# geometrian/simple-spectral

Measured on AMD Instinct MI355X. Metric: Msamples/s (w*h*spp/s) cornell-srgb 512x512, higher is better.
Workload: dtype f32

## Files before the change

### include/ssx.h

```cpp
#ifndef SSX_H
#define SSX_H

#include <stddef.h>
#include <stdint.h>

#ifdef __cplusplus
extern "C" {
#endif

#define SSX_ABI_VERSION 2

enum {
	SSX_OK = 0,
	SSX_ERR_DATA = -1,
	SSX_ERR_ARG = -2,
	SSX_ERR_SCENE = -3,
	SSX_ERR_DEVICE = -10,
	SSX_ERR_STATE = -11
};

#define SSX_MAX_DEPTH 10u
#define SSX_TILE_SIZE 8u
#define SSX_SAMPLE_WAVELENGTHS 4u
#define SSX_MAX_TEXTURES 64u
// ... 46 lines not shown
	uint32_t struct_size;
	uint32_t reserved;
	double pv_inv[16];
	float cam_pos[3];
	float lambda_min;
	float lambda_step;
	uint32_t spec_xbar, spec_ybar, spec_zbar;
	uint32_t spec_basis_r, spec_basis_g, spec_basis_b;
	const ssx_spectrum* spectra;  uint32_t n_spectra;
	const float* samples;         uint32_t n_samples;
	const ssx_material* materials; uint32_t n_materials;
	const ssx_quad* quads;        uint32_t n_quads;
	const uint32_t* lights;       uint32_t n_lights;
	const ssx_texture* textures;  uint32_t n_textures;
	float srgb_to_linear[256];
	uint32_t uplift;
	uint32_t jh_res;
	const float* jh_scale;
	const float* jh_data;
	const ssx_meng_grid* meng;
	float cam_dir[3];
	uint32_t reserved2;
} ssx_scene_desc;

typedef struct ssx_render_params {
	uint32_t struct_size;
	uint32_t width, height;
	uint32_t spp;
	uint32_t indirect_only;
	uint32_t tile_first;
	uint32_t tile_stride;
	uint32_t spp_per_launch;
	uint32_t no_explicit_light_sampling;
	uint32_t no_flat_field_correction;
	uint32_t tile_major;
	uint32_t tile_skew;
	uint64_t seed;
	uint32_t libm;
	uint32_t reserved3;
} ssx_render_params;
enum { SSX_LIBM_BUILD = 0, SSX_LIBM_GLIBC_2_35 = 1 };


typedef struct ssx_ctx ssx_ctx;

int ssx_create(int device, ssx_ctx** out);
void ssx_destroy(ssx_ctx* ctx);

int ssx_upload_scene(ssx_ctx* ctx, const ssx_scene_desc* scene);

int ssx_render_start(ssx_ctx* ctx, const ssx_render_params* params);
int ssx_render_stop(ssx_ctx* ctx);
int ssx_is_rendering(ssx_ctx* ctx);
float ssx_progress(ssx_ctx* ctx);
uint32_t ssx_done_spp(ssx_ctx* ctx);
uint32_t ssx_done_tiles(ssx_ctx* ctx);
int ssx_render_wait(ssx_ctx* ctx, float* xyza_out);

int ssx_render_device(ssx_ctx* ctx, const ssx_render_params* params, void* d_xyza_out, void* hip_stream);
int ssx_render_device_wait(ssx_ctx* ctx);

void* ssx_device_framebuffer(ssx_ctx* ctx);
int ssx_device_index(ssx_ctx* ctx);
int ssx_read_framebuffer(ssx_ctx* ctx, float* xyza_out);
int ssx_accumulate_peer(ssx_ctx* ctx, void* d_dst, int src_device, const void* d_src, uint32_t width, uint32_t height, void* hip_stream);

int ssx_reduce_rccl(ssx_ctx** ctxs, int n, uint32_t width, uint32_t height);
int ssx_rccl_probe(char* report, size_t report_size);
uint64_t ssx_rccl_groups_made(void);

const char* ssx_last_error(const ssx_ctx* ctx);

int ssx_set_timing(ssx_ctx* ctx, int enable);
int ssx_get_timing(ssx_ctx* ctx, float stage_ms[4]);

int ssx_abi_version(void);
int ssx_kernel_info(ssx_ctx* ctx, int* vgprs, int* sgprs, int* lds_bytes, int* scratch_bytes, int* max_blocks_per_cu);
int ssx_plan_info(ssx_ctx* ctx, float* frames_per_sample, int* fold_in_path_kernel);
int ssx_calibration_info(ssx_ctx* ctx, float* frames_per_sample, float* rays_left_per_sample, int* camera_rays_pretraced);
int ssx_scratch_info(ssx_ctx* ctx, uint64_t* sample_bytes, uint64_t* log_bytes);
int ssx_sums_info(ssx_ctx* ctx, uint64_t* units_parked, uint64_t* units_chained);
int ssx_units_info(ssx_ctx* ctx, uint64_t* units_enqueued);
int ssx_generate_info(ssx_ctx* ctx, uint64_t* generate_launches, uint64_t* fused_launches);
int ssx_kernel_variant(ssx_ctx* ctx);
enum { SSX_JIT_OFF = 0, SSX_JIT_AT_UPLOAD = 1, SSX_JIT_BACKGROUND = 2 };
int ssx_set_jit(ssx_ctx* ctx, int mode);
enum { SSX_JIT_STATE_NONE = 0,
       SSX_JIT_STATE_GENERIC_MEANWHILE = 1,
       SSX_JIT_STATE_SPECIALISED = 2,
       SSX_JIT_STATE_FAILED = -1 };
int ssx_jit_status(ssx_ctx* ctx, int wait_ms, char* message, size_t message_size);
void ssx_jit_counters(uint64_t* compiled, uint64_t* disk_hits);
const char* ssx_kernel_name(ssx_ctx* ctx);
enum { SSX_TRAIT_INDIRECT_ONLY = 1u, SSX_TRAIT_NO_ELS = 2u, SSX_TRAIT_MIRROR = 4u, SSX_TRAIT_TRI_LIGHT = 8u, SSX_TRAIT_UPLIFT = 16u,
       SSX_TRAIT_RGB_MODE = 32u, SSX_TRAIT_NO_FLAT_FIELD = 64u, SSX_TRAIT_KEEP_SAMPLES = 128u,
       SSX_TRAIT_LIBM = 256u, SSX_TRAIT_SPECTRAL_BINS = 512u, SSX_TRAIT_FORCED_OFF = 1024u };
int ssx_scene_traits(const ssx_scene_desc* scene);
int ssx_render_traits(const ssx_render_params* params);
int ssx_switches_info(ssx_ctx* ctx);


int ssx_render_continue(ssx_ctx* ctx, uint32_t spp_more);

typedef struct ssx_sums_info_t {
	uint32_t struct_size;
	uint32_t width, height;
	uint32_t done_spp;
	uint64_t seed;
	uint32_t indirect_only, no_explicit_light_sampling, no_flat_field_correction, libm;
	uint32_t rgb_mode;
	uint32_t tile_first, tile_stride, tile_skew;
	uint32_t noise_batches;
	uint32_t reserved;
	uint64_t scene_digest;
} ssx_sums_info_t;
uint64_t ssx_scene_digest(ssx_ctx* ctx);
int ssx_sums_export(ssx_ctx* ctx, ssx_sums_info_t* info, double* sums, double* noise_s2);
int ssx_sums_import(ssx_ctx* ctx, const ssx_render_params* params, const ssx_sums_info_t* info, const double* sums, const double* noise_s2);

int ssx_set_noise_estimate(ssx_ctx* ctx, int enable);
int ssx_noise_info(ssx_ctx* ctx, double* v_out, double summary[4]);


int ssx_set_spectral_bins(ssx_ctx* ctx, uint32_t bins);
typedef struct ssx_spectral_info_t {
	uint32_t struct_size;
	uint32_t width, height;
	uint32_t bins;
	uint32_t done_spp;
	uint32_t reserved;
	float lambda_min;
	float bin_width;
} ssx_spectral_info_t;
int ssx_spectral_read(ssx_ctx* ctx, ssx_spectral_info_t* info, float* mean, double* sums, uint32_t* counts);
int ssx_spectral_import(ssx_ctx* ctx, const ssx_spectral_info_t* info, const double* sums , const uint32_t* counts );


int ssx_guides(ssx_ctx* ctx, uint32_t width, uint32_t height, uint32_t* prim, float* depth, float* normal, float* albedo);
typedef struct ssx_denoise_params {
	uint32_t struct_size;
	uint32_t levels;
	float sigma_l, sigma_a;
} ssx_denoise_params;
int ssx_denoise_images(ssx_ctx* ctx, const ssx_denoise_params* params, uint32_t width, uint32_t height, const float* xyza, const float* var,
                       const uint32_t* prim, const float* albedo, float* xyza_out, float* var_out);
int ssx_denoise(ssx_ctx* ctx, const ssx_denoise_params* params, float* xyza_out, float* var_out);


int ssx_denoise_channels(ssx_ctx* ctx, const ssx_denoise_params* params, uint32_t width, uint32_t height, const float* xyza, const float* var,
                         const uint32_t* prim, const float* albedo, uint32_t channels, const float* extra ,
                         float* xyza_out, float* var_out, float* extra_out );
int ssx_denoise_spectral(ssx_ctx* ctx, const ssx_denoise_params* params, float* mean_out , float* xyza_out, float* var_out);


int ssx_develop_images(ssx_ctx* ctx, uint32_t width, uint32_t height, uint32_t bins, const float* q , const float* weights ,
                       uint32_t channels, float* out );
int ssx_spectral_develop(ssx_ctx* ctx, const ssx_denoise_params* denoise, const float* weights , uint32_t channels, float* out );


int ssx_albedo_bins(ssx_ctx* ctx, uint32_t width, uint32_t height, uint32_t bins, uint32_t supersample, float* rho_out );
#define SSX_DEMOD_DEFAULT_FLOOR 0.0625f
#define SSX_DEMOD_DEFAULT_SIGMA_L 1.0f
typedef struct ssx_demod_params {
	uint32_t struct_size;
	uint32_t supersample;
	float albedo_floor;
// ... 190 lines not shown
```

### simple_spectral_amd/_capi.py

```python
import ctypes as C
import os

from . import build as _build


class SsxSpectrum(C.Structure):
    _fields_ = [("offset", C.c_uint32), ("n", C.c_uint32), ("low", C.c_float), ("high", C.c_float),
                ("delta_recip", C.c_float)]


class SsxVertex(C.Structure):
    _fields_ = [("pos", C.c_float * 3), ("st", C.c_float * 2)]


class SsxQuad(C.Structure):
    _fields_ = [("v00", SsxVertex), ("v10", SsxVertex), ("v11", SsxVertex), ("v01", SsxVertex),
                ("normal0", C.c_float * 3), ("normal1", C.c_float * 3),
                ("material", C.c_uint32), ("flags", C.c_uint32)]


class SsxMaterial(C.Structure):
    _fields_ = [("kind", C.c_uint32), ("albedo_mode", C.c_uint32), ("albedo_spectrum", C.c_uint32),
                ("albedo_texture", C.c_uint32), ("emission_spectrum", C.c_uint32)]

# ... 41 lines not shown
                ("indirect_only", C.c_uint32), ("no_explicit_light_sampling", C.c_uint32), ("no_flat_field_correction", C.c_uint32), ("libm", C.c_uint32),
                ("rgb_mode", C.c_uint32), ("tile_first", C.c_uint32), ("tile_stride", C.c_uint32), ("tile_skew", C.c_uint32),
                ("noise_batches", C.c_uint32), ("reserved", C.c_uint32), ("scene_digest", C.c_uint64)]


class SsxSpectralInfo(C.Structure):
    _fields_ = [("struct_size", C.c_uint32), ("width", C.c_uint32), ("height", C.c_uint32), ("bins", C.c_uint32), ("done_spp", C.c_uint32),
                ("reserved", C.c_uint32), ("lambda_min", C.c_float), ("bin_width", C.c_float)]


class SsxDemodParams(C.Structure):
    _fields_ = [("struct_size", C.c_uint32), ("supersample", C.c_uint32), ("albedo_floor", C.c_float)]


SSX_DEMOD_DEFAULT_SUPERSAMPLE, SSX_DEMOD_DEFAULT_FLOOR, SSX_DEMOD_DEFAULT_SIGMA_L = 2, 0.0625, 1.0


class SsxDenoiseParams(C.Structure):
    _fields_ = [("struct_size", C.c_uint32), ("levels", C.c_uint32), ("sigma_l", C.c_float), ("sigma_a", C.c_float)]


class SsxOpticsParams(C.Structure):
    _fields_ = [("struct_size", C.c_uint32), ("cx", C.c_float), ("cy", C.c_float), ("max_radius", C.c_uint32),
                ("scale", C.c_void_p), ("radius", C.c_void_p), ("taps", C.c_void_p)]


SSX_OPTICS_MAX_RADIUS = 12


class SsxDefocusParams(C.Structure):
    _fields_ = [("struct_size", C.c_uint32), ("max_radius", C.c_uint32), ("gain", C.c_float), ("focus", C.c_void_p)]


SSX_DEFOCUS_MAX_RADIUS = 12


class SsxSensorParams(C.Structure):
    _fields_ = [("struct_size", C.c_uint32), ("cfa", C.c_uint32 * 4), ("noise", C.c_uint32), ("seed", C.c_uint32), ("frame", C.c_uint32),
                ("exposure", C.c_float), ("inv_exposure", C.c_float), ("read_var", C.c_float), ("dn_per_e", C.c_float), ("e_per_dn", C.c_float),
                ("black", C.c_float), ("white", C.c_float), ("weights", C.c_void_p), ("taps", C.c_void_p), ("ccm", C.c_void_p)]


SSH_DEMOSAIC_BILINEAR, SSH_DEMOSAIC_MHC = 0, 1


class SshSpectrum(C.Structure):
    _fields_ = [("samples", C.POINTER(C.c_float)), ("n", C.c_uint32), ("low", C.c_float), ("high", C.c_float)]


SSH_SPACE_XYZ, SSH_SPACE_LRGB = 0, 1
SSX_LIBM_BUILD, SSX_LIBM_GLIBC_2_35 = 0, 1
LIBM_MODES = {"build": SSX_LIBM_BUILD, "glibc-2.35": SSX_LIBM_GLIBC_2_35}


SSX_MODE_RGB, SSX_UPLIFT_OURS, SSX_UPLIFT_MENG, SSX_UPLIFT_JH = 0, 1, 2, 3
SSX_PRIM_LIGHT, SSX_PRIM_TRI = 1, 0x100
SSX_OK, SSX_ERR_DATA, SSX_ERR_ARG, SSX_ERR_SCENE, SSX_ERR_DEVICE, SSX_ERR_STATE = 0, -1, -2, -3, -10, -11
SSX_ABI_VERSION = 2
SSX_JIT_OFF, SSX_JIT_AT_UPLOAD, SSX_JIT_BACKGROUND = 0, 1, 2
(SSX_TRAIT_INDIRECT_ONLY, SSX_TRAIT_NO_ELS, SSX_TRAIT_MIRROR, SSX_TRAIT_TRI_LIGHT, SSX_TRAIT_UPLIFT, SSX_TRAIT_RGB_MODE, SSX_TRAIT_NO_FLAT_FIELD,
 SSX_TRAIT_KEEP_SAMPLES, SSX_TRAIT_LIBM, SSX_TRAIT_SPECTRAL_BINS, SSX_TRAIT_FORCED_OFF) = (1 << i for i in range(11))
SSX_JIT_STATE_NONE, SSX_JIT_STATE_GENERIC_MEANWHILE, SSX_JIT_STATE_SPECIALISED, SSX_JIT_STATE_FAILED = 0, 1, 2, -1

HIP_SYMBOLS = ["ssx_create", "ssx_destroy", "ssx_upload_scene", "ssx_render_start", "ssx_render_stop",
               "ssx_is_rendering", "ssx_progress", "ssx_render_wait", "ssx_render_device", "ssx_last_error",
               "ssx_abi_version", "ssx_kernel_info", "ssx_plan_info", "ssx_set_timing", "ssx_get_timing",
               "ssx_device_framebuffer", "ssx_device_index", "ssx_read_framebuffer", "ssx_accumulate_peer",
               "ssx_debug_eval", "ssx_debug_samples", "ssx_debug_sweep", "ssx_kernel_variant", "ssx_kernel_name", "ssx_scratch_info", "ssx_calibration_info", "ssx_set_jit", "ssx_debug_pass1_source", "ssx_done_spp", "ssx_reduce_rccl", "ssx_sums_info", "ssx_rccl_groups_made", "ssx_jit_status", "ssx_jit_counters", "ssx_done_tiles", "ssx_render_device_wait", "ssx_units_info", "ssx_rccl_probe",
               "ssx_render_continue", "ssx_scene_digest", "ssx_sums_export", "ssx_sums_import", "ssx_set_noise_estimate", "ssx_noise_info",
               "ssx_set_spectral_bins", "ssx_spectral_read", "ssx_debug_sample_flux",
               "ssx_guides", "ssx_denoise_images", "ssx_denoise", "ssx_denoise_channels", "ssx_denoise_spectral",
               "ssx_develop_images", "ssx_spectral_develop",
               "ssx_albedo_bins", "ssx_denoise_spectral_demod", "ssx_spectral_develop_demod",
               "ssx_spectral_import",
               "ssx_set_spectral_moments", "ssx_spectral_variance", "ssx_spectral_probe", "ssx_probe_arrays",
               "ssx_spectral_noise", "ssx_spectral_noise_reduce",
               "ssx_spectral_moments_import",
               "ssx_spectral_compare", "ssx_spectral_compare_arrays",
               "ssx_delta_e_images", "ssx_spectral_delta_e",
               "ssx_optics_images", "ssx_spectral_develop_optics",
               "ssx_defocus_images", "ssx_spectral_develop_lens",
               "ssx_sensor_images", "ssx_demosaic_images", "ssx_spectral_develop_sensor",
               "ssx_debug_tile_mask", "ssx_debug_spectral_accumulate", "ssx_debug_fold", "ssx_debug_step",
               "ssx_debug_generate", "ssx_generate_info",
               "ssx_scene_traits", "ssx_render_traits", "ssx_switches_info"]
SSX_GENERATE_FILL_BYTE = 0xA6
SSX_FOLD_ROW_WORDS, SSX_FOLD_LAMBDA0, SSX_FOLD_CAM_DIR, SSX_FOLD_HIT, SSX_FOLD_N, SSX_FOLD_LEVEL0, SSX_FOLD_LEVEL_WORDS = 160, 0, 1, 4, 5, 10, 15
SSX_FOLD_L_FS, SSX_FOLD_L_NDL, SSX_FOLD_L_PDF, SSX_FOLD_L_FLAGS, SSX_FOLD_L_EMISSION, SSX_FOLD_L_NEE = 0, 4, 5, 6, 7, 11
SSX_FOLD_EMISSION, SSX_FOLD_NEE, SSX_FOLD_NEE_VISIBLE = 1, 2, 4
SSX_STEP_ROW_WORDS, SSX_STEP_R_ORIG, SSX_STEP_R_DIR, SSX_STEP_R_IGNORE, SSX_STEP_R_DEPTH, SSX_STEP_R_LAMBDA0, SSX_STEP_R_RNG, SSX_STEP_R_PREV_SLOT = 16, 0, 3, 6, 7, 8, 9, 13
SSX_STEP_NO_SLOT, SSX_STEP_OUT_WORDS = 0x1FFF, 40
(SSX_STEP_O_FLAGS, SSX_STEP_O_HIT_TRI, SSX_STEP_O_HIT_DIST, SSX_STEP_O_HIT_ST, SSX_STEP_O_EMISSION, SSX_STEP_O_NEE, SSX_STEP_O_NEE_TERM, SSX_STEP_O_FS, SSX_STEP_O_NDL,
 SSX_STEP_O_PDF, SSX_STEP_O_PREV_SLOT, SSX_STEP_O_TAIL_DEPTH, SSX_STEP_O_TAIL_HIT, SSX_STEP_O_NEXT_ORIG, SSX_STEP_O_NEXT_DIR, SSX_STEP_O_NEXT_IGNORE,
 SSX_STEP_O_NEXT_DEPTH, SSX_STEP_O_RNG, SSX_STEP_O_SLOT) = 0, 1, 2, 3, 5, 9, 13, 17, 21, 22, 23, 24, 25, 26, 29, 32, 33, 34, 36
SSX_STEP_HIT, SSX_STEP_CONTINUED, SSX_STEP_EMISSION, SSX_STEP_PARKED, SSX_STEP_VISIBLE = 1, 2, 4, 8, 16
(SSX_SWEEP_RCP, SSX_SWEEP_SQRT, SSX_SWEEP_INVERSESQRT, SSX_SWEEP_SIN, SSX_SWEEP_COS, SSX_SWEEP_ACOS, SSX_SWEEP_DIV_PI,
 SSX_SWEEP_RCP64, SSX_SWEEP_DIV_PAIRS, SSX_SWEEP_ACOS_SIN, SSX_SWEEP_SIN_PROOF, SSX_SWEEP_COS_PROOF, SSX_SWEEP_ACOS_PROOF) = range(1, 14)
(SSX_DBG_FMATH, SSX_DBG_SPHTRI, SSX_DBG_ARVO, SSX_DBG_SAMPLE_LIGHT, SSX_DBG_COSHEMI, SSX_DBG_TRACE, SSX_DBG_RAND_CHOICE,
 SSX_DBG_ALBEDO, SSX_DBG_FLUX_TO_XYZ, SSX_DBG_RAND_1F) = range(1, 11)
(SSX_DBG_GLIBC_MATH, SSX_DBG_SPHTRI_GLIBC, SSX_DBG_ARVO_GLIBC, SSX_DBG_SAMPLE_LIGHT_GLIBC, SSX_DBG_COSHEMI_GLIBC) = range(11, 16)
(SSX_SWEEP_GLIBC_SIN, SSX_SWEEP_GLIBC_COS, SSX_SWEEP_GLIBC_ACOS, SSX_SWEEP_GLIBC_COS_LDS) = range(14, 18)
SSX_DBG_TRACE_TOPO = 17
SSX_DBG_TRACE_MASKED = 16
HOST_SYMBOLS = ["ssh_scene_create", "ssh_scene_create_ex", "ssh_scene_destroy", "ssh_scene_desc", "ssh_xyza_to_srgba", "ssh_save_image",
                "ssh_load_png_rgb8", "ssh_free", "ssh_color_values", "ssh_last_error", "ssh_checkpoint_save", "ssh_checkpoint_load", "ssh_sums_merge", "ssh_save_npy_f32",
                "ssh_develop_weights", "ssh_relight_gain", "ssh_emitter_spectrum",
                "ssh_checkpoint_save_spectral", "ssh_checkpoint_load_spectral", "ssh_spectral_merge",
                "ssh_probe_derive", "ssh_probe_save_csv", "ssh_spectral_noise_derive", "ssh_spectral_noise_save_csv",
                "ssh_checkpoint_save_moments", "ssh_checkpoint_load_moments", "ssh_moments_merge",
                "ssh_compare_derive", "ssh_compare_save_csv",
                "ssh_delta_e_derive", "ssh_delta_e_save_csv", "ssh_develop_white",
                "ssh_optics_lens", "ssh_defocus_thin_lens", "ssh_scene_vfov",
                "ssh_sensor_bayer", "ssh_sensor_exposure", "ssh_sensor_ccm", "ssh_sensor_standin_curve"]

_hip = None
_host = None


def host_lib():
    global _host
    if _host is None:
        path = _build.HOST_LIB
        if not os.path.exists(path):
            _build.build_host()
        lib = C.CDLL(path)
        vp = C.c_void_p
        lib.ssh_last_error.restype = C.c_char_p
        lib.ssh_scene_create.argtypes = [C.c_char_p, C.c_char_p, C.c_int, vp, C.c_uint32, C.c_uint32, C.c_char_p,
                                         C.c_float, C.POINTER(vp)]
        lib.ssh_scene_create_ex.argtypes = [C.c_char_p, C.c_char_p, C.c_int, vp, C.c_uint32, C.c_uint32, C.c_char_p,
                                            C.c_float, C.c_uint32, C.c_char_p, C.c_uint32, C.POINTER(vp)]
        lib.ssh_scene_destroy.argtypes = [vp]
        lib.ssh_scene_desc.restype = C.POINTER(SsxSceneDesc)
        lib.ssh_scene_desc.argtypes = [vp]
        lib.ssh_xyza_to_srgba.argtypes = [vp, vp, vp, C.c_size_t]
        lib.ssh_save_image.argtypes = [C.c_char_p, vp, C.c_uint32, C.c_uint32]
        lib.ssh_load_png_rgb8.argtypes = [C.c_char_p, C.POINTER(C.POINTER(C.c_uint8)), C.POINTER(C.c_uint32),
                                          C.POINTER(C.c_uint32)]
        lib.ssh_free.argtypes = [vp]
        lib.ssh_color_values.argtypes = [vp, C.c_char_p, C.POINTER(C.c_float), C.c_int]
        lib.ssh_checkpoint_save.argtypes = [C.c_char_p, C.POINTER(SsxSumsInfo), C.c_char_p, C.c_char_p, vp, vp]
        lib.ssh_checkpoint_load.argtypes = [C.c_char_p, C.POINTER(SsxSumsInfo), C.c_char_p, C.c_size_t, C.c_char_p, C.c_size_t,
                                            C.POINTER(C.POINTER(C.c_double)), C.POINTER(C.POINTER(C.c_double))]
        lib.ssh_sums_merge.argtypes = [vp, vp, vp, vp, C.POINTER(SsxSumsInfo)]
        lib.ssh_checkpoint_save_spectral.argtypes = [C.c_char_p, C.POINTER(SsxSumsInfo), C.c_char_p, C.c_char_p, vp, vp, C.POINTER(SsxSpectralInfo), vp, vp]
        lib.ssh_checkpoint_load_spectral.argtypes = [C.c_char_p, C.POINTER(SsxSumsInfo), C.c_char_p, C.c_size_t, C.c_char_p, C.c_size_t,
                                                     C.POINTER(C.POINTER(C.c_double)), C.POINTER(C.POINTER(C.c_double)),
                                                     C.POINTER(SsxSpectralInfo), C.POINTER(C.POINTER(C.c_double)), C.POINTER(C.POINTER(C.c_uint32))]
        lib.ssh_spectral_merge.argtypes = [vp, vp, vp, vp, C.c_uint32, C.POINTER(SsxSumsInfo)]
        lib.ssh_checkpoint_save_moments.argtypes = lib.ssh_checkpoint_save_spectral.argtypes + [vp]
        lib.ssh_checkpoint_load_moments.argtypes = lib.ssh_checkpoint_load_spectral.argtypes + [C.POINTER(C.POINTER(C.c_double))]
        lib.ssh_moments_merge.argtypes = [vp, vp, C.c_uint32, C.POINTER(SsxSumsInfo)]
        lib.ssh_save_npy_f32.argtypes = [C.c_char_p, vp, C.POINTER(C.c_uint32), C.c_uint32]
        lib.ssh_probe_derive.argtypes = [C.c_uint32, C.c_uint32, vp, vp, vp, vp, vp, vp]
        lib.ssh_probe_save_csv.argtypes = [C.c_char_p, C.c_uint32, C.c_uint32, C.c_float, C.c_float, vp, vp, vp, vp]
        lib.ssh_spectral_noise_derive.argtypes = [C.c_uint32, vp, vp, vp, vp, vp, vp, vp]
        lib.ssh_spectral_noise_save_csv.argtypes = [C.c_char_p, C.c_uint32, C.c_float, C.c_float, vp, vp, vp, vp]
        lib.ssh_compare_derive.argtypes = [C.c_uint32, C.c_uint32] + [vp] * 12
        lib.ssh_compare_save_csv.argtypes = [C.c_char_p, C.c_uint32, C.c_uint32, C.c_float, C.c_float] + [vp] * 6
        lib.ssh_delta_e_derive.argtypes = [C.c_uint32] + [vp] * 11
        lib.ssh_delta_e_save_csv.argtypes = [C.c_char_p, C.c_uint32] + [vp] * 6
        lib.ssh_develop_white.argtypes = [vp, C.c_uint32, C.c_float, C.c_float, C.POINTER(SshSpectrum), vp]
        lib.ssh_develop_weights.argtypes = [C.c_char_p, C.c_int, C.POINTER(SshSpectrum), C.c_uint32, C.POINTER(SshSpectrum), vp, C.c_int, C.c_uint32,
                                            C.c_float, C.c_float, vp, vp]
        lib.ssh_relight_gain.argtypes = [C.POINTER(SshSpectrum), C.POINTER(SshSpectrum), C.c_uint32, C.c_float, C.c_float, vp]
        lib.ssh_emitter_spectrum.argtypes = [C.POINTER(SsxSceneDesc), C.POINTER(C.c_uint32)]
        lib.ssh_optics_lens.argtypes = [C.c_uint32, C.c_float, C.c_float, C.c_double, C.c_double, C.c_double, C.c_double, C.c_uint32, vp, vp, vp]
# ... 121 lines not shown
            lib.ssx_done_spp.argtypes = [vp]
            lib.ssx_done_spp.restype = C.c_uint32
            lib.ssx_reduce_rccl.argtypes = [C.POINTER(vp), C.c_int, C.c_uint32, C.c_uint32]
            lib.ssx_debug_pass1_source.argtypes = [C.POINTER(C.c_uint8), C.c_uint32, C.c_char_p, C.c_char_p, C.c_size_t]
        if not override or hasattr(lib, "ssx_sums_info"):
            lib.ssx_sums_info.argtypes = [vp, C.POINTER(C.c_uint64), C.POINTER(C.c_uint64)]
        if hasattr(lib, "ssx_rccl_probe"):
            lib.ssx_rccl_probe.argtypes = [C.c_char_p, C.c_size_t]
        if hasattr(lib, "ssx_units_info"):
            lib.ssx_units_info.argtypes = [vp, C.POINTER(C.c_uint64)]
        if not override or hasattr(lib, "ssx_jit_status"):
            lib.ssx_jit_status.argtypes = [vp, C.c_int, C.c_char_p, C.c_size_t]
            lib.ssx_jit_counters.argtypes = [C.POINTER(C.c_uint64), C.POINTER(C.c_uint64)]
            lib.ssx_jit_counters.restype = None
            lib.ssx_rccl_groups_made.restype = C.c_uint64
            lib.ssx_render_device_wait.argtypes = [vp]
            lib.ssx_done_tiles.argtypes = [vp]
            lib.ssx_done_tiles.restype = C.c_uint32
        if not override or hasattr(lib, "ssx_render_continue"):
            lib.ssx_render_continue.argtypes = [vp, C.c_uint32]
            lib.ssx_scene_digest.argtypes = [vp]
            lib.ssx_scene_digest.restype = C.c_uint64
            lib.ssx_sums_export.argtypes = [vp, C.POINTER(SsxSumsInfo), vp, vp]
            lib.ssx_sums_import.argtypes = [vp, C.POINTER(SsxRenderParams), C.POINTER(SsxSumsInfo), vp, vp]
            lib.ssx_set_noise_estimate.argtypes = [vp, C.c_int]
            lib.ssx_noise_info.argtypes = [vp, vp, C.POINTER(C.c_double)]
        if not override or hasattr(lib, "ssx_set_spectral_bins"):
            lib.ssx_set_spectral_bins.argtypes = [vp, C.c_uint32]
            lib.ssx_spectral_read.argtypes = [vp, C.POINTER(SsxSpectralInfo), vp, vp, vp]
            lib.ssx_debug_sample_flux.argtypes = [vp, C.POINTER(SsxRenderParams), vp, vp]
        if not override or hasattr(lib, "ssx_denoise"):
            lib.ssx_guides.argtypes = [vp, C.c_uint32, C.c_uint32, vp, vp, vp, vp]
            lib.ssx_denoise_images.argtypes = [vp, C.POINTER(SsxDenoiseParams), C.c_uint32, C.c_uint32, vp, vp, vp, vp, vp, vp]
            lib.ssx_denoise.argtypes = [vp, C.POINTER(SsxDenoiseParams), vp, vp]
        if not override or hasattr(lib, "ssx_denoise_spectral"):
            lib.ssx_denoise_channels.argtypes = [vp, C.POINTER(SsxDenoiseParams), C.c_uint32, C.c_uint32, vp, vp, vp, vp, C.c_uint32, vp, vp, vp, vp]
            lib.ssx_denoise_spectral.argtypes = [vp, C.POINTER(SsxDenoiseParams), vp, vp, vp]
        if not override or hasattr(lib, "ssx_spectral_develop"):
            lib.ssx_develop_images.argtypes = [vp, C.c_uint32, C.c_uint32, C.c_uint32, vp, vp, C.c_uint32, vp]
            lib.ssx_spectral_develop.argtypes = [vp, C.POINTER(SsxDenoiseParams), vp, C.c_uint32, vp]
        if not override or hasattr(lib, "ssx_albedo_bins"):
            lib.ssx_albedo_bins.argtypes = [vp, C.c_uint32, C.c_uint32, C.c_uint32, C.c_uint32, vp]
            lib.ssx_denoise_spectral_demod.argtypes = [vp, C.POINTER(SsxDenoiseParams), C.POINTER(SsxDemodParams), vp, vp, vp, vp]
            lib.ssx_spectral_develop_demod.argtypes = [vp, C.POINTER(SsxDenoiseParams), C.POINTER(SsxDemodParams), vp, vp, C.c_uint32, vp]
        if not override or hasattr(lib, "ssx_spectral_import"):
            lib.ssx_spectral_import.argtypes = [vp, C.POINTER(SsxSpectralInfo), vp, vp]
        if not override or hasattr(lib, "ssx_set_spectral_moments"):
            lib.ssx_set_spectral_moments.argtypes = [vp, C.c_int]
            lib.ssx_spectral_variance.argtypes = [vp, C.POINTER(SsxSpectralInfo), vp, vp]
            lib.ssx_spectral_probe.argtypes = [vp, vp, C.c_uint32, vp, vp, vp, vp]
            lib.ssx_probe_arrays.argtypes = [vp, C.c_uint32, C.c_uint32, C.c_uint32, vp, vp, vp, vp, C.c_uint32, vp, vp, vp, vp]
        if not override or hasattr(lib, "ssx_spectral_noise"):
            lib.ssx_spectral_noise.argtypes = [vp] * 10
            lib.ssx_spectral_noise_reduce.argtypes = [vp, C.c_uint32, C.c_uint32] + [vp] * 8
        if not override or hasattr(lib, "ssx_spectral_compare"):
            lib.ssx_spectral_compare.argtypes = [vp, C.POINTER(SsxSpectralInfo), vp, vp, vp, vp, C.c_uint32, C.c_double] + [vp] * 8
            lib.ssx_spectral_compare_arrays.argtypes = [vp, C.c_uint32, C.c_uint32, C.c_uint32] + [vp] * 7 + [C.c_uint32, C.c_double] + [vp] * 8
        if not override or hasattr(lib, "ssx_delta_e_images"):
            lib.ssx_delta_e_images.argtypes = [vp, C.c_uint32, C.c_uint32] + [vp] * 5 + [C.c_uint32] + [vp] * 9
            lib.ssx_spectral_delta_e.argtypes = [vp, C.POINTER(SsxDenoiseParams), C.c_int, C.c_int] + [vp] * 5 + [C.c_uint32] + [vp] * 9
        if not override or hasattr(lib, "ssx_optics_images"):
            lib.ssx_optics_images.argtypes = [vp, C.c_uint32, C.c_uint32, C.c_uint32, vp, C.POINTER(SsxOpticsParams), vp]
            lib.ssx_spectral_develop_optics.argtypes = [vp, C.POINTER(SsxDenoiseParams), C.POINTER(SsxOpticsParams), vp, C.c_uint32, vp, vp]
        if not override or hasattr(lib, "ssx_defocus_images"):
            lib.ssx_defocus_images.argtypes = [vp, C.c_uint32, C.c_uint32, C.c_uint32, vp, vp, C.POINTER(SsxDefocusParams), vp]
            lib.ssx_spectral_develop_lens.argtypes = [vp, C.POINTER(SsxDenoiseParams), C.POINTER(SsxDefocusParams), C.POINTER(SsxOpticsParams), vp, C.c_uint32, vp, vp]
        if not override or hasattr(lib, "ssx_sensor_images"):
            lib.ssx_sensor_images.argtypes = [vp, C.c_uint32, C.c_uint32, C.c_uint32, vp, C.POINTER(SsxSensorParams), vp, vp]
            lib.ssx_demosaic_images.argtypes = [vp, C.c_uint32, C.c_uint32, vp, C.POINTER(SsxSensorParams), vp]
            lib.ssx_spectral_develop_sensor.argtypes = [vp, C.POINTER(SsxDenoiseParams), C.POINTER(SsxDefocusParams), C.POINTER(SsxOpticsParams), C.POINTER(SsxSensorParams), vp, vp, vp]
        if not override or hasattr(lib, "ssx_spectral_moments_import"):
            lib.ssx_spectral_moments_import.argtypes = [vp, C.POINTER(SsxSpectralInfo), vp]
        if not override or hasattr(lib, "ssx_debug_tile_mask"):
            lib.ssx_debug_tile_mask.argtypes = [vp, C.POINTER(SsxRenderParams), vp]
        if not override or hasattr(lib, "ssx_debug_spectral_accumulate"):
            lib.ssx_debug_spectral_accumulate.argtypes = [vp] + [C.c_uint32] * 6 + [C.c_float, C.c_float, C.c_uint32] + [vp] * 6
        if not override or hasattr(lib, "ssx_debug_fold"):
            lib.ssx_debug_fold.argtypes = [vp, C.POINTER(SsxRenderParams), C.c_uint32, C.c_uint32, vp, C.c_uint32, C.c_uint32, vp, vp, vp]
        if not override or hasattr(lib, "ssx_debug_step"):
            lib.ssx_debug_step.argtypes = [vp, C.POINTER(SsxRenderParams), C.c_uint32, C.c_uint32, vp, vp]
        if not override or hasattr(lib, "ssx_debug_generate"):
            lib.ssx_debug_generate.argtypes = [vp, C.POINTER(SsxRenderParams), C.c_uint32, C.c_uint32, C.c_int, vp, vp, vp]
            lib.ssx_generate_info.argtypes = [vp, C.POINTER(C.c_uint64), C.POINTER(C.c_uint64)]
        lib.ssx_kernel_variant.argtypes = [vp]
        lib.ssx_kernel_name.argtypes = [vp]
        lib.ssx_kernel_name.restype = C.c_char_p
        if hasattr(lib, "ssx_switches_info"):
            lib.ssx_switches_info.argtypes = [vp]
            lib.ssx_scene_traits.argtypes = [vp]
            lib.ssx_render_traits.argtypes = [vp]
        _hip = lib
    return _hip
```

### simple_spectral_amd/csrc/ssx_api.hip

```cpp
#include "ssx_kernels.hip"
#include "ssx_debug.hip"

#include "../../include/ssx.h"

#include <chrono>
#include <array>
#include <atomic>
#include <cstdarg>
#include <cstdio>
#include <cstdlib>
#include <cmath>
#include <algorithm>
#include <cstring>
#include <mutex>
#include <string>
#include <thread>
#include <vector>

#include <limits.h>
#include <set>

#include "ssx_jit.h"

namespace {
// ... 2 lines not shown

const char* debug_env(const char* name) {
	const char* m = getenv("SSX_DEBUG_ENV");
	if (!m || m[0] != '1' || m[1] != '\0') return nullptr;
	return getenv(name);
}
bool env_on(const char* name) { const char* e = debug_env(name); return e && e[0] != '\0' && e[0] != '0'; }

std::string fmt(const char* f, ...) {
	char buf[512];
	va_list ap; va_start(ap, f); vsnprintf(buf, sizeof buf, f, ap); va_end(ap);
	return buf;
}

struct DeviceBuffer {
	void* ptr = nullptr;
	size_t bytes = 0;
	DeviceBuffer() = default;
	DeviceBuffer(DeviceBuffer&& o) noexcept : ptr(o.ptr), bytes(o.bytes) { o.ptr = nullptr; o.bytes = 0; }
	DeviceBuffer& operator=(DeviceBuffer&& o) noexcept { std::swap(ptr, o.ptr); std::swap(bytes, o.bytes); return *this; }
	~DeviceBuffer() { release(); }
	void release() { if (ptr) (void)hipFree(ptr); ptr = nullptr; bytes = 0; }
	hipError_t reserve(size_t n) {
		if (n <= bytes) return hipSuccess;
		release();
		const hipError_t e = hipMalloc(&ptr, n);
		if (e == hipSuccess) bytes = n; else ptr = nullptr;
		return e;
	}
	template <class T> T* as() const { return static_cast<T*>(ptr); }
};

}

#include "ssx_pack.h"

struct ssx_ctx {
	int device = 0;
	int n_cus = 0;
	hipStream_t stream = nullptr;
	DeviceBuffer d_blob;
	uint32_t blob_words = 0;
	uint32_t path_blob_words = 0;
	uint32_t topology = 0;
	int jit_mode = SSX_JIT_BACKGROUND;
	const ssx_jit::Kernels* jit_kernels[ssx_jit::kVariants] = {};
	uint32_t libm = SSX_LIBM_BUILD;
	uint32_t variant = SSX_LIBM_BUILD;
	bool jit_pending = false, jit_requested = false;
	ssx_jit::VidTable jit_vid;
	DeviceBuffer d_blob_jit; uint32_t blob_jit_words = 0, path_blob_jit_words = 0;
	uint64_t generic_samples = 0;
	int jit_state = SSX_JIT_STATE_NONE; std::string jit_message;
	std::vector<DeviceBuffer> d_textures;
	DeviceBuffer d_jh_data;
	bool rgb_mode = false;
	uint32_t scene_traits = 0;
	bool fuse_resolve = true;
	float calib_frames = 0.0f;
	float calib_left = 0.0f;
	bool pre_hits = false;
	DeviceBuffer d_accum;
	DeviceBuffer d_unit_counter;
	int resident_blocks = 0;
	int gen_blocks = 0;
	uint32_t max_wave_slots = 0;
	uint32_t queue_words = SSX_QUEUE_WORDS_WIDE;
	DeviceBuffer d_samples;
	DeviceBuffer d_logs;
	DeviceBuffer d_out;
	DeviceBuffer d_peer;
	bool have_scene = false;
	bool have_cam_dir = false;

	std::thread worker;
	std::atomic<int> rendering{0};
	std::atomic<int> stop_flag{0};
	std::atomic<uint32_t> done_spp{0};
	std::atomic<uint32_t> done_tiles{0};
	uint32_t total_spp = 0;
	int worker_rc = 0;
	std::atomic<uint64_t> units_enqueued{0};
	std::atomic<uint64_t> launches_generated{0}, launches_fused{0};
	ssx_render_params cur{};
	struct SumsState { bool continuable = false, noise_valid = false, spectral_valid = false, moments_valid = false, imported = false, spectral_imported = false; uint32_t noise_batches = 0; } sums;
	uint32_t k_begin = 0;
	uint64_t scene_digest = 0;
	bool noise_on = false;
	DeviceBuffer d_noise;
	DeviceBuffer d_stage;
	uint32_t spectral_bins = 0;
	DeviceBuffer d_spectral_sums, d_spectral_counts;
	std::string spectral_note;
	float lambda_min = 0.0f, lambda_step = 0.0f;
	uint32_t n_quads = 0;
	bool spectral_moments = false;
	DeviceBuffer d_spectral_moments, d_probe;
	std::string moments_note;
	DeviceBuffer d_guides, d_denoise, d_denoise_channels;
	DeviceBuffer d_develop;
	DeviceBuffer d_optics;
	DeviceBuffer d_defocus;
	DeviceBuffer d_sensor;
	uint32_t guides_width = 0, guides_height = 0;
	DeviceBuffer d_albedo_bins, d_demod;
	uint32_t abins_width = 0, abins_height = 0, abins_bins = 0, abins_supersample = 0;
	uint64_t abins_serial = 0;
	const void* demod_rc_base = nullptr; uint64_t demod_rc_bins_serial = 0; float demod_rc_floor = 0.0f; std::vector<float> demod_rc_weights;

	bool timing = false;
	std::vector<hipEvent_t> ev_pool;
	size_t ev_used = 0;
	float stage_ms[4] = { 0, 0, 0, 0 };

	hipEvent_t ev_device_done = nullptr;
	bool device_pending = false;

	void* rccl_comm = nullptr; uint64_t rccl_group = 0; int rccl_rank = -1, rccl_size = 0;

	std::mutex error_mutex;
	std::string error;
	std::string error_out;
};

namespace {

void set_error(ssx_ctx* ctx, const std::string& msg) { std::lock_guard<std::mutex> g(ctx->error_mutex); ctx->error = msg; }

#define SSX_HIP(ctx, call)                                                                          \
	do {                                                                                            \
		hipError_t e_ = (call);                                                                     \
		if (e_ != hipSuccess) {                                                                     \
			set_error((ctx), fmt("%s failed: %s", #call, hipGetErrorString(e_)));                   \
			return SSX_ERR_DEVICE;                                                                  \
		}                                                                                           \
	} while (0)

int fail(ssx_ctx* ctx, int code, const std::string& msg) { set_error(ctx, msg); return code; }

int check_params(ssx_ctx* ctx, const ssx_render_params* p) {
	if (!p || p->struct_size != sizeof(ssx_render_params)) return fail(ctx, SSX_ERR_ARG, "ssx_render_params.struct_size mismatch");
	if (p->libm != SSX_LIBM_BUILD && p->libm != SSX_LIBM_GLIBC_2_35) return fail(ctx, SSX_ERR_ARG, "ssx_render_params.libm: unknown value");
	if (!ctx->have_scene) return fail(ctx, SSX_ERR_STATE, "no scene uploaded");
	if (p->width == 0 || p->height == 0 || p->spp == 0) return fail(ctx, SSX_ERR_ARG, "width, height and spp must be positive");
	if ((uint64_t)p->width * p->height > (1ull << 28)) return fail(ctx, SSX_ERR_ARG, "image too large");
	if (p->tile_stride == 0 || p->tile_first >= p->tile_stride) return fail(ctx, SSX_ERR_ARG, "need tile_first < tile_stride");
	if (p->no_flat_field_correction && !ctx->have_cam_dir) return fail(ctx, SSX_ERR_ARG, "no_flat_field_correction needs ssx_scene_desc.cam_dir (caller built against an older ssx.h)");
	return SSX_OK;
}

int take_params(ssx_ctx* ctx, const ssx_render_params* in, ssx_render_params* out) {
	if (!in) return fail(ctx, SSX_ERR_ARG, "ssx_render_params is NULL");
	memset(out, 0, sizeof *out);
	if (in->struct_size == offsetof(ssx_render_params, libm)) { memcpy(out, in, offsetof(ssx_render_params, libm)); out->struct_size = sizeof *out; }
	else memcpy(out, in, in->struct_size == sizeof *out ? sizeof *out : sizeof out->struct_size);
	return check_params(ctx, out);
}
int begin_render(ssx_ctx* ctx, const ssx_render_params* in, ssx_render_params* out, const char* busy) {
	const int rc = take_params(ctx, in, out);
	if (rc) return rc;
	return ctx->rendering.load() ? fail(ctx, SSX_ERR_STATE, busy) : SSX_OK;
}

int wait_device_pending(ssx_ctx* ctx) {
	if (ctx->device_pending) { SSX_HIP(ctx, hipEventSynchronize(ctx->ev_device_done)); ctx->device_pending = false; }
	return SSX_OK;
}

int idle_on_device(ssx_ctx* ctx) {
	if (ctx->rendering.load()) return fail(ctx, SSX_ERR_STATE, "render in progress");
	SSX_HIP(ctx, hipSetDevice(ctx->device));
	return wait_device_pending(ctx);
}

uint32_t tiles_across(uint32_t pixels) { return (pixels + 7u) / 8u; }
size_t accum_bytes(uint32_t width, uint32_t height) { return (size_t)tiles_across(width) * tiles_across(height) * 64u * 4 * sizeof(double); }
size_t image_bytes(uint32_t width, uint32_t height) { return (size_t)width * height * 4 * sizeof(float); }

SsxPixelGrid pixel_grid(const ssx_render_params* p) {
	const uint32_t tx = tiles_across(p->width);
	return SsxPixelGrid{ p->width, p->height, tx, p->tile_first, p->tile_stride, p->tile_skew % tx };
}
uint32_t owned_tiles(const ssx_render_params& p) {
	const uint32_t n_tiles = tiles_across(p.width) * tiles_across(p.height);
	return n_tiles > p.tile_first ? (n_tiles - p.tile_first + p.tile_stride - 1u) / p.tile_stride : 0u;
}
dim3 pixel_blocks(const ssx_render_params* p) { return dim3((p->width * p->height + 255u) / 256u); }

int clear_sums(ssx_ctx* ctx, uint32_t width, uint32_t height, hipStream_t stream) {
	SSX_HIP(ctx, hipMemsetAsync(ctx->d_accum.ptr, 0, accum_bytes(width, height), stream));
	return SSX_OK;
}
void sums_invalidate(ssx_ctx* ctx) { ctx->sums = ssx_ctx::SumsState{}; }
void sums_publish(ssx_ctx* ctx, uint32_t done_spp, int64_t noise_batches = -1) {
	if (noise_batches >= 0) { ctx->sums.noise_valid = true; ctx->sums.noise_batches = (uint32_t)noise_batches; }
	ctx->done_spp.store(done_spp); ctx->sums.continuable = true;
}

constexpr size_t kSampleBufferBudget = (size_t)16 << 30;
size_t bytes_per_sample(const ssx_ctx* ctx) { return ctx->spectral_bins ? SSX_BYTES_PER_SAMPLE_FLUX : SSX_BYTES_PER_SAMPLE; }
constexpr size_t kAuxWordsPer64Records = 5;
size_t bytes_per_64_records(const ssx_ctx* ctx) { return 64u * bytes_per_sample(ctx) + kAuxWordsPer64Records * sizeof(uint32_t); }
size_t sample_bytes(const ssx_ctx* ctx, size_t records) { return records / 64u * bytes_per_64_records(ctx); }
size_t sample_slots(const ssx_ctx* ctx) { return ctx->d_samples.bytes / bytes_per_64_records(ctx) * 64u; }
size_t log_records(const ssx_ctx* ctx) { return ctx->d_logs.bytes / SSX_LOG_BYTES_PER_RECORD; }
constexpr uint32_t kMinUnits = 3072;
constexpr uint64_t kSamplesPerSync = (uint64_t)32 << 20;

struct LaunchPlan { SsxKernelArgs args; uint32_t max_spp_per_launch; };

uint32_t scene_traits_of(const ssx_scene_desc* s) {
	uint32_t t = 0;
	for (uint32_t q = 0; q < s->n_quads; ++q) if (s->quads[q].material < s->n_materials && s->materials[s->quads[q].material].kind != SSX_MTL_LAMBERTIAN) t |= SSX_TRAIT_MIRROR;
	for (uint32_t i = 0; i < s->n_lights; ++i) if (s->lights[i] < s->n_quads && (s->quads[s->lights[i]].flags & SSX_PRIM_TRI)) t |= SSX_TRAIT_TRI_LIGHT;
	if (s->uplift == SSX_MODE_RGB) t |= SSX_TRAIT_RGB_MODE;
	else if (s->uplift != SSX_UPLIFT_OURS) t |= SSX_TRAIT_UPLIFT;
	return t;
}
uint32_t render_traits_of(const ssx_render_params* p, bool keep_samples) {
	return (p->indirect_only ? SSX_TRAIT_INDIRECT_ONLY : 0u) | (p->no_explicit_light_sampling ? SSX_TRAIT_NO_ELS : 0u) |
	       (p->no_flat_field_correction ? SSX_TRAIT_NO_FLAT_FIELD : 0u) | (keep_samples ? SSX_TRAIT_KEEP_SAMPLES : 0u) | (p->libm != SSX_LIBM_BUILD ? SSX_TRAIT_LIBM : 0u);
}
uint32_t traits_of(const ssx_ctx* ctx, const ssx_render_params* p, bool keep_samples) {
	const char* e = debug_env("SSX_PLAIN_KERNEL");
	return ctx->scene_traits | render_traits_of(p, keep_samples) | (ctx->spectral_bins ? SSX_TRAIT_SPECTRAL_BINS : 0u) | (e && e[0] == '0' ? SSX_TRAIT_FORCED_OFF : 0u);
}
uint32_t variant_of(const ssx_ctx* ctx, const ssx_render_params* p, bool keep_samples = false) {
	if (ctx->spectral_bins && p->libm == SSX_LIBM_BUILD && !ctx->rgb_mode) return ssx_jit::kVariantFlux;
	return traits_of(ctx, p, keep_samples) == 0u ? (uint32_t)ssx_jit::kVariantPlain : p->libm;
}

LaunchPlan make_plan(ssx_ctx* ctx, const ssx_render_params* p, bool ask_device = true) {
	LaunchPlan pl{};
	SsxKernelArgs& a = pl.args;
	a.blob = ctx->d_blob.as<uint32_t>(); a.blob_words = ctx->path_blob_words;
	a.width = p->width; a.height = p->height;
	a.inv_width = 1.0 / (double)p->width; a.inv_height = 1.0 / (double)p->height;
	a.tiles_x = tiles_across(p->width);
	a.n_tiles = a.tiles_x * tiles_across(p->height);
	a.tile_first = p->tile_first; a.tile_stride = p->tile_stride; a.tile_skew = p->tile_skew % a.tiles_x;
	a.indirect_only = p->indirect_only ? 1u : 0u;
	a.no_els = p->no_explicit_light_sampling ? 1u : 0u;
	a.no_flat_field = p->no_flat_field_correction ? 1u : 0u;
	a.seed = p->seed;
	a.rgb_mode = ctx->rgb_mode ? 1u : 0u;
	a.fuse_resolve = ctx->fuse_resolve ? 1u : 0u;
	a.pre_hits = ctx->pre_hits ? 1u : 0u;
	a.my_tiles = owned_tiles(*p);
	size_t per_spp = (size_t)(a.my_tiles ? a.my_tiles : 1u) * 64u * bytes_per_sample(ctx);
	size_t budget = kSampleBufferBudget, free_b = 0, total_b = 0;
	if (ask_device && hipMemGetInfo(&free_b, &total_b) == hipSuccess) {
		const size_t avail = (size_t)((double)(free_b + sample_slots(ctx) * bytes_per_sample(ctx)) * 0.8);
		if (avail < budget) budget = avail;
	}
	size_t cap = budget / per_spp;
	const size_t idx_cap = (size_t)0xFFFFFFFFu / ((size_t)(a.my_tiles ? a.my_tiles : 1u) * 64u);
	if (cap > idx_cap) cap = idx_cap;
	pl.max_spp_per_launch = (uint32_t)(cap < 1 ? 1 : (cap > 65536 ? 65536 : cap));
	return pl;
}

void cap_to_allocation(const ssx_ctx* ctx, LaunchPlan& pl) {
	const size_t per_spp = (size_t)(pl.args.my_tiles ? pl.args.my_tiles : 1u) * 64u;
	const size_t fit = sample_slots(ctx) / per_spp;
	if (fit >= 1 && fit < pl.max_spp_per_launch) pl.max_spp_per_launch = (uint32_t)fit;
}

int ensure_samples(ssx_ctx* ctx, const LaunchPlan& pl, uint32_t n_k) {
	const size_t need = (size_t)pl.args.my_tiles * 64u * n_k;
	const hipError_t e = ctx->d_samples.reserve(sample_bytes(ctx, need));
	if (e == hipErrorOutOfMemory) { (void)hipGetLastError(); return fail(ctx, SSX_ERR_DEVICE, fmt("out of device memory for %zu samples in flight; lower spp_per_launch", need)); }
	SSX_HIP(ctx, e);
	return SSX_OK;
// ... 74 lines not shown
	a.n_groups = (n_k + a.group_spp - 1) / a.group_spp;
	b.units = a.my_tiles * a.n_groups;
	b.n_rec = a.n_records;
	b.rc = ensure_logs(ctx, a.unit_cohorts);
	if (b.rc == SSX_OK) bind_arrays(a, ctx->d_samples.as<uint8_t>(), a.n_records, ctx->d_logs.as<uint8_t>(), log_records(ctx), ctx->spectral_bins != 0u);
	a.accum = ctx->d_accum.as<double>();
	uint32_t* const aux = reinterpret_cast<uint32_t*>(ctx->d_samples.as<uint8_t>() + sample_slots(ctx) * bytes_per_sample(ctx));
	a.unit_state = aux;
	a.tile_mask = aux + b.units;
	if (b.rc == SSX_OK && (size_t)a.my_tiles * 4u + b.units > (sample_slots(ctx) / 64u) * kAuxWordsPer64Records) b.rc = fail(ctx, SSX_ERR_STATE, "internal: launch larger than the sample allocation");
	return b;
}

size_t staged_blob_lds(uint32_t blob_words) { return ((size_t)blob_words + SSX_LDS_PREFIX_WORDS) * 4; }
size_t path_lds_bytes(uint32_t blob_words, uint32_t queue_words) {
	size_t n = staged_blob_lds(blob_words) + 4u * ((size_t)SSX_QUEUE_ENTRIES * queue_words + SSX_WAVE_COUNTER_WORDS) * 4u;
#ifdef SSX_REGTIME
	n += 4u * SSX_NTIME * 8u;
#endif
	return n;
}
struct PathKernel { const char* name; void (*host)(SsxKernelArgs); };
#define SSX_PK(k) { #k, k }
static const PathKernel kPathKernels[ssx_jit::kVariants][3][2] = {
	{ { SSX_PK(ssx_render_kernel), SSX_PK(ssx_render_kernel_nq) }, { SSX_PK(ssx_render_kernel_cornell), SSX_PK(ssx_render_kernel_cornell_nq) },
	  { SSX_PK(ssx_render_kernel_plane), SSX_PK(ssx_render_kernel_plane_nq) } },
	{ { SSX_PK(ssx_render_kernel_glibc), SSX_PK(ssx_render_kernel_nq_glibc) }, { SSX_PK(ssx_render_kernel_cornell_glibc), SSX_PK(ssx_render_kernel_cornell_nq_glibc) },
	  { SSX_PK(ssx_render_kernel_plane_glibc), SSX_PK(ssx_render_kernel_plane_nq_glibc) } },
	{ { SSX_PK(ssx_render_kernel_flux), SSX_PK(ssx_render_kernel_nq_flux) }, { SSX_PK(ssx_render_kernel_cornell_flux), SSX_PK(ssx_render_kernel_cornell_nq_flux) },
	  { SSX_PK(ssx_render_kernel_plane_flux), SSX_PK(ssx_render_kernel_plane_nq_flux) } },
	{ { SSX_PK(ssx_render_kernel_plain), SSX_PK(ssx_render_kernel_nq_plain) }, { SSX_PK(ssx_render_kernel_cornell_plain), SSX_PK(ssx_render_kernel_cornell_nq_plain) },
	  { SSX_PK(ssx_render_kernel_plane_plain), SSX_PK(ssx_render_kernel_plane_nq_plain) } } };
#undef SSX_PK
static const char* const kJitKernelNames[2] = { "ssx_render_kernel_jit", "ssx_render_kernel_jit_nq" };
const PathKernel& path_kernel_of(const ssx_ctx* ctx, bool narrow) { return kPathKernels[ctx->variant][ctx->topology < 3u ? ctx->topology : 0u][narrow]; }
struct KernelRef { const void* host = nullptr; hipFunction_t mod = nullptr; };
KernelRef path_kernel_ref(const ssx_ctx* ctx, bool narrow) {
	KernelRef k;
	const ssx_jit::Kernels* jk = ctx->jit_kernels[ctx->variant];
	if (ctx->topology == 3u && jk) k.mod = narrow ? jk->path_nq : jk->path;
	else k.host = (const void*)path_kernel_of(ctx, narrow).host;
	return k;
}
int occupancy_of(ssx_ctx* ctx, const KernelRef& k, size_t lds, int* per_cu) {
	if (k.mod) SSX_HIP(ctx, hipModuleOccupancyMaxActiveBlocksPerMultiprocessor(per_cu, k.mod, 256, lds));
	else SSX_HIP(ctx, hipOccupancyMaxActiveBlocksPerMultiprocessor(per_cu, k.host, 256, lds));
	return SSX_OK;
}
int blocks_that_fit(ssx_ctx* ctx, const KernelRef& k, size_t lds, int* blocks) {
	int per_cu = 0;
	const int rc = occupancy_of(ctx, k, lds, &per_cu);
	if (rc) return rc;
	*blocks = (per_cu > 0 ? per_cu : 1) * ctx->n_cus;
	return SSX_OK;
}
int launch_kernel(ssx_ctx* ctx, const KernelRef& k, uint32_t blocks, size_t lds, hipStream_t stream, SsxKernelArgs& a) {
	if (k.mod) {
		size_t size = sizeof a;
		void* config[] = { HIP_LAUNCH_PARAM_BUFFER_POINTER, &a, HIP_LAUNCH_PARAM_BUFFER_SIZE, &size, HIP_LAUNCH_PARAM_END };
		SSX_HIP(ctx, hipModuleLaunchKernel(k.mod, blocks, 1, 1, 256, 1, 1, (unsigned)lds, stream, nullptr, config));
	} else {
		void* args[] = { &a };
		SSX_HIP(ctx, hipLaunchKernel(k.host, dim3(blocks), dim3(256), args, lds, stream));
	}
	return SSX_OK;
}
int pick_queue(ssx_ctx* ctx, uint32_t blob_words, uint32_t* queue_words, int* blocks_per_cu) {
	int wide = 0, narrow = 0, rc;
	if (path_lds_bytes(blob_words, SSX_QUEUE_WORDS_WIDE) <= 65536u)
		if ((rc = occupancy_of(ctx, path_kernel_ref(ctx, false), path_lds_bytes(blob_words, SSX_QUEUE_WORDS_WIDE), &wide))) return rc;
	if ((rc = occupancy_of(ctx, path_kernel_ref(ctx, true), path_lds_bytes(blob_words, SSX_QUEUE_WORDS_NARROW), &narrow))) return rc;
	const bool use_narrow = narrow > wide || env_on("SSX_NARROW_QUEUE");
	*queue_words = use_narrow ? SSX_QUEUE_WORDS_NARROW : SSX_QUEUE_WORDS_WIDE;
	if (blocks_per_cu) *blocks_per_cu = use_narrow ? narrow : wide;
	return SSX_OK;
}

bool fuses_generate(const ssx_ctx* ctx, const SsxKernelArgs& a) {
	const char* fuse_env = debug_env("SSX_FUSE_GEN");
	const bool tiles_fit = a.tiles_x <= 0xFFFFu && tiles_across(a.height) <= 0xFFFFu;
	return ctx->topology == 2u && !a.pre_hits && tiles_fit && !(fuse_env && fuse_env[0] == '0');
}

int enqueue_generate(ssx_ctx* ctx, const Batch& b, hipStream_t stream) {
	SsxKernelArgs ga = b.a;
	ga.blob_words = ctx->blob_words;
	if (ga.pre_hits) {
		hipLaunchKernelGGL(ssx_tile_mask_kernel, dim3((ga.my_tiles + 3u) / 4u), dim3(256), 0, stream, ga);
		SSX_HIP(ctx, hipGetLastError());
	}
	const KernelRef gen_kernel{ (const void*)ssx_generate_kernel };
	const size_t gen_lds = staged_blob_lds(ga.blob_words);
	if (ctx->gen_blocks == 0) { const int rc = blocks_that_fit(ctx, gen_kernel, gen_lds, &ctx->gen_blocks); if (rc) return rc; }
	const uint64_t want = (b.n_rec + 255u) / 256u;
	return launch_kernel(ctx, gen_kernel, (uint32_t)(want < (uint64_t)ctx->gen_blocks ? want : (uint64_t)ctx->gen_blocks), gen_lds, stream, ga);
}

int enqueue_path(ssx_ctx* ctx, Batch& b, const KernelRef& kernel, uint32_t queue_words, uint32_t blob_words, int resident_blocks, hipStream_t stream) {
	if (!ctx->d_unit_counter.ptr) {
		SSX_HIP(ctx, ctx->d_unit_counter.reserve(4 * sizeof(uint32_t)));
		SSX_HIP(ctx, hipMemsetAsync(ctx->d_unit_counter.ptr, 0, 4 * sizeof(uint32_t), stream));
	}
	b.a.blob_words = blob_words; b.a.queue_words = queue_words;
	SSX_HIP(ctx, hipMemsetAsync(ctx->d_unit_counter.ptr, 0, 2 * sizeof(uint32_t), stream));
	SSX_HIP(ctx, hipMemsetAsync(b.a.unit_state, 0, (size_t)b.units * sizeof(uint32_t), stream));
	b.a.unit_counter = ctx->d_unit_counter.as<uint32_t>();
	const uint32_t want_blocks = (b.units + 3u) / 4u;
	uint32_t blocks = want_blocks < (uint32_t)resident_blocks ? want_blocks : (uint32_t)resident_blocks;
	if (blocks * 4u > ctx->max_wave_slots) blocks = ctx->max_wave_slots / 4u;
	return launch_kernel(ctx, kernel, blocks, path_lds_bytes(blob_words, queue_words), stream, b.a);
}

int launch_batch(ssx_ctx* ctx, Batch& b, hipStream_t stream) {
	if (b.rc) return b.rc;
	int rc;
	if (ctx->variant == ssx_jit::kVariantPlain && (b.a.indirect_only | b.a.no_els | b.a.no_flat_field | b.a.rgb_mode | b.a.keep_samples | ctx->scene_traits))
		return fail(ctx, SSX_ERR_STATE, "internal: a render with a switch set was about to launch the kernel with the switches compiled in");
	if (ctx->timing) { if ((rc = timing_events(ctx, &b.tev))) return rc; SSX_HIP(ctx, hipEventRecord(b.tev[0], stream)); }
	b.a.fuse_gen = fuses_generate(ctx, b.a) ? 1u : 0u;
	if (!b.a.fuse_gen && (rc = enqueue_generate(ctx, b, stream))) return rc;
	if (ctx->timing) SSX_HIP(ctx, hipEventRecord(b.tev[1], stream));
	const bool plan = ctx->resident_blocks == 0;
	if (plan && (rc = pick_queue(ctx, b.a.blob_words, &ctx->queue_words, nullptr))) return rc;
	const KernelRef path_kernel = path_kernel_ref(ctx, ctx->queue_words == SSX_QUEUE_WORDS_NARROW);
	if (plan && (rc = blocks_that_fit(ctx, path_kernel, path_lds_bytes(b.a.blob_words, ctx->queue_words), &ctx->resident_blocks))) return rc;
	if ((rc = enqueue_path(ctx, b, path_kernel, ctx->queue_words, b.a.blob_words, ctx->resident_blocks, stream))) return rc;
	ctx->units_enqueued.fetch_add(b.units);
	(b.a.fuse_gen ? ctx->launches_fused : ctx->launches_generated).fetch_add(1u);
	if (ctx->timing) for (int k = 2; k < 6; ++k) SSX_HIP(ctx, hipEventRecord(b.tev[k], stream));
	return SSX_OK;
}

constexpr uint64_t kJitAfterSamples = kSamplesPerSync;
void maybe_swap_jit(ssx_ctx* ctx, uint64_t samples) {
	if (!ctx->jit_pending) return;
	std::string err;
	const ssx_jit::Kernels* k = nullptr;
	const ssx_jit::State st = ssx_jit::lookup(ctx->device, ctx->jit_vid, &k, &err, ctx->variant);
	if (st == ssx_jit::State::Ready) {
		std::swap(ctx->d_blob, ctx->d_blob_jit);
		ctx->blob_words = ctx->blob_jit_words; ctx->path_blob_words = ctx->path_blob_jit_words;
		ctx->topology = 3u;
		ctx->jit_kernels[ctx->variant] = k;
		ctx->resident_blocks = 0; ctx->gen_blocks = 0;
		ctx->jit_pending = false; ctx->jit_state = SSX_JIT_STATE_SPECIALISED;
	} else if (st == ssx_jit::State::Failed) {
		ctx->jit_pending = false; ctx->jit_state = SSX_JIT_STATE_FAILED; ctx->jit_message = err;
	} else {
		ctx->generic_samples += samples;
		if (!ctx->jit_requested && ctx->generic_samples >= kJitAfterSamples) { ssx_jit::request(ctx->jit_vid, ctx->variant); ctx->jit_requested = true; }
	}
}

int ensure_libm_kernels(ssx_ctx* ctx, uint32_t libm) {
	const ssx_jit::Kernels*& have = ctx->jit_kernels[libm];
	if (ctx->topology != 3u || have) return SSX_OK;
	std::string err;
	const ssx_jit::Kernels* k = ssx_jit::get(ctx->device, ctx->jit_vid, &err, libm);
	if (!k) return fail(ctx, SSX_ERR_STATE, "the scene's specialised kernels for this libm could not be compiled: " + err);
	have = k;
	return SSX_OK;
}

int ready_to_launch(ssx_ctx* ctx, const ssx_render_params* p, bool need_out, bool keep_samples = false) {
	const uint32_t variant = variant_of(ctx, p, keep_samples);
	const int rc = ensure_libm_kernels(ctx, variant);
	if (rc) return rc;
	ctx->libm = p->libm;
	if (ctx->variant != variant) { ctx->variant = variant; ctx->resident_blocks = 0; ctx->jit_requested = false; }
	SSX_HIP(ctx, ctx->d_accum.reserve(accum_bytes(p->width, p->height)));
	if (need_out) SSX_HIP(ctx, ctx->d_out.reserve(image_bytes(p->width, p->height)));
	return SSX_OK;
}

int launch_range(ssx_ctx* ctx, LaunchPlan& pl, uint32_t k0, uint32_t k1, hipStream_t stream) {
	if (pl.args.my_tiles == 0 || k1 <= k0) return SSX_OK;
	Batch b = make_batch(ctx, pl, k0, k1);
	return launch_batch(ctx, b, stream);
}

int launch_batches(ssx_ctx* ctx, LaunchPlan& pl, uint32_t spp, uint32_t batch, hipStream_t stream) {
	for (uint32_t k0 = 0; k0 < spp; k0 += batch) {
		int rc = launch_range(ctx, pl, k0, (spp - k0 < batch) ? spp : k0 + batch, stream);
		if (rc) return rc;
	}
	return SSX_OK;
}

int calibrate(ssx_ctx* ctx) {
	ssx_render_params cp{};
	cp.struct_size = sizeof cp; cp.width = 64; cp.height = 64; cp.spp = 4; cp.tile_stride = 1;
	ctx->fuse_resolve = false;
	ctx->pre_hits = false;
	LaunchPlan pl = make_plan(ctx, &cp);
	int rc = ensure_samples(ctx, pl, cp.spp);
	if (rc) return rc;
	Batch b = make_batch(ctx, pl, 0, cp.spp);
	if (b.rc) return b.rc;
	if ((rc = enqueue_generate(ctx, b, ctx->stream))) return rc;
	const KernelRef kernel{ (const void*)ssx_calibrate_kernel };
	int blocks = 0;
	if ((rc = blocks_that_fit(ctx, kernel, path_lds_bytes(ctx->blob_words, SSX_QUEUE_WORDS_NARROW), &blocks))) return rc;
	if ((rc = enqueue_path(ctx, b, kernel, SSX_QUEUE_WORDS_NARROW, ctx->blob_words, blocks, ctx->stream))) return rc;
	SSX_HIP(ctx, hipStreamSynchronize(ctx->stream));
	std::vector<uint4> recs((size_t)b.n_rec);
	SSX_HIP(ctx, hipMemcpy(recs.data(), b.a.st, recs.size() * sizeof(uint4), hipMemcpyDeviceToHost));
	uint64_t frames = 0;
	for (const uint4& r : recs) frames += (r.y >> 2) & 0xFu;
	ctx->calib_frames = (float)((double)frames / (double)recs.size());
	uint32_t counters[2] = { 0u, 0u };
	SSX_HIP(ctx, hipMemcpy(counters, ctx->d_unit_counter.ptr, sizeof counters, hipMemcpyDeviceToHost));
	ctx->calib_left = (float)((double)counters[1] / (double)recs.size());
	ctx->pre_hits = ctx->calib_left >= 0.3f;
	if (const char* e = debug_env("SSX_PRE_HITS")) { if (e[0] != '\0') ctx->pre_hits = e[0] != '0'; }
	ctx->fuse_resolve = true;
	return ensure_logs(ctx, (unit_spp_of(ctx) + SSX_COHORT_KS - 1u) / SSX_COHORT_KS);
}

int launch_finalize(ssx_ctx* ctx, const ssx_render_params* p, uint32_t spp, float* d_out, hipStream_t stream, uint32_t done_tiles = 0xFFFFFFFFu) {
	hipLaunchKernelGGL(ssx_finalize_kernel, pixel_blocks(p), dim3(256), 0, stream,
	                   ctx->d_accum.as<const double>(), (float4*)d_out, pixel_grid(p), spp, ctx->rgb_mode ? 1u : 0u, done_tiles);
	SSX_HIP(ctx, hipGetLastError());
	return SSX_OK;
}

int noise_begin(ssx_ctx* ctx, const ssx_render_params* p, uint32_t k_begin, bool continuing);
int noise_batch(ssx_ctx* ctx, const ssx_render_params* p, uint32_t n_k, hipStream_t stream);
int spectral_refuses(ssx_ctx* ctx, const ssx_render_params& p, bool tile_walk);
int spectral_begin(ssx_ctx* ctx, uint32_t my_tiles, bool continuing, bool* active);
int spectral_batch(ssx_ctx* ctx, const ssx_render_params* p, const LaunchPlan& pl, uint32_t n_k, hipStream_t stream);
int moments_reserve(ssx_ctx* ctx, uint32_t my_tiles, bool continuing);
int moments_begin(ssx_ctx* ctx, uint32_t my_tiles, bool continuing, bool spectral, bool* active);
int moments_batch(ssx_ctx* ctx, const ssx_render_params* p, const LaunchPlan& pl, uint32_t n_k, hipStream_t stream);
void moments_publish(ssx_ctx* ctx, bool active);
void moments_invalidate(ssx_ctx* ctx, const char* why);
void moments_drop(ssx_ctx* ctx);

int finish_walk(ssx_ctx* ctx, const ssx_render_params& p, uint32_t spp, uint32_t done_tiles) {
	if (const int rc = launch_finalize(ctx, &p, spp, ctx->d_out.as<float>(), ctx->stream, done_tiles)) return rc;
	SSX_HIP(ctx, hipStreamSynchronize(ctx->stream));
	return SSX_OK;
}

uint32_t sample_walk_chunk(const ssx_render_params& p, uint32_t span, const LaunchPlan& pl) {
	const size_t pixels = (size_t)p.width * p.height;
	const uint64_t min_spp = kSamplesPerSync / (pixels ? pixels : 1) + 1u;
	uint32_t chunk = p.spp_per_launch ? p.spp_per_launch : (span + 31u) / 32u;
	if (!p.spp_per_launch && chunk < min_spp) chunk = (uint32_t)(min_spp < span ? min_spp : span);
	if (chunk == 0) chunk = 1;
	return chunk > pl.max_spp_per_launch ? pl.max_spp_per_launch : chunk;
}

struct TileLaunch { uint32_t tiles, spp; };
TileLaunch tile_walk_launch(const ssx_render_params& p, const LaunchPlan& pl) {
	const uint32_t owned = pl.args.my_tiles;
	uint32_t spp_l = p.spp_per_launch ? p.spp_per_launch : p.spp;
	if (spp_l > p.spp) spp_l = p.spp;
	uint64_t per_launch = kSamplesPerSync / ((uint64_t)64 * p.spp) + 1u;
	if (const char* e = debug_env("SSX_TILES_PER_LAUNCH")) { const int v = atoi(e); if (v >= 1) per_launch = (uint64_t)v; }
	if (per_launch > owned) per_launch = owned;
	const uint64_t budget_records = (uint64_t)pl.max_spp_per_launch * owned * 64u;
	while (spp_l > 1u && (uint64_t)spp_l * 64u > budget_records) spp_l = (spp_l + 1u) / 2u;
	const uint64_t fit = budget_records / ((uint64_t)spp_l * 64u);
	if (per_launch > fit) per_launch = fit ? fit : 1u;
	return TileLaunch{ (uint32_t)per_launch, spp_l };
}

int render_sample_walk(ssx_ctx* ctx, const ssx_render_params& p, uint32_t k_begin, bool continuing) {
	int rc;
	if (!continuing && (rc = clear_sums(ctx, p.width, p.height, ctx->stream))) return rc;
	if ((rc = noise_begin(ctx, &p, k_begin, continuing))) return rc;
	maybe_swap_jit(ctx, 0);
	if ((rc = moments_reserve(ctx, owned_tiles(p), continuing))) return rc;
	LaunchPlan pl = make_plan(ctx, &p);
	bool spectral = false, moments = false;
	if ((rc = spectral_begin(ctx, pl.args.my_tiles, continuing, &spectral))) return rc;
	if ((rc = moments_begin(ctx, pl.args.my_tiles, continuing, spectral, &moments))) return rc;
	const uint32_t span = p.spp - k_begin, chunk = sample_walk_chunk(p, span, pl);
	if ((rc = ensure_samples(ctx, pl, chunk < span ? chunk : span))) return rc;
	for (uint32_t k0 = k_begin; k0 < p.spp && !ctx->stop_flag.load(); k0 += chunk) {
		const uint32_t k1 = (p.spp - k0 < chunk) ? p.spp : k0 + chunk;
		if (ctx->jit_pending) {
			maybe_swap_jit(ctx, (uint64_t)p.width * p.height * (k1 - k0) / p.tile_stride);
			if (!ctx->jit_pending) { const uint32_t cap = pl.max_spp_per_launch; pl = make_plan(ctx, &p); pl.max_spp_per_launch = cap; }
		}
		if ((rc = launch_range(ctx, pl, k0, k1, ctx->stream))) return rc;
		if (ctx->noise_on && (rc = noise_batch(ctx, &p, k1 - k0, ctx->stream))) return rc;
		if (spectral && (rc = spectral_batch(ctx, &p, pl, k1 - k0, ctx->stream))) return rc;
		if (moments && (rc = moments_batch(ctx, &p, pl, k1 - k0, ctx->stream))) return rc;
		SSX_HIP(ctx, hipStreamSynchronize(ctx->stream));
		ctx->done_spp.store(k1);
	}
	const uint32_t done = ctx->done_spp.load();
	if ((rc = finish_walk(ctx, p, done ? done : p.spp, 0xFFFFFFFFu))) return rc;
	ctx->done_tiles.store(pl.args.my_tiles);
	ctx->sums.spectral_valid = spectral;
	if (!spectral) ctx->spectral_note = "the render that made these sums ran without them (it continued sums that had none)";
	moments_publish(ctx, moments);
	sums_publish(ctx, done);
	return SSX_OK;
}

int render_tile_walk(ssx_ctx* ctx, const ssx_render_params& p) {
	int rc;
	if ((rc = clear_sums(ctx, p.width, p.height, ctx->stream))) return rc;
	maybe_swap_jit(ctx, 0);
	const LaunchPlan pl = make_plan(ctx, &p);
	const uint32_t owned = pl.args.my_tiles;
	const TileLaunch per = tile_walk_launch(p, pl);
	LaunchPlan sized = pl; sized.args.my_tiles = per.tiles;
	if ((rc = ensure_samples(ctx, sized, per.spp))) return rc;
	for (uint32_t j0 = 0; j0 < owned && !ctx->stop_flag.load(); j0 += per.tiles) {
		const uint32_t j1 = (owned - j0 < per.tiles) ? owned : j0 + per.tiles;
		maybe_swap_jit(ctx, (uint64_t)(j1 - j0) * 64u * p.spp);
		LaunchPlan part = make_plan(ctx, &p);
		part.args.tile_first = p.tile_first + p.tile_stride * j0;
		part.args.my_tiles = j1 - j0;
		if ((rc = launch_batches(ctx, part, p.spp, per.spp, ctx->stream))) return rc;
		SSX_HIP(ctx, hipStreamSynchronize(ctx->stream));
		ctx->done_tiles.store(j1);
		ctx->done_spp.store((uint32_t)((uint64_t)p.spp * j1 / owned));
	}
	const uint32_t done = ctx->done_tiles.load();
	if ((rc = finish_walk(ctx, p, p.spp, done))) return rc;
	if (done == owned) sums_publish(ctx, p.spp);
	return SSX_OK;
}

int render_walk(ssx_ctx* ctx, const ssx_render_params p, uint32_t k_begin, bool continuing) {
	SSX_HIP(ctx, hipSetDevice(ctx->device));
	return (p.tile_major && !continuing) ? render_tile_walk(ctx, p) : render_sample_walk(ctx, p, k_begin, continuing);
}
void worker_main(ssx_ctx* ctx, uint32_t k_begin, bool continuing) {
	const int rc = render_walk(ctx, ctx->cur, k_begin, continuing);
	if (rc) sums_invalidate(ctx);
	ctx->worker_rc = rc;
	ctx->rendering.store(0);
}

int start_worker(ssx_ctx* ctx, const ssx_render_params& p, uint32_t k_begin, bool continuing, uint32_t total_spp) {
	if (ctx->worker.joinable()) ctx->worker.join();
	if (const int rc = spectral_refuses(ctx, p, p.tile_major && !continuing)) return rc;
	if (const int rc = ready_to_launch(ctx, &p, true)) return rc;
	ctx->cur = p; ctx->total_spp = total_spp; ctx->k_begin = k_begin;
	if (!continuing) { sums_invalidate(ctx); ctx->done_spp.store(0); ctx->done_tiles.store(0); }
	ctx->sums.imported = ctx->sums.spectral_imported = false;
	ctx->stop_flag.store(0); ctx->worker_rc = 0;
	ctx->rendering.store(1);
	ctx->worker = std::thread(worker_main, ctx, k_begin, continuing);
	return SSX_OK;
}

uint64_t digest_mix(uint64_t h, uint64_t w) {
	uint64_t z = (h ^ w) + 0x9E3779B97F4A7C15ull;
	z = (z ^ (z >> 30)) * 0xBF58476D1CE4E5B9ull;
	z = (z ^ (z >> 27)) * 0x94D049BB133111EBull;
	return z ^ (z >> 31);
}
uint64_t digest_bytes(uint64_t h, const void* data, size_t n) {
	const uint8_t* p = static_cast<const uint8_t*>(data);
	h = digest_mix(h, (uint64_t)n);
	for (; n >= 8; n -= 8, p += 8) { uint64_t w; memcpy(&w, p, 8); h = digest_mix(h, w); }
	if (n) { uint64_t w = 0; memcpy(&w, p, n); h = digest_mix(h, w); }
	return h;
}
uint64_t scene_digest_of(const ssx_scene_desc* s) {
	std::vector<uint32_t> blob;
	std::string err;
	const std::vector<const void*> no_tex(s->n_textures, nullptr);
	if (pack_blob(s, no_tex, nullptr, blob, err) != SSX_OK) return 0;
	uint64_t h = digest_bytes(0x5353584449474553ull, blob.data(), blob.size() * 4);
	for (uint32_t i = 0; i < s->n_textures; ++i) h = digest_bytes(h, s->textures[i].rgb, (size_t)3 * s->textures[i].width * s->textures[i].height);
	if (s->uplift == SSX_UPLIFT_JH) h = digest_bytes(h, s->jh_data, (size_t)3 * s->jh_res * s->jh_res * s->jh_res * 3 * sizeof(float));
	if (s->uplift == SSX_UPLIFT_MENG) {
		const ssx_meng_grid* g = s->meng;
// ... 175 lines not shown
	const uint32_t upload_variant = variant_of(ctx, &defaults) == ssx_jit::kVariantPlain ? (uint32_t)ssx_jit::kVariantPlain : (uint32_t)SSX_LIBM_BUILD;
	if (ctx->variant == SSX_LIBM_BUILD || ctx->variant == ssx_jit::kVariantPlain) ctx->variant = upload_variant;
	if (info.candidate && jit_mode != SSX_JIT_OFF) {
		std::string err;
		const ssx_jit::Kernels* k = nullptr;
		ssx_jit::State st = ssx_jit::lookup(ctx->device, info.vid, &k, &err, upload_variant);
		if (st != ssx_jit::State::Ready && st != ssx_jit::State::Failed && jit_mode == SSX_JIT_AT_UPLOAD) {
			k = ssx_jit::get(ctx->device, info.vid, &err, upload_variant);
			st = k ? ssx_jit::State::Ready : ssx_jit::State::Failed;
		}
		if (st == ssx_jit::State::Failed) { ctx->jit_state = SSX_JIT_STATE_FAILED; ctx->jit_message = err; }
		else if ((rc = pack_blob(s, tex, ctx->d_jh_data.ptr, blob_jit, pack_err, 3))) return fail(ctx, rc, pack_err);
		else if (st == ssx_jit::State::Ready) { blob.swap(blob_jit); blob_jit.clear(); ctx->jit_kernels[upload_variant] = k; ctx->jit_vid = info.vid; ctx->jit_state = SSX_JIT_STATE_SPECIALISED; }
		else { ctx->jit_pending = true; ctx->jit_vid = info.vid; ctx->jit_state = SSX_JIT_STATE_GENERIC_MEANWHILE; ctx->jit_requested = (st == ssx_jit::State::Pending); }
	}
	if (ctx->jit_pending) {
		SSX_HIP(ctx, ctx->d_blob_jit.reserve(blob_jit.size() * 4));
		SSX_HIP(ctx, hipMemcpy(ctx->d_blob_jit.ptr, blob_jit.data(), blob_jit.size() * 4, hipMemcpyHostToDevice));
		const SsxBlobHeader* bh = reinterpret_cast<const SsxBlobHeader*>(blob_jit.data());
		ctx->blob_jit_words = (uint32_t)blob_jit.size(); ctx->path_blob_jit_words = bh->words_without_perm;
	}
	SSX_HIP(ctx, ctx->d_blob.reserve(blob.size() * 4));
	SSX_HIP(ctx, hipMemcpy(ctx->d_blob.ptr, blob.data(), blob.size() * 4, hipMemcpyHostToDevice));
	ctx->blob_words = (uint32_t)blob.size();
	{
		SsxBlobHeader* bh = reinterpret_cast<SsxBlobHeader*>(blob.data());
		ctx->topology = bh->topology;
		ctx->path_blob_words = (bh->topology || bh->perm_hbm) ? bh->words_without_perm : ctx->blob_words;
		if (bh->perm_hbm) {
			const uint64_t at = (uint64_t)(uintptr_t)(ctx->d_blob.as<uint32_t>() + bh->off_perm);
			bh->perm_ptr_lo = (uint32_t)at; bh->perm_ptr_hi = (uint32_t)(at >> 32);
			SSX_HIP(ctx, hipMemcpy(ctx->d_blob.ptr, blob.data(), sizeof(SsxBlobHeader), hipMemcpyHostToDevice));
			ctx->blob_words = bh->words_without_perm;
		}
	}
	ctx->have_cam_dir = have_cam_dir;
	ctx->lambda_min = s->lambda_min; ctx->lambda_step = s->lambda_step;
	ctx->n_quads = s->n_quads;
	ctx->resident_blocks = 0; ctx->gen_blocks = 0;
	ctx->have_scene = true;
	ctx->scene_digest = scene_digest_of(s);
	return calibrate(ctx);
}

static uint32_t device_batch(const ssx_render_params* p, const LaunchPlan& pl) {
	uint32_t batch = p->spp_per_launch ? p->spp_per_launch : p->spp;
	if (batch > p->spp) batch = p->spp;
	if (batch > pl.max_spp_per_launch) {
		const uint32_t n = (p->spp + pl.max_spp_per_launch - 1u) / pl.max_spp_per_launch;
		batch = (p->spp + n - 1u) / n;
	}
	return batch;
}

int ssx_render_device(ssx_ctx* ctx, const ssx_render_params* p_in, void* d_xyza_out, void* hip_stream) {
	if (!ctx) return SSX_ERR_ARG;
	ssx_render_params pp;
	int rc = take_params(ctx, p_in, &pp);
	if (rc) return rc;
	const ssx_render_params* const p = &pp;
	if (!d_xyza_out) return fail(ctx, SSX_ERR_ARG, "d_xyza_out is NULL");
	if (ctx->spectral_bins) return fail(ctx, SSX_ERR_ARG, "spectral output is on (ssx_set_spectral_bins): ssx_render_device does not bin its samples; use ssx_render_start");
	if (ctx->rendering.load()) return fail(ctx, SSX_ERR_STATE, "asynchronous render in progress");
	hipStream_t stream = (hipStream_t)hip_stream;
	SSX_HIP(ctx, hipSetDevice(ctx->device));
	if (!ctx->ev_device_done) SSX_HIP(ctx, hipEventCreateWithFlags(&ctx->ev_device_done, hipEventDisableTiming));
	hipStreamCaptureStatus capture = hipStreamCaptureStatusNone;
	(void)hipStreamIsCapturing(stream, &capture);
	const bool capturing = capture == hipStreamCaptureStatusActive;
	if (ctx->device_pending && capturing) return fail(ctx, SSX_ERR_STATE, "a render of this context may still be queued: ssx_render_device_wait before capturing another into a graph");
	if (capturing && ctx->variant != variant_of(ctx, p)) return fail(ctx, SSX_ERR_STATE, "ssx_render_params.libm differs from the context's last render: run it once outside the stream capture first");
	if (ctx->device_pending) SSX_HIP(ctx, hipStreamWaitEvent(stream, ctx->ev_device_done, 0));
	{
		LaunchPlan probe = make_plan(ctx, p, !capturing);
		if (capturing) cap_to_allocation(ctx, probe);
		const uint32_t probe_batch = device_batch(p, probe);
		const size_t need = (size_t)probe.args.my_tiles * 64u * probe_batch;
		const bool grow = ctx->d_accum.bytes < accum_bytes(p->width, p->height) || ctx->d_samples.bytes < sample_bytes(ctx, need);
		if (grow && capturing) return fail(ctx, SSX_ERR_STATE, "the context's buffers have to grow for this render: run it once outside the stream capture first");
		if (grow && (rc = wait_device_pending(ctx))) return rc;
	}
	if ((rc = ready_to_launch(ctx, p, false))) return rc;
	sums_invalidate(ctx);
	if ((rc = clear_sums(ctx, p->width, p->height, stream))) return rc;
	if (!capturing) maybe_swap_jit(ctx, (uint64_t)p->width * p->height * p->spp / p->tile_stride);
	LaunchPlan pl = make_plan(ctx, p, !capturing);
	if (capturing) cap_to_allocation(ctx, pl);
	const uint32_t batch = device_batch(p, pl);
	if ((rc = ensure_samples(ctx, pl, batch))) return rc;
	if ((rc = launch_batches(ctx, pl, p->spp, batch, stream))) return rc;
	if ((rc = launch_finalize(ctx, p, p->spp, (float*)d_xyza_out, stream))) return rc;
	if (!capturing) {
		SSX_HIP(ctx, hipEventRecord(ctx->ev_device_done, stream));
		ctx->device_pending = true;
	}
	return SSX_OK;
}

int ssx_render_device_wait(ssx_ctx* ctx) {
	if (!ctx) return SSX_ERR_ARG;
	if (!ctx->device_pending) return SSX_OK;
	SSX_HIP(ctx, hipSetDevice(ctx->device));
	return wait_device_pending(ctx);
}

int ssx_render_start(ssx_ctx* ctx, const ssx_render_params* p_in) {
	if (!ctx) return SSX_ERR_ARG;
	ssx_render_params pp;
	int rc = begin_render(ctx, p_in, &pp, "render already in progress");
	if (rc) return rc;
	SSX_HIP(ctx, hipSetDevice(ctx->device));
	if ((rc = wait_device_pending(ctx))) return rc;
	return start_worker(ctx, pp, 0, false, pp.spp);
}

int ssx_render_stop(ssx_ctx* ctx) {
	if (!ctx) return SSX_ERR_ARG;
	ctx->stop_flag.store(1);
	return SSX_OK;
}

int ssx_is_rendering(ssx_ctx* ctx) { return ctx ? ctx->rendering.load() : 0; }

float ssx_progress(ssx_ctx* ctx) {
	if (!ctx || ctx->total_spp == 0) return 0.0f;
	const uint32_t done = ctx->done_spp.load();
	return done > ctx->k_begin ? (float)(done - ctx->k_begin) / (float)ctx->total_spp : 0.0f;
}

uint32_t ssx_done_spp(ssx_ctx* ctx) { return ctx ? ctx->done_spp.load() : 0u; }

uint32_t ssx_done_tiles(ssx_ctx* ctx) { return ctx ? ctx->done_tiles.load() : 0u; }

int ssx_render_wait(ssx_ctx* ctx, float* xyza_out) {
	if (!ctx) return SSX_ERR_ARG;
	if (!ctx->worker.joinable()) return fail(ctx, SSX_ERR_STATE, "no render was started");
	ctx->worker.join();
	if (ctx->worker_rc) return ctx->worker_rc;
	if (xyza_out) {
		SSX_HIP(ctx, hipSetDevice(ctx->device));
		SSX_HIP(ctx, hipMemcpy(xyza_out, ctx->d_out.ptr, image_bytes(ctx->cur.width, ctx->cur.height), hipMemcpyDeviceToHost));
	}
	return SSX_OK;
}

int ssx_set_timing(ssx_ctx* ctx, int enable) {
	if (!ctx) return SSX_ERR_ARG;
	ctx->timing = enable != 0;
	for (float& m : ctx->stage_ms) m = 0;
	ctx->ev_used = 0;
	return SSX_OK;
}

int ssx_get_timing(ssx_ctx* ctx, float stage_ms[4]) {
	if (!ctx || !stage_ms) return SSX_ERR_ARG;
	SSX_HIP(ctx, hipSetDevice(ctx->device));
	int rc = collect_timing(ctx);
	if (rc) return rc;
	for (int k = 0; k < 4; ++k) { stage_ms[k] = ctx->stage_ms[k]; ctx->stage_ms[k] = 0; }
	return SSX_OK;
}

int ssx_read_framebuffer(ssx_ctx* ctx, float* xyza_out) {
	if (!ctx || !xyza_out) return SSX_ERR_ARG;
	if (ctx->rendering.load()) return fail(ctx, SSX_ERR_STATE, "render in progress");
	if (!ctx->d_out.ptr || ctx->cur.width == 0) return fail(ctx, SSX_ERR_STATE, "no render was started");
	SSX_HIP(ctx, hipSetDevice(ctx->device));
	SSX_HIP(ctx, hipMemcpy(xyza_out, ctx->d_out.ptr, image_bytes(ctx->cur.width, ctx->cur.height), hipMemcpyDeviceToHost));
	return SSX_OK;
}

void* ssx_device_framebuffer(ssx_ctx* ctx) { return ctx ? ctx->d_out.ptr : nullptr; }

int ssx_device_index(ssx_ctx* ctx) { return ctx ? ctx->device : -1; }
// ... 85 lines not shown
	if ((rc = spectral_refuses(ctx, pp, false))) return rc;
	SSX_HIP(ctx, hipSetDevice(ctx->device));
	if ((rc = wait_device_pending(ctx))) return rc;
	if ((rc = ready_to_launch(ctx, p, false, true))) return rc;
	LaunchPlan pl = make_plan(ctx, p);
	if (p->spp > pl.max_spp_per_launch) return fail(ctx, SSX_ERR_ARG, "ssx_debug_samples: too many samples for one launch");
	if ((rc = ensure_samples(ctx, pl, p->spp))) return rc;
	sums_invalidate(ctx);
	if ((rc = clear_sums(ctx, p->width, p->height, ctx->stream))) return rc;
	Batch b = make_batch(ctx, pl, 0, p->spp);
	b.a.keep_samples = 1u;
	if ((rc = launch_batch(ctx, b, ctx->stream))) return rc;
	SSX_HIP(ctx, hipStreamSynchronize(ctx->stream));
	std::vector<float4> ray((size_t)b.n_rec);
	std::vector<uint4> st((size_t)b.n_rec);
	SSX_HIP(ctx, hipMemcpy(ray.data(), b.a.ray, ray.size() * sizeof(float4), hipMemcpyDeviceToHost));
	SSX_HIP(ctx, hipMemcpy(st.data(), b.a.st, st.size() * sizeof(uint4), hipMemcpyDeviceToHost));
	const uint32_t spp = p->spp, tiles_x = tiles_across(p->width);
	for (uint32_t j = 0; j < p->height; ++j) for (uint32_t i = 0; i < p->width; ++i) {
		const uint32_t tile = (j >> 3) * tiles_x + (i >> 3), lane = (j & 7u) * 8u + (i & 7u);
		for (uint32_t k = 0; k < spp; ++k) {
			const size_t r = ((size_t)tile * spp + k) * 64u + lane, o = ((size_t)j * p->width + i) * spp + k;
			if (xyza) { xyza[4 * o + 0] = ray[r].x; xyza[4 * o + 1] = ray[r].y; xyza[4 * o + 2] = ray[r].z; xyza[4 * o + 3] = ray[r].w; }
			if (rng_state) rng_state[o] = ((uint64_t)st[r].w << 32) | st[r].z;
			if (levels) levels[o] = (st[r].y >> 2) & 0xFu;
		}
	}
	return SSX_OK;
}

int ssx_debug_tile_mask(ssx_ctx* ctx, const ssx_render_params* p_in, uint32_t* out) {
	if (!ctx || !out) return SSX_ERR_ARG;
	ssx_render_params pp;
	int rc = begin_render(ctx, p_in, &pp, "render in progress");
	if (rc) return rc;
	SSX_HIP(ctx, hipSetDevice(ctx->device));
	if ((rc = wait_device_pending(ctx))) return rc;
	const LaunchPlan pl = make_plan(ctx, &pp);
	SsxKernelArgs ga = pl.args;
	if (ga.my_tiles == 0u) return SSX_OK;
	ga.blob_words = ctx->blob_words;
	const size_t bytes = (size_t)ga.my_tiles * 4u * sizeof(uint32_t);
	DeviceBuffer d_mask;
	if (d_mask.reserve(bytes) != hipSuccess) { (void)hipGetLastError(); return fail(ctx, SSX_ERR_DEVICE, "out of device memory (ssx_debug_tile_mask)"); }
	ga.tile_mask = d_mask.as<uint32_t>();
	hipLaunchKernelGGL(ssx_tile_mask_kernel, dim3((ga.my_tiles + 3u) / 4u), dim3(256), 0, ctx->stream, ga);
	SSX_HIP(ctx, hipGetLastError());
	SSX_HIP(ctx, hipStreamSynchronize(ctx->stream));
	SSX_HIP(ctx, hipMemcpy(out, d_mask.ptr, bytes, hipMemcpyDeviceToHost));
	return SSX_OK;
}

int ssx_debug_generate(ssx_ctx* ctx, const ssx_render_params* p_in, uint32_t k0, uint32_t n_k, int pre_hits, float* ray, uint32_t* st, float* hit) {
	if (!ctx || !ray || !st) return SSX_ERR_ARG;
	ssx_render_params pp;
	int rc = begin_render(ctx, p_in, &pp, "render in progress");
	if (rc) return rc;
	if (n_k == 0) return fail(ctx, SSX_ERR_ARG, "ssx_debug_generate: n_k must be positive");
	if ((uint64_t)k0 + n_k > 0xFFFFFFFFull) return fail(ctx, SSX_ERR_ARG, "ssx_debug_generate: k0 + n_k does not fit in 32 bits");
	if (pre_hits < -1 || pre_hits > 1) return fail(ctx, SSX_ERR_ARG, "ssx_debug_generate: pre_hits is 0, 1 or -1 (the context's own choice)");
	const bool pre = pre_hits < 0 ? ctx->pre_hits : pre_hits == 1;
	if (pre && !hit) return fail(ctx, SSX_ERR_ARG, "ssx_debug_generate: camera rays are pre-traced, hit must not be NULL");
	SSX_HIP(ctx, hipSetDevice(ctx->device));
	if ((rc = wait_device_pending(ctx))) return rc;
	const LaunchPlan pl = make_plan(ctx, &pp);
	if (n_k > pl.max_spp_per_launch) return fail(ctx, SSX_ERR_ARG, fmt("ssx_debug_generate: %u samples per pixel are more than one launch may cover (%u)", n_k, pl.max_spp_per_launch));
	Batch b{};
	b.a = pl.args;
	SsxKernelArgs& a = b.a;
	if (a.my_tiles == 0u) return SSX_OK;
	a.k0 = k0; a.k1 = k0 + n_k;
	a.n_records = (uint64_t)a.my_tiles * n_k * 64u;
	a.pre_hits = pre ? 1u : 0u;
	b.n_rec = a.n_records;
	const size_t rec_bytes = (size_t)a.n_records * 16u, mask_bytes = (size_t)a.my_tiles * 4u * sizeof(uint32_t);
	DeviceBuffer d_rec, d_mask;
	if (d_rec.reserve(3u * rec_bytes) != hipSuccess || d_mask.reserve(mask_bytes) != hipSuccess) { (void)hipGetLastError(); return fail(ctx, SSX_ERR_DEVICE, "out of device memory (ssx_debug_generate)"); }
	SSX_HIP(ctx, hipMemsetAsync(d_rec.ptr, (int)SSX_GENERATE_FILL_BYTE, 3u * rec_bytes, ctx->stream));
	SSX_HIP(ctx, hipMemsetAsync(d_mask.ptr, 0, mask_bytes, ctx->stream));
	a.ray = reinterpret_cast<float4*>(d_rec.as<uint8_t>());
	a.st = reinterpret_cast<uint4*>(d_rec.as<uint8_t>() + rec_bytes);
	a.hit = reinterpret_cast<float4*>(d_rec.as<uint8_t>() + 2u * rec_bytes);
	a.tile_mask = d_mask.as<uint32_t>();
	if ((rc = enqueue_generate(ctx, b, ctx->stream))) return rc;
	SSX_HIP(ctx, hipStreamSynchronize(ctx->stream));
	SSX_HIP(ctx, hipMemcpy(ray, a.ray, rec_bytes, hipMemcpyDeviceToHost));
	SSX_HIP(ctx, hipMemcpy(st, a.st, rec_bytes, hipMemcpyDeviceToHost));
	if (hit) SSX_HIP(ctx, hipMemcpy(hit, a.hit, rec_bytes, hipMemcpyDeviceToHost));
	return SSX_OK;
}

int ssx_debug_fold(ssx_ctx* ctx, const ssx_render_params* p_in, uint32_t n_pixels, uint32_t spp, const uint32_t* levels, uint32_t order_seed, uint32_t parked,
                   float* out_flux, float* out_xyza, double* out_sums) {
	if (!ctx || !levels) return SSX_ERR_ARG;
	ssx_render_params pp;
	int rc = begin_render(ctx, p_in, &pp, "render in progress");
	if (rc) return rc;
	if (n_pixels == 0 || (n_pixels & 63u) || n_pixels > (1u << 20)) return fail(ctx, SSX_ERR_ARG, "ssx_debug_fold: n_pixels must be a multiple of 64, at most 2^20");
	if (spp == 0 || spp > SSX_MAX_UNIT_KS) return fail(ctx, SSX_ERR_ARG, "ssx_debug_fold: spp must be 1..8, the samples per pixel of a work unit");
	if (parked > 1u) return fail(ctx, SSX_ERR_ARG, "ssx_debug_fold: parked is 0 or 1");
	const bool flux = ctx->spectral_bins && pp.libm == SSX_LIBM_BUILD && !ctx->rgb_mode;
	if (ctx->spectral_bins && !flux) return fail(ctx, SSX_ERR_STATE, "ssx_debug_fold: spectral output is on, and it renders spectral scenes with the default libm only");
	if (out_flux && !flux) return fail(ctx, SSX_ERR_STATE, "ssx_debug_fold: out_flux needs spectral output (ssx_set_spectral_bins)");
	SSX_HIP(ctx, hipSetDevice(ctx->device));
	if ((rc = wait_device_pending(ctx))) return rc;
	const uint32_t variant = flux ? (uint32_t)ssx_jit::kVariantFlux : pp.libm, variant_was = ctx->variant;
	uint32_t qw = 0;
	ctx->variant = variant;
	rc = pick_queue(ctx, ctx->path_blob_words, &qw, nullptr);
	ctx->variant = variant_was;
	if (rc) return rc;
	const bool narrow = qw == SSX_QUEUE_WORDS_NARROW;
	const uint32_t n_tiles = n_pixels / 64u, cohorts = (spp + SSX_COHORT_KS - 1u) / SSX_COHORT_KS;
	const size_t n_rec = (size_t)n_pixels * spp, log_records = (size_t)n_tiles * 2u * cohorts * SSX_COHORT_RECORDS;
	const size_t row_bytes = n_rec * SSX_FOLD_ROW_WORDS * 4u;
	if (log_records * SSX_LOG_BYTES_PER_RECORD >= ((size_t)1 << 32)) return fail(ctx, SSX_ERR_ARG, "ssx_debug_fold: level logs beyond 4 GiB for this many pixels and samples; fold fewer pixels per call");
	DeviceBuffer d_rows, d_samples, d_logs, d_sums;
	if (d_rows.reserve(row_bytes) != hipSuccess || d_samples.reserve(n_rec * SSX_BYTES_PER_SAMPLE_FLUX) != hipSuccess ||
	    d_logs.reserve(log_records * SSX_LOG_BYTES_PER_RECORD) != hipSuccess || d_sums.reserve((size_t)n_tiles * 256u * sizeof(double)) != hipSuccess) {
		(void)hipGetLastError();
		return fail(ctx, SSX_ERR_DEVICE, "out of device memory (ssx_debug_fold)");
	}
	SSX_HIP(ctx, hipMemcpy(d_rows.ptr, levels, row_bytes, hipMemcpyHostToDevice));
	SsxKernelArgs a{};
	a.blob = ctx->d_blob.as<uint32_t>(); a.blob_words = ctx->path_blob_words;
	a.rgb_mode = ctx->rgb_mode ? 1u : 0u;
	a.no_flat_field = pp.no_flat_field_correction ? 1u : 0u;
	a.keep_samples = 1u;
	a.unit_cohorts = cohorts; a.group_spp = spp; a.n_records = n_rec;
	bind_arrays(a, d_samples.as<uint8_t>(), n_rec, d_logs.as<uint8_t>(), log_records, flux);
	a.accum = d_sums.as<double>();
	static const void* const kFoldKernels[ssx_jit::kVariants][2] = {
		{ (const void*)ssx_debug_fold_kernel, (const void*)ssx_debug_fold_kernel_nq }, { (const void*)ssx_debug_fold_kernel_glibc, (const void*)ssx_debug_fold_kernel_nq_glibc },
		{ (const void*)ssx_debug_fold_kernel_flux, (const void*)ssx_debug_fold_kernel_nq_flux } };
	const uint32_t* d_in = d_rows.as<uint32_t>();
	void* args[] = { &a, &d_in, (void*)&n_tiles, &spp, &order_seed, &parked };
	const size_t lds = staged_blob_lds(a.blob_words) + 4u * SSX_WAVE_COUNTER_WORDS * 4u;
	SSX_HIP(ctx, hipLaunchKernel(kFoldKernels[variant][narrow], dim3((n_tiles + 3u) / 4u), dim3(256), args, lds, ctx->stream));
	SSX_HIP(ctx, hipStreamSynchronize(ctx->stream));
	std::vector<float4> rec(n_rec);
	std::vector<double> sums((size_t)n_tiles * 256u);
	auto gather = [&](const void* d_src, float* out) -> int {
		SSX_HIP(ctx, hipMemcpy(rec.data(), d_src, n_rec * sizeof(float4), hipMemcpyDeviceToHost));
		for (uint32_t t = 0; t < n_tiles; ++t) for (uint32_t k = 0; k < spp; ++k) for (uint32_t l = 0; l < 64u; ++l)
			memcpy(out + 4u * (((size_t)t * 64u + l) * spp + k), &rec[((size_t)t * spp + k) * 64u + l], sizeof(float4));
		return SSX_OK;
	};
	if (out_flux && (rc = gather(a.flux, out_flux))) return rc;
	if (out_xyza && (rc = gather(a.ray, out_xyza))) return rc;
	if (out_sums) {
		SSX_HIP(ctx, hipMemcpy(sums.data(), d_sums.ptr, sums.size() * sizeof(double), hipMemcpyDeviceToHost));
		for (uint32_t t = 0; t < n_tiles; ++t) for (uint32_t l = 0; l < 64u; ++l) for (uint32_t c = 0; c < 4u; ++c)
			out_sums[((size_t)t * 64u + l) * 4u + c] = sums[(size_t)t * 256u + c * 64u + l];
	}
	return SSX_OK;
}

int ssx_debug_step(ssx_ctx* ctx, const ssx_render_params* p_in, uint32_t n_rows, uint32_t n_rounds, const uint32_t* rows, uint32_t* out) {
	if (!ctx || !rows || !out) return SSX_ERR_ARG;
	ssx_render_params pp;
	int rc = begin_render(ctx, p_in, &pp, "render in progress");
	if (rc) return rc;
	if (n_rounds == 0 || n_rounds > SSX_MAX_UNIT_KS) return fail(ctx, SSX_ERR_ARG, "ssx_debug_step: n_rounds must be 1..8, the samples per pixel of a work unit (SSX_COHORT_KS x unit_cohorts)");
	if (n_rows == 0 || (n_rows & 63u)) return fail(ctx, SSX_ERR_ARG, "ssx_debug_step: n_rows must be a multiple of 64");
	if (n_rows % (64u * n_rounds)) return fail(ctx, SSX_ERR_ARG, "ssx_debug_step: n_rows must be a multiple of 64 * n_rounds (whole tiles)");
	const uint32_t n_tiles = n_rows / (64u * n_rounds), cohorts = (n_rounds + SSX_COHORT_KS - 1u) / SSX_COHORT_KS;
// ... 67 lines not shown
	(void)hipDeviceSynchronize();
	return (int)hipMemcpyFromSymbol(out, HIP_SYMBOL(g_regtime), SSX_NTIME * sizeof(unsigned long long));
}
#endif

int ssx_set_jit(ssx_ctx* ctx, int mode) {
	if (!ctx || mode < SSX_JIT_OFF || mode > SSX_JIT_BACKGROUND) return SSX_ERR_ARG;
	ctx->jit_mode = mode;
	return SSX_OK;
}

int ssx_jit_status(ssx_ctx* ctx, int wait_ms, char* message, size_t message_size) {
	if (!ctx) return SSX_ERR_ARG;
	if (ctx->rendering.load()) return fail(ctx, SSX_ERR_STATE, "render in progress");
	if (ctx->jit_pending && wait_ms != 0) {
		if (hipSetDevice(ctx->device) != hipSuccess) return fail(ctx, SSX_ERR_DEVICE, "hipSetDevice failed");
		if (!ctx->jit_requested) { ssx_jit::request(ctx->jit_vid, ctx->variant); ctx->jit_requested = true; }
		(void)ssx_jit::wait(ctx->jit_vid, wait_ms < 0 ? 600000 : wait_ms, ctx->variant);
		maybe_swap_jit(ctx, 0);
	}
	copy_text(ctx->jit_message, message, message_size);
	return ctx->jit_state;
}

void ssx_jit_counters(uint64_t* compiled, uint64_t* disk_hits) {
	ssx_jit::Shared& S = ssx_jit::shared();
	std::lock_guard<std::mutex> g(S.m);
	if (compiled) *compiled = S.compiled;
	if (disk_hits) *disk_hits = S.disk_hits;
}

int ssx_debug_pass1_source(const uint8_t* vid, uint32_t n_quads, const char* name, char* out, size_t out_size) {
	if (!vid || !name || n_quads == 0 || n_quads > 32u) return SSX_ERR_ARG;
	ssx_jit::VidTable t(n_quads);
	for (uint32_t q = 0; q < n_quads; ++q) for (int v = 0; v < 4; ++v) t[q][v] = vid[4 * q + v];
	const std::string text = ssx_jit::pass1_source(name, t);
	copy_text(text, out, out_size);
	return (int)text.size();
}

int ssx_calibration_info(ssx_ctx* ctx, float* frames_per_sample, float* rays_left_per_sample, int* camera_rays_pretraced) {
	if (!ctx) return SSX_ERR_ARG;
	if (!ctx->have_scene) return fail(ctx, SSX_ERR_STATE, "no scene uploaded");
	if (frames_per_sample) *frames_per_sample = ctx->calib_frames;
	if (rays_left_per_sample) *rays_left_per_sample = ctx->calib_left;
	if (camera_rays_pretraced) *camera_rays_pretraced = ctx->pre_hits ? 1 : 0;
	return SSX_OK;
}

int ssx_scratch_info(ssx_ctx* ctx, uint64_t* sample_bytes, uint64_t* log_bytes) {
	if (!ctx) return SSX_ERR_ARG;
	if (sample_bytes) *sample_bytes = (uint64_t)sample_slots(ctx) * bytes_per_sample(ctx) + (ctx->spectral_moments ? (uint64_t)ctx->d_spectral_moments.bytes : 0u);
	if (log_bytes) *log_bytes = (uint64_t)ctx->d_logs.bytes;
	return SSX_OK;
}

int ssx_sums_info(ssx_ctx* ctx, uint64_t* units_parked, uint64_t* units_chained) {
	if (!ctx) return SSX_ERR_ARG;
	uint32_t c[4] = { 0u, 0u, 0u, 0u };
	if (ctx->d_unit_counter.ptr) {
		SSX_HIP(ctx, hipSetDevice(ctx->device));
		const int rc = wait_device_pending(ctx);
		if (rc) return rc;
		SSX_HIP(ctx, hipMemcpy(c, ctx->d_unit_counter.ptr, sizeof c, hipMemcpyDeviceToHost));
	}
	if (units_parked) *units_parked = c[2];
	if (units_chained) *units_chained = c[3];
	return SSX_OK;
}

int ssx_units_info(ssx_ctx* ctx, uint64_t* units_enqueued) {
	if (!ctx) return SSX_ERR_ARG;
	if (units_enqueued) *units_enqueued = ctx->units_enqueued.load();
	return SSX_OK;
}

int ssx_generate_info(ssx_ctx* ctx, uint64_t* generate_launches, uint64_t* fused_launches) {
	if (!ctx) return SSX_ERR_ARG;
	if (generate_launches) *generate_launches = ctx->launches_generated.load();
	if (fused_launches) *fused_launches = ctx->launches_fused.load();
	return SSX_OK;
}

int ssx_kernel_variant(ssx_ctx* ctx) { return (ctx && ctx->have_scene) ? (int)ctx->topology : -1; }

const char* ssx_kernel_name(ssx_ctx* ctx) {
	if (!ctx || !ctx->have_scene) return nullptr;
	if (hipSetDevice(ctx->device) != hipSuccess) return nullptr;
	uint32_t qw = 0;
	if (pick_queue(ctx, ctx->path_blob_words, &qw, nullptr) != SSX_OK) return nullptr;
	const bool narrow = qw == SSX_QUEUE_WORDS_NARROW;
	const uint32_t named = ctx->variant == ssx_jit::kVariantPlain ? (uint32_t)SSX_LIBM_BUILD : ctx->variant;
	return ctx->topology == 3u ? kJitKernelNames[narrow] : kPathKernels[named][ctx->topology][narrow].name;
}

int ssx_switches_info(ssx_ctx* ctx) { return (ctx && ctx->have_scene) ? (ctx->variant == ssx_jit::kVariantPlain ? 1 : 0) : -1; }
int ssx_scene_traits(const ssx_scene_desc* s) {
	if (!s || s->struct_size != sizeof(ssx_scene_desc) || (s->n_quads && (!s->quads || !s->materials)) || (s->n_lights && !s->lights)) return -1;
	return (int)scene_traits_of(s);
}
int ssx_render_traits(const ssx_render_params* p) {
	if (!p || p->struct_size != sizeof(ssx_render_params)) return -1;
	return (int)render_traits_of(p, false);
}

int ssx_plan_info(ssx_ctx* ctx, float* frames_per_sample, int* fold_in_path_kernel) {
	if (!ctx) return SSX_ERR_ARG;
	if (!ctx->have_scene) return fail(ctx, SSX_ERR_STATE, "no scene uploaded");
	if (frames_per_sample) *frames_per_sample = ctx->calib_frames;
	if (fold_in_path_kernel) *fold_in_path_kernel = ctx->fuse_resolve ? 1 : 0;
	return SSX_OK;
}

int ssx_kernel_info(ssx_ctx* ctx, int* vgprs, int* sgprs, int* lds_bytes, int* scratch_bytes, int* max_blocks_per_cu) {
	if (!ctx) return SSX_ERR_ARG;
	SSX_HIP(ctx, hipSetDevice(ctx->device));
	hipFuncAttributes at;
	uint32_t qw = 0; int nb = 0;
	int r = pick_queue(ctx, ctx->path_blob_words, &qw, &nb);
	if (r) return r;
	const KernelRef k = path_kernel_ref(ctx, qw == SSX_QUEUE_WORDS_NARROW);
	if (k.mod) {
		int v = 0;
		SSX_HIP(ctx, hipFuncGetAttribute(&v, HIP_FUNC_ATTRIBUTE_NUM_REGS, k.mod)); at.numRegs = v;
		SSX_HIP(ctx, hipFuncGetAttribute(&v, HIP_FUNC_ATTRIBUTE_SHARED_SIZE_BYTES, k.mod)); at.sharedSizeBytes = (size_t)v;
		SSX_HIP(ctx, hipFuncGetAttribute(&v, HIP_FUNC_ATTRIBUTE_LOCAL_SIZE_BYTES, k.mod)); at.localSizeBytes = (size_t)v;
	} else SSX_HIP(ctx, hipFuncGetAttributes(&at, k.host));
	if (vgprs) *vgprs = at.numRegs;
	if (sgprs) *sgprs = 0;
	if (lds_bytes) *lds_bytes = (int)at.sharedSizeBytes + (int)path_lds_bytes(ctx->path_blob_words, qw);
	if (scratch_bytes) *scratch_bytes = (int)at.localSizeBytes;
	if (max_blocks_per_cu) *max_blocks_per_cu = nb;
	return SSX_OK;
}

}

#include "ssx_progressive.hip"
#include "ssx_spectral.hip"
#include "ssx_denoise.hip"
#include "ssx_develop.hip"
#include "ssx_optics.hip"
#include "ssx_defocus.hip"
#include "ssx_sensor.hip"
#include "ssx_demod.hip"
#include "ssx_spectral_stats.hip"
#include "ssx_spectral_noise.hip"
#include "ssx_spectral_compare.hip"
#include "ssx_delta_e.hip"
```

### simple_spectral_amd/csrc/ssx_blob.h

```cpp
#pragma once
#include <stdint.h>
#include <hip/hip_runtime.h>

#define SSX_QUEUE_ENTRIES 128u
#define SSX_QUEUE_WORDS_WIDE 12u
#define SSX_QUEUE_WORDS_NARROW 8u
#define SSX_LDS_PREFIX_WORDS 80u
#define SSX_BLOB_MAX_BYTES 48576u

#define SSX_PERM_COUNT 3u
#define SSX_PERM_WORDS_PER_QUAD (SSX_PERM_COUNT * 12u)
#define SSX_PERM_AXES { { 1u, 2u }, { 0u, 2u }, { 0u, 1u } }

struct SsxBlobSpectrum {
	uint32_t offset;
	uint32_t n;
	float low, delta_recip;
};

struct SsxBlobQuad {
	float pos[4][3];
	float st[4][2];
	float normal[2][3];
	uint32_t kind;
// ... 11 lines not shown
	double pv_inv[16];
	float cam_pos[3];
	float lambda_min, lambda_step;
	uint32_t n_quads, n_lights, n_materials, n_spectra;
	uint32_t spec_xbar, spec_ybar, spec_zbar, spec_basis_r, spec_basis_g, spec_basis_b;
	uint32_t off_perm, off_quads, off_lights, off_spectra, off_lut, off_tex;
	uint32_t n_textures;
	uint32_t total_words;
	uint32_t basis_one_grid;
	uint32_t uplift, jh_res, off_jh_scale, jh_data_lo, jh_data_hi;
	uint32_t observer_one_grid;
	uint32_t off_basis4, off_observer4;
	uint32_t topology, n_verts, off_vtab, vtab_stride, off_vid, words_without_perm, off_vtab4, off_triofs;
	uint64_t tri_valid[4];
	uint32_t perm_hbm, perm_ptr_lo, perm_ptr_hi;
	float cam_dir[3];
	uint32_t black_ends_path;
	uint32_t pad4_[1];
	float lambda_steps[4];
	double n_lights_recip;
	double q_const[4];
	double cam_pos_d[3];
};
static_assert(sizeof(SsxBlobHeader) % 16 == 0, "header must keep 16-byte alignment");

struct SsxBlobTexture {
	uint32_t ptr_lo, ptr_hi, w, h;
};

#define SSX_MAX_FRAMES 9u
#define SSX_MAX_LEVELS 10u
#define SSX_NO_SLOT 0x1FFFu
#ifndef SSX_COHORT_KS
#define SSX_COHORT_KS 2u
#endif
#define SSX_COHORT_RECORDS (64u * SSX_COHORT_KS)
#ifndef SSX_MAX_UNIT_KS
#define SSX_MAX_UNIT_KS 8u
#endif
#define SSX_UNIT_COHORTS (SSX_MAX_UNIT_KS / SSX_COHORT_KS)
#define SSX_WAVE_COUNTER_WORDS (4u * SSX_UNIT_COHORTS + 4u)
#define SSX_UNIT_PARKED 1u
#define SSX_UNIT_TURN 2u
#define SSX_BYTES_PER_SAMPLE (16u + 16u + 16u)
#define SSX_BYTES_PER_SAMPLE_FLUX (SSX_BYTES_PER_SAMPLE + 16u)
#define SSX_LOG_BYTES_PER_RECORD ((16u + 8u + 4u) * SSX_MAX_FRAMES + (16u + 16u + 1u) * SSX_MAX_LEVELS)

struct SsxKernelArgs {
	const uint32_t* blob;
	uint32_t blob_words;
	uint32_t width, height;
	uint32_t tiles_x, n_tiles;
	uint32_t tile_first, tile_stride;
	uint32_t tile_skew;
	uint32_t k0, k1;
	uint32_t indirect_only;
	uint32_t no_els;
	uint32_t my_tiles;
	uint32_t group_spp;
	uint32_t n_groups;
	uint64_t seed;
	float4* ray;
	uint4* st;
	float4* hit;
	uint8_t* logs;
	uint32_t log_cap;
	uint64_t n_records;
	uint32_t* unit_counter;
	uint32_t rgb_mode;
	uint32_t fuse_resolve;
	uint32_t unit_cohorts;
	double* accum;
	uint32_t* tile_mask;
	uint32_t* unit_state;
	uint32_t no_flat_field;
	uint32_t keep_samples;
	uint32_t pre_hits;
	uint32_t queue_words;
	uint32_t unit_grab;
	uint32_t pad_grab_;
	double inv_width, inv_height;
	uint32_t fuse_gen;
	float4* flux;
};
```

### simple_spectral_amd/csrc/ssx_kernels.hip

```cpp
#include <hip/hip_runtime.h>
#ifndef __HIPCC_RTC__
#include <stdint.h>
#endif

#include "ssx_blob.h"
#include "ssx_exact.h"
#include "ssx_lanestat.h"
extern __shared__ __attribute__((aligned(16))) uint32_t ssx_lds[];
#define SSX_FM_TABLE (reinterpret_cast<const double*>(ssx_lds))
#ifdef SSX_JIT_BUILD
#include "ssx_fmath.h"
#else
#include "../../include/ssx_fmath.h"
#endif
#define SSX_GM_TABLE (SSX_FM_TABLE + SSX_FM_I_A11)
#ifdef SSX_JIT_BUILD
#include "ssx_glibc_math.h"
#else
#include "../../include/ssx_glibc_math.h"
#endif
__device__ const double ssx_fm_coeff_values[SSX_FM_N_COEFF] = SSX_FM_COEFF_INIT;
__device__ const double ssx_gm_coeff_values[SSX_GM_N_COEFF] = SSX_GM_COEFF_INIT;
static_assert(2 * SSX_FM_N_COEFF <= SSX_LDS_PREFIX_WORDS, "coefficient table");
static_assert(SSX_FM_I_A11 + SSX_GM_N_COEFF <= SSX_FM_N_COEFF, "glibc coefficients in the arc-cosine slots");
// ... 898 lines not shown
			}
			if (c[0] != 0.0f || c[1] != 0.0f || c[2] != 0.0f || c[3] != 0.0f) {
				SSX_STAT(10);
				const uint64_t pushing = __ballot(1);
				const uint32_t slot = q.count + __builtin_amdgcn_mbcnt_hi((uint32_t)(pushing >> 32), __builtin_amdgcn_mbcnt_lo((uint32_t)pushing, 0u));
				const uint32_t nslot = log_append(lg, 1u);
				const uint32_t ni = nee_index(lg, nslot);
				if (NARROW) {
					store_parked_term(a, ni, c);
					float4* E = q.e + 2u * slot;
					E[0] = make_float4(hit_pos.x, hit_pos.y, hit_pos.z, sdir.x);
					E[1] = make_float4(sdir.y, sdir.z, __uint_as_float((light << 8) | hq), __uint_as_float(ni));
				} else {
					float4* E = q.e + 3u * slot;
					E[0] = make_float4(hit_pos.x, hit_pos.y, hit_pos.z, sdir.x);
					E[1] = make_float4(sdir.y, sdir.z, c[0], c[1]);
					E[2] = make_float4(c[2], c[3], __uint_as_float((light << 8) | hq), __uint_as_float(ni));
				}
				level_word = level_word_nee(level_word, nslot);
				pushed = true;
			}
		}
	}

	V3 w_i; float pdf_w_i; float f_s[4];
	if (lambert) {
		SSX_STAT(11);
		w_i = rand_coshemi<GLIBC>(p.rng, pdf_w_i);
		w_i = get_rotated_to(w_i, N);
#pragma unroll
		for (int k = 0; k < 4; ++k) f_s[k] = f_lamb[k];
	} else {
		w_i = reflect3(mk(-p.dir.x, -p.dir.y, -p.dir.z), N);
		pdf_w_i = __builtin_inff();
#pragma unroll
		for (int k = 0; k < 4; ++k) f_s[k] = alb.v[k];
	}
	bool cont = false;
	float n_dot_l = 0.0f;
	float dotfs = (f_s[0] * f_s[0] + f_s[1] * f_s[1]) + (f_s[2] * f_s[2] + f_s[3] * f_s[3]);
	if (dotfs > 0.0f) {
		if (__builtin_isfinite(pdf_w_i)) n_dot_l = dot3(w_i, N);
		else { n_dot_l = 1.0f; pdf_w_i = 1.0f; }
		cont = n_dot_l > 0.0f;
	}
	if (!cont || (els && p.depth + 2u >= SSX_MAX_DEPTH_)) return false;
	SSX_STAT(12);
	const uint32_t slot = log_append(lg, 0u);
	store_level_entry(a, lg, slot, f_s, n_dot_l, pdf_w_i, p.prev_slot, level_word);
	wave_release(lg.cnt);
	p.prev_slot = slot;
	p.dir = w_i; p.ignore = (int)hq;
	++p.depth;
	return true;
}

template <int TOPO, bool NARROW>
__device__ __forceinline__ void shadow_flush(const Lds& L, const SsxKernelArgs& a, const ShadowQ& q, uint32_t first, uint32_t n, SsxTimer& tm) {
	const uint32_t lane = threadIdx.x & 63u;
	const bool have = lane < n;
	const bool narrow = NARROW;
	float4 e0 = make_float4(0.0f, 0.0f, 0.0f, 0.0f), e1 = make_float4(0.0f, 1.0f, 0.0f, 0.0f), e2 = e0;
	if (have) {
		if (narrow) { const float4* E = q.e + 2u * (first + lane); e0 = E[0]; e1 = E[1]; e2.z = e1.z; e2.w = e1.w; }
		else { const float4* E = q.e + 3u * (first + lane); e0 = E[0]; e1 = E[1]; e2 = E[2]; }
	}
	const uint32_t tag = __float_as_uint(e2.z);
	HitInfo sh;
	trace<TOPO>(L, mk(e0.x, e0.y, e0.z), mk(e0.w, e1.x, e1.y), (int)(tag & 0xFFu), have, sh, 2, nullptr, &tm);
	if (have) {
		const bool visible = sh.tri >= 0 && ((uint32_t)sh.tri >> 1) == (tag >> 8);
		store_shadow_outcome<NARROW>(a, __float_as_uint(e2.w), visible, e1.z, e1.w, e2.x, e2.y);
		wave_release(q.cnt);
	}
}

__device__ __forceinline__ const __attribute__((address_space(4))) SsxKernelArgs& cold_args() {
	auto p = __builtin_amdgcn_kernarg_segment_ptr();
	asm volatile("" : "+s"(p));
	return *(const __attribute__((address_space(4))) SsxKernelArgs*)p;
}
__device__ __forceinline__ double ld_agent(const double* p) { return __hip_atomic_load(p, __ATOMIC_RELAXED, __HIP_MEMORY_SCOPE_AGENT); }
__device__ __forceinline__ void st_agent(double* p, double v) { __hip_atomic_store(p, v, __ATOMIC_RELAXED, __HIP_MEMORY_SCOPE_AGENT); }
__device__ __forceinline__ void add_sample(bool rgb_mode, double acc[4], float x, float y, float z, float alpha) {
	if (rgb_mode) { acc[0] += (double)x; acc[1] += (double)y; acc[2] += (double)z; acc[3] += (double)alpha; }
	else { acc[0] += (double)(x * 0.001f); acc[1] += (double)(y * 0.001f); acc[2] += (double)(z * 0.001f); acc[3] += (double)(alpha * 0.001f); }
}
__device__ __forceinline__ void stage_sample(float4* rec, float x, float y, float z, float alpha) {
	uint64_t* const q = reinterpret_cast<uint64_t*>(rec);
	__hip_atomic_store(q, (uint64_t)__float_as_uint(x) | ((uint64_t)__float_as_uint(y) << 32), __ATOMIC_RELAXED, __HIP_MEMORY_SCOPE_AGENT);
	__hip_atomic_store(q + 1, (uint64_t)__float_as_uint(z) | ((uint64_t)__float_as_uint(alpha) << 32), __ATOMIC_RELAXED, __HIP_MEMORY_SCOPE_AGENT);
}
__device__ __forceinline__ void add_staged_sample(bool rgb_mode, double acc[4], const float4* rec) {
	const uint64_t* const q = reinterpret_cast<const uint64_t*>(rec);
	const uint64_t lo = __hip_atomic_load(q, __ATOMIC_RELAXED, __HIP_MEMORY_SCOPE_AGENT), hi = __hip_atomic_load(q + 1, __ATOMIC_RELAXED, __HIP_MEMORY_SCOPE_AGENT);
	add_sample(rgb_mode, acc, __uint_as_float((uint32_t)lo), __uint_as_float((uint32_t)(lo >> 32)), __uint_as_float((uint32_t)hi), __uint_as_float((uint32_t)(hi >> 32)));
}
template <bool NARROW>
__device__ __forceinline__ float4 nee_term(const SsxKernelArgs& a, uint32_t i, bool has) {
	uint32_t v = 1u;
	float4 c = make_float4(0.0f, 0.0f, 0.0f, 0.0f);
	if (has) {
		if (NARROW) v = log_vis(a, i);
		c = log_nee(a, i);
	}
	if (!NARROW) return c;
	return make_float4(v ? c.x : 0.0f, v ? c.y : 0.0f, v ? c.z : 0.0f, v ? c.w : 0.0f);
}
template <uint32_t WAYS, bool NARROW, bool FLUX = false, bool PLAIN = false>
__device__ __forceinline__ void resolve_records(const Lds& L, const SsxKernelArgs& a, uint32_t r0, uint32_t stride, uint32_t count, uint32_t fs_base, uint32_t nee_base, uint32_t rc0, double acc[4], bool stage) {
	float rad[WAYS][4];
	uint32_t depth[WAYS];
	uint32_t K[WAYS];
	uint32_t at[WAYS];
	uint32_t top = 0;
	const float4 zero4 = make_float4(0.0f, 0.0f, 0.0f, 0.0f);
#pragma unroll
	for (uint32_t s = 0; s < WAYS; ++s) {
		depth[s] = 0; K[s] = 0; at[s] = 0;
		rad[s][0] = rad[s][1] = rad[s][2] = rad[s][3] = 0.0f;
		if (s < count) {
			const uint32_t y = a.st[r0 + s * stride].y;
			const uint32_t dep = (y >> 2) & 0xFu;
			depth[s] = dep | ((y & 1u) << 4);
			at[s] = (y >> 6) & SSX_NO_SLOT;
			const uint32_t ns = y >> 19;
			float4 last = zero4;
			if ((y >> 1) & 1u) {
				last = log_direct(a, nee_base + dep * SSX_COHORT_RECORDS + rc0 + s * 64u);
				last = make_float4(0.0f + last.x, 0.0f + last.y, 0.0f + last.z, 0.0f + last.w);
			}
			const float4 ne = nee_term<NARROW>(a, nee_base + ns, ns != SSX_NO_SLOT);
			if (dep) K[s] = log_link(a, fs_base + at[s]);
			rad[s][0] = last.x + ne.x; rad[s][1] = last.y + ne.y; rad[s][2] = last.z + ne.z; rad[s][3] = last.w + ne.w;
			top = max(top, dep);
		}
	}
	for (uint32_t d = top; d-- > 0u;) {
		float4 D[WAYS], F[WAYS]; float2 NP[WAYS];
#pragma unroll
		for (uint32_t s = 0; s < WAYS; ++s)
			if (d < (depth[s] & 0xFu)) {
				const uint32_t i = fs_base + at[s];
				F[s] = log_fs(a, i); NP[s] = log_np(a, i);
				const uint32_t ns = (K[s] >> 13) & SSX_NO_SLOT;
				const bool has_ne = ns != SSX_NO_SLOT;
				D[s] = nee_term<NARROW>(a, nee_base + ns, has_ne);
				if ((K[s] >> 26) & 1u) {
					const float4 em = log_direct(a, nee_base + d * SSX_COHORT_RECORDS + rc0 + s * 64u);
					D[s] = make_float4((0.0f + em.x) + D[s].x, (0.0f + em.y) + D[s].y, (0.0f + em.z) + D[s].z, (0.0f + em.w) + D[s].w);
				}
				at[s] = K[s] & SSX_NO_SLOT;
				if (d) K[s] = log_link(a, fs_base + at[s]);
			}
#pragma unroll
		for (uint32_t s = 0; s < WAYS; ++s)
			if (d < (depth[s] & 0xFu)) {
				SSX_STAT(14);
				const double pdf_recip = ssx_exact::div64_rcp_any(NP[s].y);
				rad[s][0] = (0.0f + D[s].x) + ssx_exact::div64_by((rad[s][0] * NP[s].x) * F[s].x, pdf_recip);
				rad[s][1] = (0.0f + D[s].y) + ssx_exact::div64_by((rad[s][1] * NP[s].x) * F[s].y, pdf_recip);
				rad[s][2] = (0.0f + D[s].z) + ssx_exact::div64_by((rad[s][2] * NP[s].x) * F[s].z, pdf_recip);
				rad[s][3] = (0.0f + D[s].w) + ssx_exact::div64_by((rad[s][3] * NP[s].x) * F[s].w, pdf_recip);
			}
	}
	const __attribute__((address_space(4))) SsxKernelArgs& c = cold_args();
	const bool rgb_mode = !PLAIN && c.rgb_mode != 0u, keep_samples = !PLAIN && c.keep_samples != 0u, no_flat_field = !PLAIN && c.no_flat_field != 0u;
#pragma unroll
	for (uint32_t s = 0; s < WAYS; ++s)
		if (s < count) {
			SSX_STAT(15);
			if (no_flat_field) {
				const float4 cr = a.ray[r0 + s * stride];
				const SsxBlobHeader& hh = L.hdr();
				const float d = dot3(mk(cr.x, cr.y, cr.z), mk(hh.cam_dir[0], hh.cam_dir[1], hh.cam_dir[2]));
				rad[s][0] *= d; rad[s][1] *= d; rad[s][2] *= d; rad[s][3] *= d;
			}
			Hero flux; flux.v[0] = rad[s][0]; flux.v[1] = rad[s][1]; flux.v[2] = rad[s][2]; flux.v[3] = rad[s][3];
			if (FLUX) c.flux[r0 + s * stride] = make_float4(rad[s][0], rad[s][1], rad[s][2], rad[s][3]);
			float xyz[3];
			if (rgb_mode) { xyz[0] = rad[s][0]; xyz[1] = rad[s][1]; xyz[2] = rad[s][2]; }
			else flux_to_xyz(L, flux, __uint_as_float(a.st[r0 + s * stride].x), xyz);
			const float alpha = (depth[s] >> 4) ? 1.0f : 0.0f;
			if (stage) stage_sample(a.ray + (r0 + s * stride), xyz[0], xyz[1], xyz[2], alpha);
			else {
				add_sample(rgb_mode, acc, xyz[0], xyz[1], xyz[2], alpha);
				if (keep_samples) a.ray[r0 + s * stride] = make_float4(xyz[0], xyz[1], xyz[2], alpha);
			}
		}
}

}

template <typename Args>
__device__ __forceinline__ uint32_t tile_of_slot(const Args& a, uint32_t slot, uint32_t& tx, uint32_t& ty) {
	const uint32_t t = a.tile_first + slot * a.tile_stride;
	ty = t / a.tiles_x;
	const uint32_t txr = t - ty * a.tiles_x, rot = (ty * a.tile_skew) % a.tiles_x;
	tx = txr >= rot ? txr - rot : txr + a.tiles_x - rot;
	return ty * a.tiles_x + tx;
}
__device__ __forceinline__ void generate_body(const SsxKernelArgs& a) {
	Lds L; L.w = stage_lds(a);
	const SsxBlobHeader& h = L.hdr();
	const V3 cam = mk(h.cam_pos[0], h.cam_pos[1], h.cam_pos[2]);
	const uint32_t n_k = a.k1 - a.k0;
	const uint32_t lane = threadIdx.x & 63u;
	const uint64_t n_waves = a.n_records >> 6;
	for (uint64_t sk = (uint64_t)blockIdx.x * (blockDim.x >> 6) + (threadIdx.x >> 6); sk < n_waves; sk += (uint64_t)gridDim.x * (blockDim.x >> 6)) {
		const uint32_t slot = (uint32_t)(sk / n_k), kk = a.k0 + (uint32_t)(sk % n_k);
		uint32_t tx, ty;
		(void)tile_of_slot(a, slot, tx, ty);
		const uint32_t i = tx * 8u + (lane & 7u), j = ty * 8u + (lane >> 3);
		const bool inside = i < a.width && j < a.height;
		float4 ray = make_float4(0.0f, 0.0f, 1.0f, 0.0f); uint4 st = make_uint4(0u, 0u, 0u, 0u);
		if (inside) generate_sample(h, a, i, j, kk, ray, st);
		const uint64_t r = sk * 64u + lane;
		if (!a.pre_hits) {
			if (inside) { a.ray[r] = ray; a.st[r] = st; }
			continue;
		}
		HitInfo hit;
		trace<0>(L, cam, mk(ray.x, ray.y, ray.z), -1, inside, hit, 16, a.tile_mask + 4u * slot);
		if (inside) {
			float st_x = 0.0f, st_y = 0.0f;
			if (hit.tri >= 0) {
				const SsxBlobQuad& Q = L.quad((uint32_t)hit.tri >> 1);
				if (Q.albedo_mode != 0u) hit_st(Q, (uint32_t)hit.tri & 1u, hit, st_x, st_y);
			} else {
				st = make_uint4(__float_as_uint(ray.w), tail_word(level_word_none(), 0u, 0u, SSX_NO_SLOT), st.x, st.y);
			}
			a.ray[r] = ray;
			a.st[r] = st;
			a.hit[r] = make_float4(hit.dist, st_x, st_y, __int_as_float(hit.tri));
		}
	}
}
#ifndef SSX_JIT_BUILD
extern "C" __global__ void __launch_bounds__(256) ssx_generate_kernel(SsxKernelArgs a) { generate_body(a); }

extern "C" __global__ void __launch_bounds__(256) ssx_tile_mask_kernel(SsxKernelArgs a) {
	const SsxBlobHeader& h = *reinterpret_cast<const SsxBlobHeader*>(a.blob);
	const uint32_t slot = blockIdx.x * 4u + (threadIdx.x >> 6), lane = threadIdx.x & 63u;
	if (slot >= a.my_tiles) return;
	uint32_t tx, ty;
	(void)tile_of_slot(a, slot, tx, ty);
	const double x0 = (double)(tx * 8u), y0 = (double)(ty * 8u);
	double d[4][3], c[3];
	camera_dir(h, a, x0, y0, d[0][0], d[0][1], d[0][2]);
	camera_dir(h, a, x0 + 8.0, y0, d[1][0], d[1][1], d[1][2]);
	camera_dir(h, a, x0 + 8.0, y0 + 8.0, d[2][0], d[2][1], d[2][2]);
	camera_dir(h, a, x0, y0 + 8.0, d[3][0], d[3][1], d[3][2]);
	camera_dir(h, a, x0 + 4.0, y0 + 4.0, c[0], c[1], c[2]);
	double n[4][3];
#pragma unroll
	for (int k = 0; k < 4; ++k) {
		const double* p = d[k]; const double* q = d[(k + 1) & 3];
		double nx = p[1] * q[2] - p[2] * q[1], ny = p[2] * q[0] - p[0] * q[2], nz = p[0] * q[1] - p[1] * q[0];
		const double inv = 1.0 / __builtin_sqrt(nx * nx + ny * ny + nz * nz);
		const double sgn = (nx * c[0] + ny * c[1] + nz * c[2]) < 0.0 ? -inv : inv;
		n[k][0] = nx * sgn; n[k][1] = ny * sgn; n[k][2] = nz * sgn;
	}
	const SsxBlobQuad* quads = reinterpret_cast<const SsxBlobQuad*>(a.blob + h.off_quads);
	for (uint32_t g = 0; g < 2u; ++g) {
		const uint32_t q = g * 64u + lane;
		bool keep = false;
		if (q < h.n_quads) {
			keep = true;
#pragma unroll
			for (int k = 0; k < 4; ++k) {
				bool all_out = true;
#pragma unroll
				for (int v = 0; v < 4; ++v) {
					const double vx = (double)quads[q].pos[v][0] - (double)h.cam_pos[0], vy = (double)quads[q].pos[v][1] - (double)h.cam_pos[1], vz = (double)quads[q].pos[v][2] - (double)h.cam_pos[2];
					const double dist = __builtin_sqrt(vx * vx + vy * vy + vz * vz);
					const double sd = n[k][0] * vx + n[k][1] * vy + n[k][2] * vz;
					all_out = all_out && (sd < -1.0e-4 * dist);
				}
				if (all_out) keep = false;
			}
		}
		const uint64_t m = __ballot(keep);
		if (lane == 0u) { a.tile_mask[4u * slot + 2u * g] = (uint32_t)m; a.tile_mask[4u * slot + 2u * g + 1u] = (uint32_t)(m >> 32); }
	}
}
#endif

struct WorkUnit {
	uint32_t slot, grp;
	uint32_t tile;
	uint32_t txy;
	uint32_t dims;
	__device__ __forceinline__ uint32_t tw() const { return dims & 15u; }
	__device__ __forceinline__ uint32_t th() const { return (dims >> 4) & 15u; }
	__device__ __forceinline__ uint32_t n_kq() const { return dims >> 8; }
	__device__ __forceinline__ uint32_t npx() const { return tw() * th(); }
	__device__ __forceinline__ uint32_t n_items() const { return npx() * n_kq(); }
	__device__ __forceinline__ uint32_t k_off(const SsxKernelArgs& a) const { return grp * a.group_spp; }
	__device__ __forceinline__ uint32_t rec_base(const SsxKernelArgs& a) const { return (slot * (a.k1 - a.k0) + grp * a.group_spp) * 64u; }
};
__device__ __forceinline__ void unit_setup(const SsxKernelArgs& hot, uint32_t unit, WorkUnit& u) {
	(void)hot;
	const __attribute__((address_space(4))) SsxKernelArgs& a = cold_args();
	const uint32_t slot = unit % a.my_tiles, grp = unit / a.my_tiles;
	uint32_t tx, ty;
	const uint32_t tile = tile_of_slot(a, slot, tx, ty);
	const uint32_t ka = a.k0 + grp * a.group_spp;
	const uint32_t kb = min(ka + a.group_spp, a.k1);
	u.dims = min(8u, a.width - tx * 8u) | (min(8u, a.height - ty * 8u) << 4) | ((kb - ka) << 8);
	u.slot = slot; u.grp = grp;
	u.tile = tile; u.txy = tx | (ty << 16);
}
__device__ __forceinline__ void sums_release(uint32_t* cnt) {
#ifdef SSX_ACCUM_FORMAL
	wave_release(cnt);
	wave_acquire(cnt);
#else
	(void)cnt;
	__builtin_amdgcn_fence(__ATOMIC_RELEASE, "workgroup");
	asm volatile("s_waitcnt vmcnt(0)" ::: "memory");
#endif
}
__device__ __forceinline__ void sums_acquire(uint32_t* cnt) {
#ifdef SSX_ACCUM_FORMAL
	wave_release(cnt);
	wave_acquire(cnt);
#else
	(void)cnt;
	__builtin_amdgcn_fence(__ATOMIC_ACQUIRE, "workgroup");
#endif
}
#ifdef SSX_ACCUM_FORMAL
#define SSX_SUMS_ACQ __ATOMIC_ACQUIRE
#define SSX_SUMS_ACQ_REL __ATOMIC_ACQ_REL
#else
#define SSX_SUMS_ACQ __ATOMIC_RELAXED
#define SSX_SUMS_ACQ_REL __ATOMIC_RELAXED
#endif
template <bool PLAIN = false>
__device__ __forceinline__ void sums_chain(uint32_t slot, uint32_t grp, uint32_t lane, uint32_t* cnt) {
	const __attribute__((address_space(4))) SsxKernelArgs& a = cold_args();
	uint32_t tx, ty;
	const uint32_t tile = tile_of_slot(a, slot, tx, ty);
	const bool has_px = (lane & 7u) < min(8u, a.width - tx * 8u) && (lane >> 3) < min(8u, a.height - ty * 8u);
	double* const px = a.accum + (size_t)tile * 256u + lane;
	uint32_t* state = a.unit_state + (slot * a.n_groups + grp);
	uint32_t rec_at = (slot * (a.k1 - a.k0) + grp * a.group_spp) * 64u;
	double acc[4] = { 0.0, 0.0, 0.0, 0.0 };
	if (has_px) { acc[0] = ld_agent(px); acc[1] = ld_agent(px + 64); acc[2] = ld_agent(px + 128); acc[3] = ld_agent(px + 192); }
	for (;;) {
		const uint32_t n = min(a.group_spp, (a.k1 - a.k0) - grp * a.group_spp);
		if (has_px) {
			for (uint32_t kq = 0; kq < n; ++kq) add_staged_sample(!PLAIN && a.rgb_mode != 0u, acc, a.ray + (rec_at + kq * 64u + lane));
			st_agent(px, acc[0]); st_agent(px + 64, acc[1]); st_agent(px + 128, acc[2]); st_agent(px + 192, acc[3]);
		}
		if (++grp >= a.n_groups) return;
		sums_release(cnt);
		++state; rec_at += a.group_spp * 64u;
		uint32_t was = 0u;
		if (lane == 0u) was = __hip_atomic_fetch_or(state, SSX_UNIT_TURN, SSX_SUMS_ACQ_REL, __HIP_MEMORY_SCOPE_AGENT);
		was = (uint32_t)__builtin_amdgcn_readfirstlane((int)was);
		sums_acquire(cnt);
		if (was != SSX_UNIT_PARKED) return;
		if (lane == 0u) atomicAdd(a.unit_counter + 3, 1u);
	}
}
template <bool NARROW, bool FLUX = false, bool PLAIN = false>
__device__ __forceinline__ void unit_fold(const Lds& L, const SsxKernelArgs& a, const WorkUnit& u, uint32_t wave_slot, uint32_t tag, uint32_t* cnt) {
	wave_acquire(cnt);
	__builtin_amdgcn_fence(__ATOMIC_RELEASE, "workgroup");
	__builtin_amdgcn_fence(__ATOMIC_ACQUIRE, "agent");
	const uint32_t lane = threadIdx.x & 63u;
	const bool has_px = (lane & 7u) < u.tw() && (lane >> 3) < u.th();
	const __attribute__((address_space(4))) SsxKernelArgs& c = cold_args();
	uint32_t* const state = c.unit_state + (u.slot * c.n_groups + u.grp);
	double* const px = c.accum + (size_t)u.tile * 256u + lane;
	bool mine = true;
	if (u.grp) {
		mine = ((uint32_t)__builtin_amdgcn_readfirstlane((int)__hip_atomic_load(state, SSX_SUMS_ACQ, __HIP_MEMORY_SCOPE_AGENT)) & SSX_UNIT_TURN) != 0u;
		sums_acquire(cnt);
	}
	double acc[4] = { 0.0, 0.0, 0.0, 0.0 };
	if (mine && has_px) { acc[0] = ld_agent(px); acc[1] = ld_agent(px + 64); acc[2] = ld_agent(px + 128); acc[3] = ld_agent(px + 192); }
	if (has_px)
		for (uint32_t kq = 0, n_kq = u.n_kq(), rec_base = u.rec_base(a); kq < n_kq; kq += SSX_COHORT_KS) {
			const uint32_t log_rec = log_region(a, wave_slot, tag, kq / SSX_COHORT_KS);
			resolve_records<SSX_COHORT_KS, NARROW, FLUX, PLAIN>(L, a, rec_base + kq * 64u + lane, 64u, min(SSX_COHORT_KS, n_kq - kq), log_rec * SSX_MAX_FRAMES, log_rec * SSX_MAX_LEVELS, lane, acc, !mine);
		}
	if (mine) {
		if (has_px) { st_agent(px, acc[0]); st_agent(px + 64, acc[1]); st_agent(px + 128, acc[2]); st_agent(px + 192, acc[3]); }
		if (u.grp + 1u >= c.n_groups) return;
		sums_release(cnt);
		uint32_t was = 0u;
		if (lane == 0u) was = __hip_atomic_fetch_or(state + 1, SSX_UNIT_TURN, SSX_SUMS_ACQ_REL, __HIP_MEMORY_SCOPE_AGENT);
		was = (uint32_t)__builtin_amdgcn_readfirstlane((int)was);
		sums_acquire(cnt);
		if (was != SSX_UNIT_PARKED) return;
		if (lane == 0u) atomicAdd(c.unit_counter + 3, 1u);
		sums_chain<PLAIN>(u.slot, u.grp + 1u, lane, cnt);
	} else {
		sums_release(cnt);
		uint32_t was = 0u;
		if (lane == 0u) {
			atomicAdd(c.unit_counter + 2, 1u);
			uint32_t expected = 0u;
			(void)__hip_atomic_compare_exchange_strong(state, &expected, SSX_UNIT_PARKED, SSX_SUMS_ACQ_REL, SSX_SUMS_ACQ, __HIP_MEMORY_SCOPE_AGENT);
			was = expected;
		}
		was = (uint32_t)__builtin_amdgcn_readfirstlane((int)was);
		sums_acquire(cnt);
		if (was == SSX_UNIT_TURN) sums_chain<PLAIN>(u.slot, u.grp, lane, cnt);
	}
}

template <int TOPO, bool NARROW, bool CALIB = false, bool GLIBC = false, bool FLUX = false, bool PLAIN = false>
__device__ __forceinline__ void render_body(const SsxKernelArgs& a) {
	constexpr bool FUSE_GEN = TOPO == 2;
	uint32_t* const lds_words = stage_lds<GLIBC>(a);
	Lds L; L.w = lds_words;

	const uint32_t wave = (uint32_t)__builtin_amdgcn_readfirstlane((int)(threadIdx.x >> 6)), lane = threadIdx.x & 63u;
	const uint32_t wave_slot = blockIdx.x * 4u + wave;
	const SsxBlobHeader& hg = *reinterpret_cast<const SsxBlobHeader*>(a.blob);
	const V3 cam = mk(hg.cam_pos[0], hg.cam_pos[1], hg.cam_pos[2]);

	Path p;
	p.orig = mk(0.0f, 0.0f, 0.0f); p.dir = mk(0.0f, 0.0f, 1.0f); p.ignore = -1; p.depth = 0; p.rec_index = 0; p.lambda_0 = 0.0f; p.prev_slot = SSX_NO_SLOT;
	p.hit_tri = 0; p.hit_dist = 0.0f; p.hit_st_x = p.hit_st_y = 0.0f;
	p.rng.state = 0; p.rng.inc = 1;
	bool active = false;
	uint32_t p_tag = 0;
	constexpr uint32_t queue_words = SSX_QUEUE_ENTRIES * (NARROW ? SSX_QUEUE_WORDS_NARROW : SSX_QUEUE_WORDS_WIDE);
	uint32_t* const log_cnt = lds_words + a.blob_words + 4u * queue_words + wave * SSX_WAVE_COUNTER_WORDS;
	SsxTimer tm;
#ifdef SSX_REGTIME
	tm.acc = reinterpret_cast<unsigned long long*>(lds_words + a.blob_words + 4u * queue_words + 4u * SSX_WAVE_COUNTER_WORDS) + wave * SSX_NTIME;
	if (lane < (uint32_t)SSX_NTIME) tm.acc[lane] = 0ull;
	tm.last = __builtin_amdgcn_s_memtime();
#endif
	ShadowQ sq;
	sq.e = reinterpret_cast<float4*>(lds_words + a.blob_words + wave * queue_words);
	sq.count = 0; sq.cnt = log_cnt;
	WorkUnit cur, old;
	bool cur_valid = false, old_pending = false, more = true;
	uint32_t cur_tag = 0, old_tag = 0;
	uint32_t next_item = 0;
	uint32_t grab = 0;
	auto end_path = [&](uint32_t level_word, uint32_t hit_anything) {
		const uint32_t tail = tail_word(level_word, hit_anything, p.depth, p.prev_slot);
		a.st[p.rec_index] = make_uint4(__float_as_uint(p.lambda_0), tail, (uint32_t)p.rng.state, (uint32_t)(p.rng.state >> 32));
		wave_release(log_cnt);
		active = false;
	};
	auto refill = [&](bool with_hit) {
		const uint32_t n_items = cur.n_items();
		if (!(cur_valid && next_item < n_items)) return;
		const uint64_t idle = __ballot(!active);
		if (!active) {
			const uint32_t item = next_item + __builtin_amdgcn_mbcnt_hi((uint32_t)(idle >> 32), __builtin_amdgcn_mbcnt_lo((uint32_t)idle, 0u));
			if (item < n_items) {
				SSX_STAT(19);
				uint32_t in_tile, kq;
				const uint32_t npx = cur.npx(), tw = cur.tw();
				if (npx == 64u) { in_tile = item & 63u; kq = item >> 6; }
				else { const uint32_t r = item % npx; kq = item / npx; in_tile = (r / tw) * 8u + r % tw; }
				p.rec_index = cur.rec_base(a) + kq * 64u + in_tile;
				float4 ray; uint4 st;
				if (FUSE_GEN && a.fuse_gen) {
					const __attribute__((address_space(4))) SsxKernelArgs& c = cold_args();
					generate_sample<PLAIN>(L.hdr(), c, (cur.txy & 0xFFFFu) * 8u + (in_tile & 7u), (cur.txy >> 16) * 8u + (in_tile >> 3), c.k0 + cur.grp * c.group_spp + kq, ray, st);
					if (!PLAIN && c.no_flat_field) c.ray[p.rec_index] = ray;
				} else {
					ray = a.ray[p.rec_index];
					st = a.st[p.rec_index];
// ... 88 lines not shown
				if (hit.tri < 0) end_path(level_word_none(), p.depth ? 1u : 0u);
				else {
					const SsxBlobQuad& Q = L.quad((uint32_t)hit.tri >> 1);
					if (Q.albedo_mode != 0u) hit_st(Q, (uint32_t)hit.tri & 1u, hit, st_x, st_y);
				}
			}
			p.hit_st_x = st_x; p.hit_st_y = st_y;
		}
		SSX_TIME(tm, 9);
		if (a.pre_hits) refill(true);
		SSX_TIME(tm, 10);
		if (!__any(active) && !cur_valid && !more && !old_pending && sq.count == 0u) break;
	}
#ifdef SSX_REGTIME
	if (lane < (uint32_t)SSX_NTIME) atomicAdd(&g_regtime[lane], tm.acc[lane]);
#endif
}

#ifndef SSX_WAVES_PER_EU
#define SSX_WAVES_PER_EU 4
#endif
#ifndef SSX_JIT_GLIBC
#define SSX_JIT_GLIBC 0
#endif
#ifndef SSX_JIT_FLUX
#define SSX_JIT_FLUX 0
#endif
#ifndef SSX_JIT_PLAIN
#define SSX_JIT_PLAIN 0
#endif
#define SSX_PATH_KERNEL(name, topo, narrow, glibc, flux, plain) \
	extern "C" __global__ void __launch_bounds__(256) __attribute__((amdgpu_waves_per_eu(SSX_WAVES_PER_EU))) name(SsxKernelArgs a) { render_body<topo, narrow, false, glibc, flux, plain>(a); }
#ifdef SSX_JIT_BUILD
#ifdef SSX_JIT_DEBUG
extern "C" __global__ void __launch_bounds__(256) ssx_debug_trace_jit(SsxKernelArgs a, const uint32_t* in, uint32_t in_words, uint32_t* out, uint32_t out_words, uint32_t n) {
	debug_trace_rows<3>(a, in, in_words, out, out_words, n);
}
#else
SSX_PATH_KERNEL(ssx_render_kernel_jit, 3, false, SSX_JIT_GLIBC, SSX_JIT_FLUX, SSX_JIT_PLAIN)
SSX_PATH_KERNEL(ssx_render_kernel_jit_nq, 3, true, SSX_JIT_GLIBC, SSX_JIT_FLUX, SSX_JIT_PLAIN)
#endif
#else
SSX_PATH_KERNEL(ssx_render_kernel, 0, false, false, false, false)
SSX_PATH_KERNEL(ssx_render_kernel_cornell, 1, false, false, false, false)
SSX_PATH_KERNEL(ssx_render_kernel_plain, 0, false, false, false, true)
SSX_PATH_KERNEL(ssx_render_kernel_cornell_plain, 1, false, false, false, true)
#if !defined(SSX_PROBE_BUILD) || defined(SSX_PROBE_PLANE)
SSX_PATH_KERNEL(ssx_render_kernel_plane, 2, false, false, false, false)
SSX_PATH_KERNEL(ssx_render_kernel_plane_plain, 2, false, false, false, true)
#endif
#ifndef SSX_PROBE_BUILD
SSX_PATH_KERNEL(ssx_render_kernel_nq, 0, true, false, false, false)
SSX_PATH_KERNEL(ssx_render_kernel_cornell_nq, 1, true, false, false, false)
SSX_PATH_KERNEL(ssx_render_kernel_plane_nq, 2, true, false, false, false)
SSX_PATH_KERNEL(ssx_render_kernel_nq_plain, 0, true, false, false, true)
SSX_PATH_KERNEL(ssx_render_kernel_cornell_nq_plain, 1, true, false, false, true)
SSX_PATH_KERNEL(ssx_render_kernel_plane_nq_plain, 2, true, false, false, true)
SSX_PATH_KERNEL(ssx_render_kernel_glibc, 0, false, true, false, false)
SSX_PATH_KERNEL(ssx_render_kernel_cornell_glibc, 1, false, true, false, false)
SSX_PATH_KERNEL(ssx_render_kernel_plane_glibc, 2, false, true, false, false)
SSX_PATH_KERNEL(ssx_render_kernel_nq_glibc, 0, true, true, false, false)
SSX_PATH_KERNEL(ssx_render_kernel_cornell_nq_glibc, 1, true, true, false, false)
SSX_PATH_KERNEL(ssx_render_kernel_plane_nq_glibc, 2, true, true, false, false)
SSX_PATH_KERNEL(ssx_render_kernel_flux, 0, false, false, true, false)
SSX_PATH_KERNEL(ssx_render_kernel_cornell_flux, 1, false, false, true, false)
SSX_PATH_KERNEL(ssx_render_kernel_plane_flux, 2, false, false, true, false)
SSX_PATH_KERNEL(ssx_render_kernel_nq_flux, 0, true, false, true, false)
SSX_PATH_KERNEL(ssx_render_kernel_cornell_nq_flux, 1, true, false, true, false)
SSX_PATH_KERNEL(ssx_render_kernel_plane_nq_flux, 2, true, false, true, false)
#endif
extern "C" __global__ void __launch_bounds__(256) __attribute__((amdgpu_waves_per_eu(3))) ssx_calibrate_kernel(SsxKernelArgs a) { render_body<0, true, true>(a); }
#endif

#ifndef SSX_JIT_BUILD
#include "ssx_pixel_grid.h"
extern "C" __global__ void __launch_bounds__(256) ssx_finalize_kernel(const double* accum, float4* out, SsxPixelGrid g, uint32_t spp, uint32_t rgb_mode, uint32_t done_tiles) {
	const uint32_t p = blockIdx.x * blockDim.x + threadIdx.x;
	if (p >= g.width * g.height) return;
	const uint32_t i = p % g.width, j = p / g.width;
	const uint32_t tile = ssx_shared_tile(g, i, j);
	float4 o = make_float4(0.0f, 0.0f, 0.0f, 0.0f);
	if (tile % g.tile_stride == g.tile_first && tile / g.tile_stride < done_tiles) {
		const double* const px = accum + ssx_sum_slot(i, j, g.tiles_x);
		if (rgb_mode) {
			const double n = (double)spp;
			o.x = (float)(px[0] / n);
			o.y = (float)(px[64] / n);
			o.z = (float)(px[128] / n);
			o.w = (float)(px[192] / n);
		} else {
			const double sc = 1000.0 / (double)spp;
			o.x = (float)(px[0] * sc);
			o.y = (float)(px[64] * sc);
			o.z = (float)(px[128] * sc);
			o.w = (float)(px[192] * sc);
		}
	}
	out[p] = o;
}

extern "C" __global__ void __launch_bounds__(256) ssx_sum_kernel(float4* dst, const float4* src, uint32_t n) {
	const uint32_t p = blockIdx.x * blockDim.x + threadIdx.x;
	if (p >= n) return;
	const float4 a = dst[p], b = src[p];
	dst[p] = make_float4(a.x + b.x, a.y + b.y, a.z + b.z, a.w + b.w);
}
#endif
```

### simple_spectral_amd/renderer.py

```python
import ctypes as C
import os
from dataclasses import dataclass, field
from typing import Optional, Tuple

import numpy as np

from . import _capi

ROOT = os.path.dirname(os.path.dirname(os.path.abspath(__file__)))
DEFAULT_DATA_DIR = os.path.join(ROOT, "data")


class SsxError(RuntimeError):
    def __init__(self, code, message):
        super().__init__("ssx error %d: %s" % (code, message))
        self.code = code


def _host(fn, *args):
    host = _capi.host_lib()
    rc = getattr(host, fn)(*args)
    if rc != 0:
        raise SsxError(rc, host.ssh_last_error().decode())

# ... 1075 lines not shown
        return out

    def defocus_images(self, q, depth, defocus):
        q = np.ascontiguousarray(q, dtype=np.float32)
        depth = np.ascontiguousarray(depth, dtype=np.float32)
        if q.ndim != 3 or depth.shape != q.shape[:2]:
            raise ValueError("defocus_images: q must have shape [H, W, B], depth [H, W]")
        H, W, B = q.shape
        df, keep = _defocus_arg(defocus)
        if keep[0].size != B:
            raise ValueError("defocus_images: an aperture for %d bins, q has %d" % (keep[0].size, B))
        out = np.zeros((H, W, B), dtype=np.float32)
        self._check(self._lib.ssx_defocus_images(self._ctx, W, H, B, q.ctypes.data, depth.ctypes.data, C.byref(df), out.ctypes.data))
        return out

    def debug_sample_flux(self, **over):
        p = self.params(**over)
        flux = np.zeros((p.height, p.width, p.spp, 4), dtype=np.float32)
        lambda_0 = np.zeros((p.height, p.width, p.spp), dtype=np.float32)
        self._check(self._lib.ssx_debug_sample_flux(self._ctx, C.byref(p), flux.ctypes.data, lambda_0.ctypes.data))
        return flux, lambda_0

    def render_device(self, d_ptr, stream=0, **over):
        p = self.params(**over)
        self._check(self._lib.ssx_render_device(self._ctx, C.byref(p), C.c_void_p(d_ptr), C.c_void_p(stream)))

    def render_device_wait(self):
        self._check(self._lib.ssx_render_device_wait(self._ctx))

    def set_jit(self, mode=_capi.SSX_JIT_AT_UPLOAD):
        self._check(self._lib.ssx_set_jit(self._ctx, int(mode)))

    def jit_status(self, wait_ms=0):
        buf = C.create_string_buffer(1024)
        st = self._lib.ssx_jit_status(self._ctx, int(wait_ms), buf, len(buf))
        if st < -1:
            self._check(st)
        return st, buf.value.decode(errors="replace")

    def upload_scene_desc(self, desc):
        self._check(self._lib.ssx_upload_scene(self._ctx, C.byref(desc) if not hasattr(desc, "contents") else desc))

    def debug_eval(self, op, inputs, out_words):
        x = np.ascontiguousarray(inputs)
        assert x.ndim == 2 and x.dtype.itemsize == 4
        out = np.zeros((x.shape[0], out_words), dtype=np.uint32)
        self._check(self._lib.ssx_debug_eval(self._ctx, op, x.ctypes.data, x.shape[1], out.ctypes.data, out_words, x.shape[0]))
        return out

    def debug_sweep(self, op, lo=0, count=1 << 32):
        res = (C.c_uint64 * 11)()
        self._check(self._lib.ssx_debug_sweep(self._ctx, op, lo, count, res))
        return int(res[0]), int(res[1]), [int(res[3 + k]) for k in range(min(int(res[2]), 8))]

    def debug_samples(self, **over):
        p = self.params(**over)
        xyza = np.zeros((p.height, p.width, p.spp, 4), dtype=np.float32)
        state = np.zeros((p.height, p.width, p.spp), dtype=np.uint64)
        levels = np.zeros((p.height, p.width, p.spp), dtype=np.uint32)
        self._check(self._lib.ssx_debug_samples(self._ctx, C.byref(p), xyza.ctypes.data, state.ctypes.data, levels.ctypes.data))
        return xyza, state, levels

    def debug_tile_mask(self, **over):
        p = self.params(**over)
        tx, ty = (p.width + 7) // 8, (p.height + 7) // 8
        slots = (tx * ty - p.tile_first + p.tile_stride - 1) // p.tile_stride if tx * ty > p.tile_first else 0
        out = np.zeros((slots, 4), dtype=np.uint32)
        self._check(self._lib.ssx_debug_tile_mask(self._ctx, C.byref(p), out.ctypes.data))
        return out

    def debug_generate(self, k0=0, n_k=1, pre_hits=-1, **over):
        p = self.params(**over)
        tx, ty = (p.width + 7) // 8, (p.height + 7) // 8
        slots = (tx * ty - p.tile_first + p.tile_stride - 1) // p.tile_stride if tx * ty > p.tile_first else 0
        ray, st, hit = (np.zeros((slots, int(n_k), 64, 4), dtype=np.uint32) for _ in range(3))
        self._check(self._lib.ssx_debug_generate(self._ctx, C.byref(p), int(k0), int(n_k), int(pre_hits), ray.ctypes.data, st.ctypes.data, hit.ctypes.data))
        return ray, st, hit

    def generate_info(self):
        a, b = C.c_uint64(), C.c_uint64()
        self._check(self._lib.ssx_generate_info(self._ctx, C.byref(a), C.byref(b)))
        return {"generate_launches": a.value, "fused_launches": b.value}

    def debug_fold(self, levels, spp, order_seed=0, parked=False, flux=False, **over):
        x = np.ascontiguousarray(levels, dtype=np.uint32)
        if x.ndim != 2 or x.shape[1] != _capi.SSX_FOLD_ROW_WORDS or spp < 1 or x.shape[0] % spp:
            raise ValueError("debug_fold: levels must be [n_pixels * spp, %d] words" % _capi.SSX_FOLD_ROW_WORDS)
        n, n_pixels = x.shape[0], x.shape[0] // spp
        fl = np.zeros((n, 4), dtype=np.uint32) if flux else None
        xyza, sums = np.zeros((n, 4), dtype=np.uint32), np.zeros((n_pixels, 4), dtype=np.float64)
        self._check(self._lib.ssx_debug_fold(self._ctx, C.byref(self.params(**over)), n_pixels, int(spp), x.ctypes.data, int(order_seed) & 0xFFFFFFFF, int(bool(parked)),
                                             None if fl is None else fl.ctypes.data, xyza.ctypes.data, sums.ctypes.data))
        return fl, xyza, sums

    def debug_step(self, rows, n_rounds, **over):
        x = np.ascontiguousarray(rows, dtype=np.uint32)
        if x.ndim != 2 or x.shape[1] != _capi.SSX_STEP_ROW_WORDS:
            raise ValueError("debug_step: rows must be [n, %d] words" % _capi.SSX_STEP_ROW_WORDS)
        out = np.zeros((x.shape[0], _capi.SSX_STEP_OUT_WORDS), dtype=np.uint32)
        self._check(self._lib.ssx_debug_step(self._ctx, C.byref(self.params(**over)), x.shape[0], int(n_rounds), x.ctypes.data, out.ctypes.data))
        return out

    def debug_spectral_accumulate(self, flux, lambda_0, bins, lambda_min, lambda_step, n_k=None, tile_first=0, tile_stride=1, tile_skew=0, moments=True):
        flux, lambda_0 = np.ascontiguousarray(flux, dtype=np.float32), np.ascontiguousarray(lambda_0, dtype=np.float32)
        if flux.ndim != 4 or flux.shape[3] != 4 or lambda_0.shape != flux.shape[:3]:
            raise ValueError("debug_spectral_accumulate: flux must have shape [H, W, K, 4], lambda_0 [H, W, K]")
        H, W, K = lambda_0.shape
        n_k = np.ascontiguousarray([K] if n_k is None else n_k, dtype=np.uint32)
        if n_k.ndim != 1 or int(n_k.astype(np.uint64).sum()) != K:
            raise ValueError("debug_spectral_accumulate: the launch lengths n_k must add up to K = %d" % K)
        B = int(bins)
        sums, counts = np.zeros((H, W, B), dtype=np.float64), np.zeros((H, W, max(B // 4, 1)), dtype=np.uint32)
        q = np.zeros((H, W, B), dtype=np.float64) if moments else None
        self._check(self._lib.ssx_debug_spectral_accumulate(self._ctx, W, H, B, int(tile_first), int(tile_stride), int(tile_skew), float(lambda_min), float(lambda_step),
                                                            len(n_k), n_k.ctypes.data, flux.ctypes.data, lambda_0.ctypes.data, sums.ctypes.data, counts.ctypes.data,
                                                            None if q is None else q.ctypes.data))
        return sums, counts, q

    def set_timing(self, enable=True):
        self._check(self._lib.ssx_set_timing(self._ctx, int(enable)))

    def get_timing(self):
        ms = (C.c_float * 4)()
        self._check(self._lib.ssx_get_timing(self._ctx, ms))
        return dict(zip(("generate", "path", "resolve", "accumulate"), [float(x) for x in ms]))

    def kernel_info(self):
        v = [C.c_int() for _ in range(5)]
        self._check(self._lib.ssx_kernel_info(self._ctx, *[C.byref(x) for x in v]))
        return dict(zip(("vgprs", "sgprs", "lds_bytes", "scratch_bytes", "max_blocks_per_cu"), [x.value for x in v]))

    def plan_info(self):
        f, k = C.c_float(), C.c_int()
        self._check(self._lib.ssx_plan_info(self._ctx, C.byref(f), C.byref(k)))
        variant = {0: "generic", 1: "cornell topology", 2: "plane topology", 3: "scene topology (compiled at upload)"}.get(self._lib.ssx_kernel_variant(self._ctx), "?")
        name = self._lib.ssx_kernel_name(self._ctx)
        left, pre = C.c_float(), C.c_int()
        if hasattr(self._lib, "ssx_calibration_info"):
            self._check(self._lib.ssx_calibration_info(self._ctx, None, C.byref(left), C.byref(pre)))
        fused = (not pre.value) and variant == "plane topology" and not (os.environ.get("SSX_DEBUG_ENV") == "1" and os.environ.get("SSX_FUSE_GEN", "")[:1] == "0")
        return {"frames_per_sample": round(f.value, 3), "fold": "path kernel", "pass1": variant,
                "rays_left_per_sample": round(left.value, 3), "camera_rays": "pre-traced (generate kernel)" if pre.value else "path loop",
                "samples_made_in": "path kernel (refill)" if fused else "generate kernel",
                "kernel": name.decode() if name else None,
                "switches": "compiled in" if hasattr(self._lib, "ssx_switches_info") and self._lib.ssx_switches_info(self._ctx) == 1 else "run time"}

    def scratch_info(self):
        a, b = C.c_uint64(), C.c_uint64()
        if hasattr(self._lib, "ssx_scratch_info"):
            self._check(self._lib.ssx_scratch_info(self._ctx, C.byref(a), C.byref(b)))
        return {"sample_bytes": a.value, "log_bytes": b.value}

    def sums_info(self):
        a, b = C.c_uint64(), C.c_uint64()
        if hasattr(self._lib, "ssx_sums_info"):
            self._check(self._lib.ssx_sums_info(self._ctx, C.byref(a), C.byref(b)))
        u = C.c_uint64()
        if hasattr(self._lib, "ssx_units_info"):
            self._check(self._lib.ssx_units_info(self._ctx, C.byref(u)))
        return {"units_parked": a.value, "units_chained": b.value, "units": u.value}

    def save(self, path):
        fb = np.ascontiguousarray(self.framebuffer, dtype=np.float32)
        _host("ssh_save_image", path.encode(), fb.ctypes.data, fb.shape[1], fb.shape[0])

    def close(self):
# ... 10 lines not shown
```

Before: 3212.

## Fold sum clears, counter resets and tile mask into one prepare kernel; write image in fold

Replaces the per-launch hipMemsetAsync calls (sums clear, unit counter, unit state) and the separate tile-mask kernel with a single ssx_prepare_kernel that zeroes those buffers and builds the tile mask. The path kernel's fold step now writes the final XYZA pixel directly when the last group completes, so the separate finalize kernel is skipped in the common non-RGB device render path. This aims to cut launch and fill overhead and an extra pass over the accumulation buffer, at the cost of more logic in the fold tail and new invariants about when the image can be written from the fold.

New measurement: 3216 (median of 2 runs). About the same (+0.1%).

```diff
diff --git a/include/ssx.h b/include/ssx.h
--- a/include/ssx.h
+++ b/include/ssx.h
@@ -152,6 +152,7 @@
 int ssx_sums_info(ssx_ctx* ctx, uint64_t* units_parked, uint64_t* units_chained);
 int ssx_units_info(ssx_ctx* ctx, uint64_t* units_enqueued);
 int ssx_generate_info(ssx_ctx* ctx, uint64_t* generate_launches, uint64_t* fused_launches);
+int ssx_launch_info(ssx_ctx* ctx, uint64_t* kernels_launched, uint64_t* fills_enqueued, uint64_t* finalize_kernels, uint64_t* fold_images);
 int ssx_kernel_variant(ssx_ctx* ctx);
 enum { SSX_JIT_OFF = 0, SSX_JIT_AT_UPLOAD = 1, SSX_JIT_BACKGROUND = 2 };
 int ssx_set_jit(ssx_ctx* ctx, int mode);
diff --git a/simple_spectral_amd/_capi.py b/simple_spectral_amd/_capi.py
--- a/simple_spectral_amd/_capi.py
+++ b/simple_spectral_amd/_capi.py
@@ -147,7 +147,7 @@
                "ssx_defocus_images", "ssx_spectral_develop_lens",
                "ssx_sensor_images", "ssx_demosaic_images", "ssx_spectral_develop_sensor",
                "ssx_debug_tile_mask", "ssx_debug_spectral_accumulate", "ssx_debug_fold", "ssx_debug_step",
-               "ssx_debug_generate", "ssx_generate_info",
+               "ssx_debug_generate", "ssx_generate_info", "ssx_launch_info",
                "ssx_scene_traits", "ssx_render_traits", "ssx_switches_info"]
 SSX_GENERATE_FILL_BYTE = 0xA6
 SSX_FOLD_ROW_WORDS, SSX_FOLD_LAMBDA0, SSX_FOLD_CAM_DIR, SSX_FOLD_HIT, SSX_FOLD_N, SSX_FOLD_LEVEL0, SSX_FOLD_LEVEL_WORDS = 160, 0, 1, 4, 5, 10, 15
@@ -435,6 +435,8 @@
         if not override or hasattr(lib, "ssx_debug_generate"):
             lib.ssx_debug_generate.argtypes = [vp, C.POINTER(SsxRenderParams), C.c_uint32, C.c_uint32, C.c_int, vp, vp, vp]
             lib.ssx_generate_info.argtypes = [vp, C.POINTER(C.c_uint64), C.POINTER(C.c_uint64)]
+        if not override or hasattr(lib, "ssx_launch_info"):
+            lib.ssx_launch_info.argtypes = [vp] + [C.POINTER(C.c_uint64)] * 4
         lib.ssx_kernel_variant.argtypes = [vp]
         lib.ssx_kernel_name.argtypes = [vp]
         lib.ssx_kernel_name.restype = C.c_char_p
diff --git a/simple_spectral_amd/csrc/ssx_api.hip b/simple_spectral_amd/csrc/ssx_api.hip
--- a/simple_spectral_amd/csrc/ssx_api.hip
+++ b/simple_spectral_amd/csrc/ssx_api.hip
@@ -108,6 +108,7 @@
 	int worker_rc = 0;
 	std::atomic<uint64_t> units_enqueued{0};
 	std::atomic<uint64_t> launches_generated{0}, launches_fused{0};
+	std::atomic<uint64_t> kernels_launched{0}, fills_enqueued{0}, finalize_launched{0}, fold_images{0};
 	ssx_render_params cur{};
 	struct SumsState { bool continuable = false, noise_valid = false, spectral_valid = false, moments_valid = false, imported = false, spectral_imported = false; uint32_t noise_batches = 0; } sums;
 	uint32_t k_begin = 0;
@@ -215,6 +216,7 @@
 
 int clear_sums(ssx_ctx* ctx, uint32_t width, uint32_t height, hipStream_t stream) {
 	SSX_HIP(ctx, hipMemsetAsync(ctx->d_accum.ptr, 0, accum_bytes(width, height), stream));
+	ctx->fills_enqueued.fetch_add(1u);
 	return SSX_OK;
 }
 void sums_invalidate(ssx_ctx* ctx) { ctx->sums = ssx_ctx::SumsState{}; }
@@ -455,32 +457,46 @@
 	return ctx->topology == 2u && !a.pre_hits && tiles_fit && !(fuse_env && fuse_env[0] == '0');
 }
 
+bool fold_image_allowed() { const char* e = debug_env("SSX_FOLD_IMAGE"); return !(e && e[0] == '0'); }
+
+int enqueue_prepare(ssx_ctx* ctx, Batch& b, hipStream_t stream) {
+	if (!ctx->d_unit_counter.ptr) {
+		SSX_HIP(ctx, ctx->d_unit_counter.reserve(4 * sizeof(uint32_t)));
+		SSX_HIP(ctx, hipMemsetAsync(ctx->d_unit_counter.ptr, 0, 4 * sizeof(uint32_t), stream));
+		ctx->fills_enqueued.fetch_add(1u);
+	}
+	b.a.unit_counter = ctx->d_unit_counter.as<uint32_t>();
+	const SsxKernelArgs& a = b.a;
+	uint64_t want = ((uint64_t)a.clear_vec4 + 255u) / 256u;
+	want = std::max<uint64_t>(want, ((uint64_t)b.units / 4u + 255u) / 256u);
+	if (a.pre_hits && !a.fuse_gen) want = std::max<uint64_t>(want, ((uint64_t)a.my_tiles + 3u) / 4u);
+	if (a.image && a.tile_stride > 1u) want = std::max<uint64_t>(want, ((uint64_t)a.n_tiles + 3u) / 4u);
+	const uint64_t most = (uint64_t)(ctx->n_cus > 0 ? ctx->n_cus : 1) * 4u;
+	const uint32_t blocks = (uint32_t)std::min<uint64_t>(std::max<uint64_t>(want, 1u), most);
+	hipLaunchKernelGGL(ssx_prepare_kernel, dim3(blocks), dim3(256), 0, stream, b.a);
+	SSX_HIP(ctx, hipGetLastError());
+	ctx->kernels_launched.fetch_add(1u);
+	return SSX_OK;
+}
+
 int enqueue_generate(ssx_ctx* ctx, const Batch& b, hipStream_t stream) {
 	SsxKernelArgs ga = b.a;
 	ga.blob_words = ctx->blob_words;
-	if (ga.pre_hits) {
-		hipLaunchKernelGGL(ssx_tile_mask_kernel, dim3((ga.my_tiles + 3u) / 4u), dim3(256), 0, stream, ga);
-		SSX_HIP(ctx, hipGetLastError());
-	}
 	const KernelRef gen_kernel{ (const void*)ssx_generate_kernel };
 	const size_t gen_lds = staged_blob_lds(ga.blob_words);
 	if (ctx->gen_blocks == 0) { const int rc = blocks_that_fit(ctx, gen_kernel, gen_lds, &ctx->gen_blocks); if (rc) return rc; }
 	const uint64_t want = (b.n_rec + 255u) / 256u;
+	ctx->kernels_launched.fetch_add(1u);
 	return launch_kernel(ctx, gen_kernel, (uint32_t)(want < (uint64_t)ctx->gen_blocks ? want : (uint64_t)ctx->gen_blocks), gen_lds, stream, ga);
 }
 
 int enqueue_path(ssx_ctx* ctx, Batch& b, const KernelRef& kernel, uint32_t queue_words, uint32_t blob_words, int resident_blocks, hipStream_t stream) {
-	if (!ctx->d_unit_counter.ptr) {
-		SSX_HIP(ctx, ctx->d_unit_counter.reserve(4 * sizeof(uint32_t)));
-		SSX_HIP(ctx, hipMemsetAsync(ctx->d_unit_counter.ptr, 0, 4 * sizeof(uint32_t), stream));
-	}
+	if (!b.a.unit_counter) return fail(ctx, SSX_ERR_STATE, "internal: path kernel enqueued without the launch's set-up kernel");
 	b.a.blob_words = blob_words; b.a.queue_words = queue_words;
-	SSX_HIP(ctx, hipMemsetAsync(ctx->d_unit_counter.ptr, 0, 2 * sizeof(uint32_t), stream));
-	SSX_HIP(ctx, hipMemsetAsync(b.a.unit_state, 0, (size_t)b.units * sizeof(uint32_t), stream));
-	b.a.unit_counter = ctx->d_unit_counter.as<uint32_t>();
 	const uint32_t want_blocks = (b.units + 3u) / 4u;
 	uint32_t blocks = want_blocks < (uint32_t)resident_blocks ? want_blocks : (uint32_t)resident_blocks;
 	if (blocks * 4u > ctx->max_wave_slots) blocks = ctx->max_wave_slots / 4u;
+	ctx->kernels_launched.fetch_add(1u);
 	return launch_kernel(ctx, kernel, blocks, path_lds_bytes(blob_words, queue_words), stream, b.a);
 }
 
@@ -491,6 +507,8 @@
 		return fail(ctx, SSX_ERR_STATE, "internal: a render with a switch set was about to launch the kernel with the switches compiled in");
 	if (ctx->timing) { if ((rc = timing_events(ctx, &b.tev))) return rc; SSX_HIP(ctx, hipEventRecord(b.tev[0], stream)); }
 	b.a.fuse_gen = fuses_generate(ctx, b.a) ? 1u : 0u;
+	if (b.a.image && (!b.a.fuse_resolve || b.a.rgb_mode || b.a.keep_samples)) return fail(ctx, SSX_ERR_STATE, "internal: the fold was to write the image of a render that needs the finalize kernel");
+	if ((rc = enqueue_prepare(ctx, b, stream))) return rc;
 	if (!b.a.fuse_gen && (rc = enqueue_generate(ctx, b, stream))) return rc;
 	if (ctx->timing) SSX_HIP(ctx, hipEventRecord(b.tev[1], stream));
 	const bool plan = ctx->resident_blocks == 0;
@@ -500,6 +518,7 @@
 	if ((rc = enqueue_path(ctx, b, path_kernel, ctx->queue_words, b.a.blob_words, ctx->resident_blocks, stream))) return rc;
 	ctx->units_enqueued.fetch_add(b.units);
 	(b.a.fuse_gen ? ctx->launches_fused : ctx->launches_generated).fetch_add(1u);
+	if (b.a.image) ctx->fold_images.fetch_add(1u);
 	if (ctx->timing) for (int k = 2; k < 6; ++k) SSX_HIP(ctx, hipEventRecord(b.tev[k], stream));
 	return SSX_OK;
 }
@@ -546,15 +565,23 @@
 	return SSX_OK;
 }
 
-int launch_range(ssx_ctx* ctx, LaunchPlan& pl, uint32_t k0, uint32_t k1, hipStream_t stream) {
-	if (pl.args.my_tiles == 0 || k1 <= k0) return SSX_OK;
+struct LaunchExtras { bool clear_sums = false; float* image = nullptr; uint32_t image_spp = 0; };
+
+int launch_range(ssx_ctx* ctx, LaunchPlan& pl, uint32_t k0, uint32_t k1, hipStream_t stream, const LaunchExtras& x = LaunchExtras{}) {
+	if (pl.args.my_tiles == 0 || k1 <= k0) return (x.clear_sums || x.image) ? fail(ctx, SSX_ERR_STATE, "internal: an empty launch was to clear the sums or write the image") : SSX_OK;
 	Batch b = make_batch(ctx, pl, k0, k1);
+	b.a.clear_vec4 = x.clear_sums ? (uint32_t)(accum_bytes(pl.args.width, pl.args.height) / 16u) : 0u;
+	b.a.image = reinterpret_cast<float4*>(x.image); b.a.image_spp = x.image_spp;
 	return launch_batch(ctx, b, stream);
 }
 
-int launch_batches(ssx_ctx* ctx, LaunchPlan& pl, uint32_t spp, uint32_t batch, hipStream_t stream) {
+int launch_batches(ssx_ctx* ctx, LaunchPlan& pl, uint32_t spp, uint32_t batch, hipStream_t stream, const LaunchExtras& x = LaunchExtras{}) {
 	for (uint32_t k0 = 0; k0 < spp; k0 += batch) {
-		int rc = launch_range(ctx, pl, k0, (spp - k0 < batch) ? spp : k0 + batch, stream);
+		const uint32_t k1 = (spp - k0 < batch) ? spp : k0 + batch;
+		LaunchExtras lx;
+		lx.clear_sums = x.clear_sums && k0 == 0u;
+		if (k1 == spp) { lx.image = x.image; lx.image_spp = x.image_spp; }
+		int rc = launch_range(ctx, pl, k0, k1, stream, lx);
 		if (rc) return rc;
 	}
 	return SSX_OK;
@@ -570,6 +597,7 @@
 	if (rc) return rc;
 	Batch b = make_batch(ctx, pl, 0, cp.spp);
 	if (b.rc) return b.rc;
+	if ((rc = enqueue_prepare(ctx, b, ctx->stream))) return rc;
 	if ((rc = enqueue_generate(ctx, b, ctx->stream))) return rc;
 	const KernelRef kernel{ (const void*)ssx_calibrate_kernel };
 	int blocks = 0;
@@ -594,6 +622,7 @@
 	hipLaunchKernelGGL(ssx_finalize_kernel, pixel_blocks(p), dim3(256), 0, stream,
 	                   ctx->d_accum.as<const double>(), (float4*)d_out, pixel_grid(p), spp, ctx->rgb_mode ? 1u : 0u, done_tiles);
 	SSX_HIP(ctx, hipGetLastError());
+	ctx->kernels_launched.fetch_add(1u); ctx->finalize_launched.fetch_add(1u);
 	return SSX_OK;
 }
 
@@ -641,7 +670,8 @@
 
 int render_sample_walk(ssx_ctx* ctx, const ssx_render_params& p, uint32_t k_begin, bool continuing) {
 	int rc;
-	if (!continuing && (rc = clear_sums(ctx, p.width, p.height, ctx->stream))) return rc;
+	bool clear_pending = !continuing;
+	if (clear_pending && (owned_tiles(p) == 0u || p.spp <= k_begin)) { if ((rc = clear_sums(ctx, p.width, p.height, ctx->stream))) return rc; clear_pending = false; }
 	if ((rc = noise_begin(ctx, &p, k_begin, continuing))) return rc;
 	maybe_swap_jit(ctx, 0);
 	if ((rc = moments_reserve(ctx, owned_tiles(p), continuing))) return rc;
@@ -657,13 +687,15 @@
 			maybe_swap_jit(ctx, (uint64_t)p.width * p.height * (k1 - k0) / p.tile_stride);
 			if (!ctx->jit_pending) { const uint32_t cap = pl.max_spp_per_launch; pl = make_plan(ctx, &p); pl.max_spp_per_launch = cap; }
 		}
-		if ((rc = launch_range(ctx, pl, k0, k1, ctx->stream))) return rc;
+		LaunchExtras lx; lx.clear_sums = clear_pending; clear_pending = false;
+		if ((rc = launch_range(ctx, pl, k0, k1, ctx->stream, lx))) return rc;
 		if (ctx->noise_on && (rc = noise_batch(ctx, &p, k1 - k0, ctx->stream))) return rc;
 		if (spectral && (rc = spectral_batch(ctx, &p, pl, k1 - k0, ctx->stream))) return rc;
 		if (moments && (rc = moments_batch(ctx, &p, pl, k1 - k0, ctx->stream))) return rc;
 		SSX_HIP(ctx, hipStreamSynchronize(ctx->stream));
 		ctx->done_spp.store(k1);
 	}
+	if (clear_pending && (rc = clear_sums(ctx, p.width, p.height, ctx->stream))) return rc;
 	const uint32_t done = ctx->done_spp.load();
 	if ((rc = finish_walk(ctx, p, done ? done : p.spp, 0xFFFFFFFFu))) return rc;
 	ctx->done_tiles.store(pl.args.my_tiles);
@@ -1005,14 +1037,17 @@
 	}
 	if ((rc = ready_to_launch(ctx, p, false))) return rc;
 	sums_invalidate(ctx);
-	if ((rc = clear_sums(ctx, p->width, p->height, stream))) return rc;
 	if (!capturing) maybe_swap_jit(ctx, (uint64_t)p->width * p->height * p->spp / p->tile_stride);
 	LaunchPlan pl = make_plan(ctx, p, !capturing);
 	if (capturing) cap_to_allocation(ctx, pl);
 	const uint32_t batch = device_batch(p, pl);
 	if ((rc = ensure_samples(ctx, pl, batch))) return rc;
-	if ((rc = launch_batches(ctx, pl, p->spp, batch, stream))) return rc;
-	if ((rc = launch_finalize(ctx, p, p->spp, (float*)d_xyza_out, stream))) return rc;
+	LaunchExtras x;
+	x.clear_sums = pl.args.my_tiles != 0u;
+	if (x.clear_sums && !ctx->rgb_mode && fold_image_allowed()) { x.image = (float*)d_xyza_out; x.image_spp = p->spp; }
+	if (!x.clear_sums && (rc = clear_sums(ctx, p->width, p->height, stream))) return rc;
+	if ((rc = launch_batches(ctx, pl, p->spp, batch, stream, x))) return rc;
+	if (!x.image && (rc = launch_finalize(ctx, p, p->spp, (float*)d_xyza_out, stream))) return rc;
 	if (!capturing) {
 		SSX_HIP(ctx, hipEventRecord(ctx->ev_device_done, stream));
 		ctx->device_pending = true;
@@ -1264,6 +1299,10 @@
 	a.st = reinterpret_cast<uint4*>(d_rec.as<uint8_t>() + rec_bytes);
 	a.hit = reinterpret_cast<float4*>(d_rec.as<uint8_t>() + 2u * rec_bytes);
 	a.tile_mask = d_mask.as<uint32_t>();
+	if (a.pre_hits) {
+		hipLaunchKernelGGL(ssx_tile_mask_kernel, dim3((a.my_tiles + 3u) / 4u), dim3(256), 0, ctx->stream, a);
+		SSX_HIP(ctx, hipGetLastError());
+	}
 	if ((rc = enqueue_generate(ctx, b, ctx->stream))) return rc;
 	SSX_HIP(ctx, hipStreamSynchronize(ctx->stream));
 	SSX_HIP(ctx, hipMemcpy(ray, a.ray, rec_bytes, hipMemcpyDeviceToHost));
@@ -1497,6 +1536,15 @@
 	return SSX_OK;
 }
 
+int ssx_launch_info(ssx_ctx* ctx, uint64_t* kernels_launched, uint64_t* fills_enqueued, uint64_t* finalize_kernels, uint64_t* fold_images) {
+	if (!ctx) return SSX_ERR_ARG;
+	if (kernels_launched) *kernels_launched = ctx->kernels_launched.load();
+	if (fills_enqueued) *fills_enqueued = ctx->fills_enqueued.load();
+	if (finalize_kernels) *finalize_kernels = ctx->finalize_launched.load();
+	if (fold_images) *fold_images = ctx->fold_images.load();
+	return SSX_OK;
+}
+
 int ssx_kernel_variant(ssx_ctx* ctx) { return (ctx && ctx->have_scene) ? (int)ctx->topology : -1; }
 
 const char* ssx_kernel_name(ssx_ctx* ctx) {
diff --git a/simple_spectral_amd/csrc/ssx_blob.h b/simple_spectral_amd/csrc/ssx_blob.h
--- a/simple_spectral_amd/csrc/ssx_blob.h
+++ b/simple_spectral_amd/csrc/ssx_blob.h
@@ -117,4 +117,7 @@
 	double inv_width, inv_height;
 	uint32_t fuse_gen;
 	float4* flux;
+	float4* image;
+	uint32_t image_spp;
+	uint32_t clear_vec4;
 };
diff --git a/simple_spectral_amd/csrc/ssx_kernels.hip b/simple_spectral_amd/csrc/ssx_kernels.hip
--- a/simple_spectral_amd/csrc/ssx_kernels.hip
+++ b/simple_spectral_amd/csrc/ssx_kernels.hip
@@ -1004,6 +1004,32 @@
 }
 __device__ __forceinline__ double ld_agent(const double* p) { return __hip_atomic_load(p, __ATOMIC_RELAXED, __HIP_MEMORY_SCOPE_AGENT); }
 __device__ __forceinline__ void st_agent(double* p, double v) { __hip_atomic_store(p, v, __ATOMIC_RELAXED, __HIP_MEMORY_SCOPE_AGENT); }
+__device__ __forceinline__ float4 pixel_of_sums(double s0, double s1, double s2, double s3, uint32_t spp, bool rgb_mode) {
+	float4 o;
+	if (rgb_mode) {
+		const double n = (double)spp;
+		o.x = (float)(s0 / n);
+		o.y = (float)(s1 / n);
+		o.z = (float)(s2 / n);
+		o.w = (float)(s3 / n);
+	} else {
+		const double sc = 1000.0 / (double)spp;
+		o.x = (float)(s0 * sc);
+		o.y = (float)(s1 * sc);
+		o.z = (float)(s2 * sc);
+		o.w = (float)(s3 * sc);
+	}
+	return o;
+}
+__device__ __forceinline__ void fold_image(const __attribute__((address_space(4))) SsxKernelArgs& c, uint32_t tile, uint32_t lane, bool has_px, const double acc[4]) {
+	float4* const image = c.image;
+	if (image == nullptr) return;
+	uint32_t tile_v, tiles_x_v;
+	asm("v_mov_b32 %0, %1" : "=v"(tile_v) : "s"(tile));
+	asm("v_mov_b32 %0, %1" : "=v"(tiles_x_v) : "s"(c.tiles_x));
+	const uint32_t ty = tile_v / tiles_x_v, tx = tile_v - ty * tiles_x_v;
+	if (has_px) image[(size_t)(ty * 8u + (lane >> 3)) * c.width + (tx * 8u + (lane & 7u))] = pixel_of_sums(acc[0], acc[1], acc[2], acc[3], c.image_spp, false);
+}
 __device__ __forceinline__ void add_sample(bool rgb_mode, double acc[4], float x, float y, float z, float alpha) {
 	if (rgb_mode) { acc[0] += (double)x; acc[1] += (double)y; acc[2] += (double)z; acc[3] += (double)alpha; }
 	else { acc[0] += (double)(x * 0.001f); acc[1] += (double)(y * 0.001f); acc[2] += (double)(z * 0.001f); acc[3] += (double)(alpha * 0.001f); }
@@ -1161,10 +1187,8 @@
 #ifndef SSX_JIT_BUILD
 extern "C" __global__ void __launch_bounds__(256) ssx_generate_kernel(SsxKernelArgs a) { generate_body(a); }
 
-extern "C" __global__ void __launch_bounds__(256) ssx_tile_mask_kernel(SsxKernelArgs a) {
+__device__ __forceinline__ void tile_mask_of_slot(const SsxKernelArgs& a, uint32_t slot, uint32_t lane) {
 	const SsxBlobHeader& h = *reinterpret_cast<const SsxBlobHeader*>(a.blob);
-	const uint32_t slot = blockIdx.x * 4u + (threadIdx.x >> 6), lane = threadIdx.x & 63u;
-	if (slot >= a.my_tiles) return;
 	uint32_t tx, ty;
 	(void)tile_of_slot(a, slot, tx, ty);
 	const double x0 = (double)(tx * 8u), y0 = (double)(ty * 8u);
@@ -1205,6 +1229,35 @@
 		const uint64_t m = __ballot(keep);
 		if (lane == 0u) { a.tile_mask[4u * slot + 2u * g] = (uint32_t)m; a.tile_mask[4u * slot + 2u * g + 1u] = (uint32_t)(m >> 32); }
 	}
+}
+extern "C" __global__ void __launch_bounds__(256) ssx_tile_mask_kernel(SsxKernelArgs a) {
+	const uint32_t slot = blockIdx.x * 4u + (threadIdx.x >> 6);
+	if (slot < a.my_tiles) tile_mask_of_slot(a, slot, threadIdx.x & 63u);
+}
+
+#include "ssx_pixel_grid.h"
+extern "C" __global__ void __launch_bounds__(256) ssx_prepare_kernel(SsxKernelArgs a) {
+	const uint32_t lane = threadIdx.x & 63u;
+	const uint32_t n_threads = gridDim.x * 256u, t = blockIdx.x * 256u + threadIdx.x;
+	const uint32_t n_waves = gridDim.x * 4u, wave = blockIdx.x * 4u + (threadIdx.x >> 6);
+	const uint4 zero = make_uint4(0u, 0u, 0u, 0u);
+	uint4* const sums = reinterpret_cast<uint4*>(a.accum);
+	for (uint32_t i = t; i < a.clear_vec4; i += n_threads) sums[i] = zero;
+	const uint32_t units = a.my_tiles * a.n_groups, units4 = units >> 2;
+	uint4* const state = reinterpret_cast<uint4*>(a.unit_state);
+	for (uint32_t i = t; i < units4; i += n_threads) state[i] = zero;
+	if (t < (units & 3u)) a.unit_state[(units4 << 2) + t] = 0u;
+	if (t < 2u) a.unit_counter[t] = 0u;
+	if (a.image != nullptr && a.tile_stride > 1u) {
+		const SsxPixelGrid g{ a.width, a.height, a.tiles_x, a.tile_first, a.tile_stride, a.tile_skew };
+		for (uint32_t tile = wave; tile < a.n_tiles; tile += n_waves) {
+			const uint32_t ty = tile / a.tiles_x, tx = tile - ty * a.tiles_x;
+			const uint32_t i = tx * 8u + (lane & 7u), j = ty * 8u + (lane >> 3);
+			if (!ssx_owns_pixel(g, i, j) && i < a.width && j < a.height) a.image[(size_t)j * a.width + i] = make_float4(0.0f, 0.0f, 0.0f, 0.0f);
+		}
+	}
+	if (a.pre_hits && !a.fuse_gen)
+		for (uint32_t slot = wave; slot < a.my_tiles; slot += n_waves) tile_mask_of_slot(a, slot, lane);
 }
 #endif
 
@@ -1276,7 +1329,7 @@
 			for (uint32_t kq = 0; kq < n; ++kq) add_staged_sample(!PLAIN && a.rgb_mode != 0u, acc, a.ray + (rec_at + kq * 64u + lane));
 			st_agent(px, acc[0]); st_agent(px + 64, acc[1]); st_agent(px + 128, acc[2]); st_agent(px + 192, acc[3]);
 		}
-		if (++grp >= a.n_groups) return;
+		if (++grp >= a.n_groups) { fold_image(a, tile, lane, has_px, acc); return; }
 		sums_release(cnt);
 		++state; rec_at += a.group_spp * 64u;
 		uint32_t was = 0u;
@@ -1311,7 +1364,7 @@
 		}
 	if (mine) {
 		if (has_px) { st_agent(px, acc[0]); st_agent(px + 64, acc[1]); st_agent(px + 128, acc[2]); st_agent(px + 192, acc[3]); }
-		if (u.grp + 1u >= c.n_groups) return;
+		if (u.grp + 1u >= c.n_groups) { fold_image(c, u.tile, lane, has_px, acc); return; }
 		sums_release(cnt);
 		uint32_t was = 0u;
 		if (lane == 0u) was = __hip_atomic_fetch_or(state + 1, SSX_UNIT_TURN, SSX_SUMS_ACQ_REL, __HIP_MEMORY_SCOPE_AGENT);
@@ -1566,19 +1619,7 @@
 	float4 o = make_float4(0.0f, 0.0f, 0.0f, 0.0f);
 	if (tile % g.tile_stride == g.tile_first && tile / g.tile_stride < done_tiles) {
 		const double* const px = accum + ssx_sum_slot(i, j, g.tiles_x);
-		if (rgb_mode) {
-			const double n = (double)spp;
-			o.x = (float)(px[0] / n);
-			o.y = (float)(px[64] / n);
-			o.z = (float)(px[128] / n);
-			o.w = (float)(px[192] / n);
-		} else {
-			const double sc = 1000.0 / (double)spp;
-			o.x = (float)(px[0] * sc);
-			o.y = (float)(px[64] * sc);
-			o.z = (float)(px[128] * sc);
-			o.w = (float)(px[192] * sc);
-		}
+		o = pixel_of_sums(px[0], px[64], px[128], px[192], spp, rgb_mode != 0u);
 	}
 	out[p] = o;
 }
diff --git a/simple_spectral_amd/renderer.py b/simple_spectral_amd/renderer.py
--- a/simple_spectral_amd/renderer.py
+++ b/simple_spectral_amd/renderer.py
@@ -1181,6 +1181,11 @@
         self._check(self._lib.ssx_generate_info(self._ctx, C.byref(a), C.byref(b)))
         return {"generate_launches": a.value, "fused_launches": b.value}
 
+    def launch_info(self):
+        v = [C.c_uint64() for _ in range(4)]
+        self._check(self._lib.ssx_launch_info(self._ctx, *[C.byref(x) for x in v]))
+        return dict(zip(("kernels_launched", "fills_enqueued", "finalize_kernels", "fold_images"), (x.value for x in v)))
+
     def debug_fold(self, levels, spp, order_seed=0, parked=False, flux=False, **over):
         x = np.ascontiguousarray(levels, dtype=np.uint32)
         if x.ndim != 2 or x.shape[1] != _capi.SSX_FOLD_ROW_WORDS or spp < 1 or x.shape[0] % spp:
```
